# ethz-asl/okvis

Hardware: AMD Instinct MI355X
Metric: Gauss-Newton iterations/sec on 10-KF x 2-cam x 400-landmark windows (batch throughput: window-iterations/s) (higher is better)
Workload: dtype f64

## Files before the change

include/okvis_amd_ba.h:

```cpp
#ifndef OKVIS_AMD_BA_H_
#define OKVIS_AMD_BA_H_

#include <stdint.h>

#ifdef __cplusplus
extern "C" {
#endif

#define OKVIS_BA_ABI_VERSION 7

#define OKVIS_BA_OK 0
#define OKVIS_BA_ERR_ARG (-1)
#define OKVIS_BA_ERR_STATE (-2)
#define OKVIS_BA_ERR_UNSUPPORTED (-3)
#define OKVIS_BA_ERR_NO_DEVICE (-4)
#define OKVIS_BA_ERR_NUMERIC (-5)
#define OKVIS_BA_HIP_ERROR_BASE 1000

#define OKVIS_BA_DIST_NONE 0
#define OKVIS_BA_DIST_RADTAN 1
#define OKVIS_BA_DIST_EQUIDISTANT 2
#define OKVIS_BA_DIST_RADTAN8 3

#define OKVIS_BA_IMU_CACHE_DOUBLES 290
// ... 11 lines not shown
  double a_max;
} okvis_ba_imu_params;

typedef struct okvis_ba_window {
  int32_t n_pose;
  const double* pose;
  const uint8_t* pose_fixed;
  int32_t n_sb;
  const double* sb;
  const uint8_t* sb_fixed;
  int32_t n_lm;
  const double* lm;

  int32_t n_cam;
  const double* cam_intr;
  const int32_t* cam_model;

  int32_t n_obs;
  const int32_t* obs_lm;
  const int32_t* obs_pose;
  const int32_t* obs_ext;
  const int32_t* obs_cam;
  const double* obs_uv;
  const double* obs_sqrtw;
  double cauchy_b;

  int32_t n_imu;
  const int32_t* imu_pose0;
  const int32_t* imu_sb0;
  const int32_t* imu_pose1;
  const int32_t* imu_sb1;
  const int64_t* imu_t0;
  const int64_t* imu_t1;
  const int32_t* imu_s_begin;
  const int32_t* imu_s_count;
  int32_t n_imu_samples;
  const int64_t* imu_s_t;
  const double* imu_s_gyr;
  const double* imu_s_acc;
  okvis_ba_imu_params imu_params;

  int32_t n_pprior;
  const int32_t* pprior_pose;
  const double* pprior_meas;
  const double* pprior_sqrtinfo;

  int32_t n_sbprior;
  const int32_t* sbprior_sb;
  const double* sbprior_meas;
  const double* sbprior_sqrtinfo;

  int32_t n_relpose;
  const int32_t* rel_pose0;
  const int32_t* rel_pose1;
  const double* rel_sqrtinfo;

  int32_t marg_dim;
  int32_t marg_nblocks;
  const int32_t* marg_block_type;
  const int32_t* marg_block_idx;
  const int32_t* marg_block_off;
  const double* marg_J;
  const double* marg_e0;
  const double* marg_lin;

  const double* imu_sb_ref;
  const uint8_t* imu_sb_ref_valid;
  const double* imu_cache;
} okvis_ba_window;

#define OKVIS_BA_STRATEGY_DOGLEG 0
#define OKVIS_BA_STRATEGY_LM 1
#define OKVIS_BA_TUNE_SCHUR_DECIDES 0x1u
#define OKVIS_BA_TUNE_SCHUR_VALU 0x2u
#define OKVIS_BA_TUNE_SCHUR_MFMA_LARGE 0x4u
#define OKVIS_BA_TUNE_NO_LDL_COMP 0x8u
#define OKVIS_BA_TUNE_LDL_COMP_ALL 0x10u
#define OKVIS_BA_TUNE_H0_ON_HOST 0x20u
#define OKVIS_BA_TUNE_NO_EARLY_PREINTEGRATION 0x40u
#define OKVIS_BA_TUNE_NO_MARG_TILES 0x80u
#define OKVIS_BA_TUNE_NO_SMALL_RIDE 0x100u
#define OKVIS_BA_TUNE_SCHUR_SERIAL_BATCHES 0x200u
#define OKVIS_BA_TUNE_LIN_NO_RECORDS 0x400u
#define OKVIS_BA_SOLVE_AUTO 0
#define OKVIS_BA_SOLVE_DENSE 1
#define OKVIS_BA_SOLVE_CHAIN 2
typedef struct okvis_ba_tuning {
  uint32_t flags;
  int32_t fused_max_windows;
  int32_t group_lm;
  int32_t group_work;
  int32_t split_small_min;
  int32_t lin2_occupancy;
  int32_t stagger_us;
  int32_t solve_mode;
} okvis_ba_tuning;
typedef struct okvis_ba_options {
  double initial_radius;
  double max_radius;
  double min_radius;
  double min_lm_diagonal;
  double max_lm_diagonal;
  double min_relative_decrease;
  double function_tolerance;
  double gradient_tolerance;
  double parameter_tolerance;
  int32_t use_graph;
  int32_t schur_lm_per_block;
  int32_t debug_arrays;
  int32_t gauss_newton;
  int32_t n_streams;
  int32_t fp32_linearize;
  int32_t strategy;
  int32_t jacobi_scaling;
  int32_t max_consecutive_invalid_steps;
  int32_t reserved0;
  okvis_ba_tuning tuning;
} okvis_ba_options;

typedef struct okvis_ba_summary {
  double initial_cost;
  double final_cost;
  int32_t iterations;
  int32_t successful_steps;
  int32_t termination;
  int32_t reserved;
  double final_radius;
  double gradient_max_norm;
} okvis_ba_summary;

typedef struct okvis_ba_limits {
  int32_t max_obs_per_lm;
  int32_t max_reduced_dim;
  int32_t max_marg_dim;
  int32_t max_imu_samples_per_factor;
} okvis_ba_limits;

typedef struct okvis_ba_solver okvis_ba_solver;

enum okvis_ba_array {
  OKVIS_BA_ARR_POSE = 0,
  OKVIS_BA_ARR_SB = 1,
  OKVIS_BA_ARR_LM = 2,
  OKVIS_BA_ARR_OBS_RESIDUAL = 3,
  OKVIS_BA_ARR_LM_V = 4,
  OKVIS_BA_ARR_LM_B = 5,
  OKVIS_BA_ARR_LM_HQ = 6,
  OKVIS_BA_ARR_PAIR_W = 7,
  OKVIS_BA_ARR_REDUCED_S = 8,
  OKVIS_BA_ARR_REDUCED_RHS = 9,
  OKVIS_BA_ARR_STEP = 10,
  OKVIS_BA_ARR_LM_QUALITY = 11,
  OKVIS_BA_ARR_GRADIENT = 12,
  OKVIS_BA_ARR_IMU_RESIDUAL = 13,
  OKVIS_BA_ARR_HPP = 14,
  OKVIS_BA_ARR_DAMPING = 15,
  OKVIS_BA_ARR_IMU_SB_REF = 16,
  OKVIS_BA_ARR_IMU_LIN = 17
};
#define OKVIS_BA_IMU_LIN_DOUBLES 511

int okvis_ba_abi_version(void);
void okvis_ba_get_limits(okvis_ba_limits* out);
void okvis_ba_default_options(okvis_ba_options* out);
const char* okvis_ba_error_string(int status);

int okvis_ba_create(okvis_ba_solver** out, int device);
int okvis_ba_destroy(okvis_ba_solver* s);

int okvis_ba_upload(okvis_ba_solver* s, int n_windows, const okvis_ba_window* windows);
int okvis_ba_check_window(const okvis_ba_window* w, const okvis_ba_options* opt, int64_t* stats);
#define OKVIS_BA_LIST_GROUPS 0
#define OKVIS_BA_LIST_LM_OBS_BEGIN 1
#define OKVIS_BA_LIST_LM_PAIR_BEGIN 2
#define OKVIS_BA_LIST_PAIR_LM 3
#define OKVIS_BA_LIST_PAIR_BLOCK 4
#define OKVIS_BA_LIST_PAIR_OFF 5
#define OKVIS_BA_LIST_PAIR_ROLE 6
#define OKVIS_BA_LIST_LM_PIECE_BEGIN 7
#define OKVIS_BA_LIST_PAIR_PIECE 8
#define OKVIS_BA_LIST_PAIR_LIST_BEGIN 9
#define OKVIS_BA_LIST_PAIR_LIST 10
#define OKVIS_BA_LIST_TASKS 11
#define OKVIS_BA_LIST_TASK_LIST 12
#define OKVIS_BA_LIST_CHUNKS 13
#define OKVIS_BA_LIST_CHUNK_DIAG_BEGIN 14
#define OKVIS_BA_LIST_CHUNK_DIAG_OUT 15
#define OKVIS_BA_LIST_CHUNK_DESC 16
#define OKVIS_BA_LIST_PIECE_PATH 17
#define OKVIS_BA_LIST_LDL_COMP 18
#define OKVIS_BA_LIST_CHAIN 19
#define OKVIS_BA_LIST_CHUNK_RECS 20
#define OKVIS_BA_LIST_GROUP_RECS 21
int okvis_ba_check_window_lists(const okvis_ba_window* w, const okvis_ba_options* opt, int32_t n_windows, int32_t which,
                                int32_t* out, int64_t capacity, int64_t* n);
#define OKVIS_BA_PATCH_POSE_PRIORS 1
#define OKVIS_BA_PATCH_SB_PRIORS 2
#define OKVIS_BA_PATCH_RELPOSE 4
#define OKVIS_BA_PATCH_MARG_PRIOR 8
typedef struct okvis_ba_patch {
  int32_t n_remove_obs;  const int32_t* remove_obs;
  int32_t n_remove_lm;   const int32_t* remove_lm;
  int32_t n_remove_pose; const int32_t* remove_pose;
  int32_t n_remove_sb;   const int32_t* remove_sb;
  int32_t n_remove_imu;  const int32_t* remove_imu;
  int32_t n_add_pose; const double* add_pose;  const uint8_t* add_pose_fixed;
  int32_t n_add_sb;   const double* add_sb;    const uint8_t* add_sb_fixed;
  int32_t n_add_lm;   const double* add_lm;
  int32_t n_add_obs;
  const int32_t* add_obs_lm; const int32_t* add_obs_pose; const int32_t* add_obs_ext; const int32_t* add_obs_cam;
  const double* add_obs_uv; const double* add_obs_sqrtw;
  int32_t n_add_imu;
  const int32_t* add_imu_pose0; const int32_t* add_imu_sb0; const int32_t* add_imu_pose1; const int32_t* add_imu_sb1;
  const int64_t* add_imu_t0; const int64_t* add_imu_t1; const int32_t* add_imu_s_begin; const int32_t* add_imu_s_count;
  int32_t n_add_imu_samples;
  const int64_t* add_imu_s_t; const double* add_imu_s_gyr; const double* add_imu_s_acc;
  int32_t replace;
  int32_t n_pprior;  const int32_t* pprior_pose; const double* pprior_meas; const double* pprior_sqrtinfo;
  int32_t n_sbprior; const int32_t* sbprior_sb;  const double* sbprior_meas; const double* sbprior_sqrtinfo;
  int32_t n_relpose; const int32_t* rel_pose0; const int32_t* rel_pose1; const double* rel_sqrtinfo;
  int32_t marg_dim; int32_t marg_nblocks; const int32_t* marg_block_type; const int32_t* marg_block_idx; const int32_t* marg_block_off;
  const double* marg_J; const double* marg_e0; const double* marg_lin;
  int32_t n_set_pose; const int32_t* set_pose_idx; const double* set_pose;
  int32_t n_set_sb;   const int32_t* set_sb_idx;   const double* set_sb;
  int32_t n_set_lm;   const int32_t* set_lm_idx;   const double* set_lm;
  const int32_t* add_lm_before;
} okvis_ba_patch;

typedef struct okvis_ba_window_store okvis_ba_window_store;
int okvis_ba_store_create(const okvis_ba_window* w, okvis_ba_window_store** out);
int okvis_ba_store_patch(okvis_ba_window_store* st, const okvis_ba_patch* p);
int okvis_ba_store_view(const okvis_ba_window_store* st, okvis_ba_window* out);
void okvis_ba_store_destroy(okvis_ba_window_store* st);

int okvis_ba_set_patchable(okvis_ba_solver* s, int on);
int okvis_ba_patch_window(okvis_ba_solver* s, int w, const okvis_ba_patch* p);
int okvis_ba_patched_view(okvis_ba_solver* s, int w, okvis_ba_window* out);
int okvis_ba_set_marg_prior_values(okvis_ba_solver* s, int w, const double* J, const double* e0);

int okvis_ba_set_state(okvis_ba_solver* s, int w, const double* pose, const double* sb, const double* lm);
int okvis_ba_set_options(okvis_ba_solver* s, const okvis_ba_options* opt);

int okvis_ba_optimize(okvis_ba_solver* s, int num_iter, okvis_ba_summary* summaries);

int okvis_ba_optimize_timed(okvis_ba_solver* s, int max_iter, int min_iter, double time_limit_s,
                            okvis_ba_summary* summaries);

int okvis_ba_begin(okvis_ba_solver* s);
int okvis_ba_iterate(okvis_ba_solver* s, int n);
int okvis_ba_finish(okvis_ba_solver* s, okvis_ba_summary* summaries);

int okvis_ba_evaluate_cost(okvis_ba_solver* s, double* costs);

int okvis_ba_get_state(okvis_ba_solver* s, int w, double* pose, double* sb, double* lm);
int okvis_ba_fetch_results(okvis_ba_solver* s, int w, double* pose, double* sb, double* lm, double* lm_quality,
                           double* imu_sb_ref);
int okvis_ba_fetch_imu_caches(okvis_ba_solver* s, int w, double* caches);
int okvis_ba_array_size(okvis_ba_solver* s, int w, int which, int64_t* n_doubles);
int okvis_ba_download(okvis_ba_solver* s, int w, int which, double* out, int64_t n_doubles);
int okvis_ba_reduced_dim(okvis_ba_solver* s, int w, int32_t* dim);
int okvis_ba_pair_count(okvis_ba_solver* s, int w, int32_t* n_pair);
int okvis_ba_pairs(okvis_ba_solver* s, int w, int32_t* pair_lm, int32_t* pair_block);

int okvis_ba_last_iterate_ms(okvis_ba_solver* s, float* total_ms);
int okvis_ba_profile_iterations(okvis_ba_solver* s, int n, float* ms4);
int okvis_ba_profile_launches(okvis_ba_solver* s, int n, float* ms );
int okvis_ba_algorithmic_bytes(okvis_ba_solver* s, int64_t* linearize_bytes, int64_t* schur_bytes,
                               int64_t* solve_bytes, int64_t* small_bytes);
int okvis_ba_synchronize(okvis_ba_solver* s);
int okvis_ba_helper_timeouts(okvis_ba_solver* s, int64_t* count);
#define OKVIS_BA_ROUTE_WINDOWS 0
#define OKVIS_BA_ROUTE_FUSED 1
#define OKVIS_BA_ROUTE_DECISION_FREE_SCHUR 2
#define OKVIS_BA_ROUTE_PIECE_PATH 3
#define OKVIS_BA_ROUTE_SPLIT_SMALL 4
#define OKVIS_BA_ROUTE_SUB_BATCHES 5
#define OKVIS_BA_ROUTE_SUB_BATCH_MAX_WINDOWS 6
#define OKVIS_BA_ROUTE_SCHUR_KERNEL 7
#define OKVIS_BA_ROUTE_SOLVE_DBUF 8
#define OKVIS_BA_ROUTE_SOLVE_TILED 9
#define OKVIS_BA_ROUTE_SOLVE_HELPERS 10
#define OKVIS_BA_ROUTE_GRAPH 11
#define OKVIS_BA_ROUTE_MAX_CHUNKS 12
#define OKVIS_BA_ROUTE_SLOTS 13
#define OKVIS_BA_ROUTE_SOLVE_MODE 14
#define OKVIS_BA_ROUTE_SMALL_RIDES 15
#define OKVIS_BA_ROUTE_LIN_RECORDS 16
#define OKVIS_BA_ROUTE_COUNT 17
int okvis_ba_launch_route(okvis_ba_solver* s, int32_t* route);

#define OKVIS_BA_MARG_MAX_WINDOW_DIM 900
typedef struct okvis_ba_marg_spec {
  const uint8_t* pose_marg;
  const uint8_t* sb_marg;
  int32_t prior_dim, prior_nblocks;
  const int32_t* prior_block_type;
  const int32_t* prior_block_idx;
  const int32_t* prior_block_off;
  const double* prior_H;
  const double* prior_b0;
} okvis_ba_marg_spec;

typedef struct okvis_ba_marg_result {
  int32_t capacity_dim, capacity_blocks;
  int32_t dim, nblocks, rank;
  int32_t* block_type;
  int32_t* block_idx;
  int32_t* block_off;
  double* H;
  double* b0;
  double* J;
  double* e0;
  int32_t sweeps[2];
} okvis_ba_marg_result;

int okvis_ba_marginalize(okvis_ba_solver* s, int w, const okvis_ba_marg_spec* spec, okvis_ba_marg_result* result);
int okvis_ba_marginalize_begin(okvis_ba_solver* s, int w, const okvis_ba_marg_spec* spec, okvis_ba_marg_result* result);
int okvis_ba_marginalize_end(okvis_ba_solver* s, okvis_ba_marg_result* result);
int okvis_ba_marginalize_batch(okvis_ba_solver* s, int w0, int n, const okvis_ba_marg_spec* specs, okvis_ba_marg_result* results);
int okvis_ba_marginalize_batch_begin(okvis_ba_solver* s, int w0, int n, const okvis_ba_marg_spec* specs, okvis_ba_marg_result* results);
int okvis_ba_marginalize_batch_end(okvis_ba_solver* s, okvis_ba_marg_result* results);

#define OKVIS_BA_COV_MAX_WINDOW_DIM 174
#define OKVIS_BA_COV_MAX_DIM 30

typedef struct okvis_ba_cov_spec {
  int32_t n_blocks;
  const int32_t *block_type, *block_idx;
} okvis_ba_cov_spec;

typedef struct okvis_ba_cov_result {
  int32_t capacity;
  int32_t dim, info;
  double min_pivot;
  double* cov;
  double* S0;
} okvis_ba_cov_result;

int okvis_ba_state_covariance(okvis_ba_solver* s, int w0, int n,
                              const okvis_ba_cov_spec* specs, okvis_ba_cov_result* results);
int okvis_ba_last_covariance_ms(okvis_ba_solver* s, float* assembly_ms, float* kernel_ms);

typedef struct okvis_ba_lmcov_spec {
  int32_t n_lm;
  const int32_t* lm_idx;
} okvis_ba_lmcov_spec;

typedef struct okvis_ba_lmcov_result {
  int32_t capacity;
  int32_t n, info;
  double min_pivot;
  double* cov;
  uint8_t* flags;
  double *S0, *Spp, *V, *W;
} okvis_ba_lmcov_result;

int okvis_ba_landmark_covariance(okvis_ba_solver* s, int w0, int n,
                                 const okvis_ba_lmcov_spec* specs, okvis_ba_lmcov_result* results);
int okvis_ba_last_landmark_covariance_ms(okvis_ba_solver* s, float* assembly_ms, float* inverse_ms, float* landmark_ms);

#define OKVIS_BA_PRED_NO_COV 1
#define OKVIS_BA_PRED_NO_PROJECTION 2

typedef struct okvis_ba_pred_spec {
  int32_t n_q;
  const int32_t *q_lm, *q_pose, *q_ext, *q_cam;
} okvis_ba_pred_spec;

typedef struct okvis_ba_pred_result {
  int32_t capacity;
  int32_t n, info;
  double min_pivot;
// ... 35 lines not shown
```

okvis_amd/_lib.py:

```python
from __future__ import annotations

import ctypes as C
import os

from .window import CovResultC, CovSpecC, LimitsC, LmcovResultC, LmcovSpecC, MargResultC, MargSpecC, OptionsC, PatchC, PredResultC, PredSpecC, SummaryC, WindowC

_HERE = os.path.dirname(os.path.abspath(__file__))
LIB_PATH = os.path.join(os.environ.get("OKVIS_AMD_LIB_DIR") or os.path.join(_HERE, "lib"), "libokvis_amd_ba.so")

SYMBOLS = [
    "okvis_ba_abi_version", "okvis_ba_get_limits", "okvis_ba_default_options", "okvis_ba_error_string",
    "okvis_ba_create", "okvis_ba_destroy", "okvis_ba_upload", "okvis_ba_check_window", "okvis_ba_check_window_lists", "okvis_ba_set_state", "okvis_ba_set_options",
    "okvis_ba_optimize", "okvis_ba_optimize_timed", "okvis_ba_begin", "okvis_ba_iterate", "okvis_ba_finish",
    "okvis_ba_evaluate_cost", "okvis_ba_get_state", "okvis_ba_fetch_results", "okvis_ba_fetch_imu_caches", "okvis_ba_array_size", "okvis_ba_download",
    "okvis_ba_reduced_dim", "okvis_ba_pair_count", "okvis_ba_pairs", "okvis_ba_last_iterate_ms",
    "okvis_ba_profile_iterations", "okvis_ba_profile_launches", "okvis_ba_algorithmic_bytes", "okvis_ba_synchronize",
    "okvis_ba_helper_timeouts", "okvis_ba_launch_route", "okvis_ba_marginalize", "okvis_ba_marginalize_begin", "okvis_ba_marginalize_end",
    "okvis_ba_marginalize_batch", "okvis_ba_marginalize_batch_begin", "okvis_ba_marginalize_batch_end",
    "okvis_ba_state_covariance", "okvis_ba_last_covariance_ms",
    "okvis_ba_landmark_covariance", "okvis_ba_last_landmark_covariance_ms",
    "okvis_ba_predicted_measurement", "okvis_ba_last_predicted_measurement_ms",
    "okvis_ba_store_create", "okvis_ba_store_patch", "okvis_ba_store_view", "okvis_ba_store_destroy", "okvis_ba_set_patchable",
    "okvis_ba_patch_window", "okvis_ba_patched_view", "okvis_ba_set_marg_prior_values",
    "okvis_ba_dense_solve", "okvis_ba_reduced_solve", "okvis_ba_shard", "okvis_ba_batch_run", "okvis_ba_gather_records", "okvis_ba_batch_run_gathered",
]

_dp = C.POINTER(C.c_double)
_ip = C.POINTER(C.c_int32)
_lib = None


class BackendError(RuntimeError):
    def __init__(self, status, what=""):
        self.status = status
        msg = lib().okvis_ba_error_string(status).decode() if _lib is not None else str(status)
        super().__init__(f"okvis_ba status {status}: {msg} {what}")


def lib():
    global _lib
    if _lib is not None:
        return _lib
    if not os.path.exists(LIB_PATH):
        raise ImportError(f"{LIB_PATH} is missing: run `python -m okvis_amd.build` (hipcc, gfx950). "
                          "okvis_amd has no CPU fallback.")
    L = C.CDLL(LIB_PATH)
    for s in SYMBOLS:
        getattr(L, s)
    vp = C.c_void_p
    L.okvis_ba_error_string.restype = C.c_char_p
    L.okvis_ba_error_string.argtypes = [C.c_int]
    L.okvis_ba_get_limits.argtypes = [C.POINTER(LimitsC)]
    L.okvis_ba_default_options.argtypes = [C.POINTER(OptionsC)]
    L.okvis_ba_create.argtypes = [C.POINTER(vp), C.c_int]
    L.okvis_ba_destroy.argtypes = [vp]
    L.okvis_ba_upload.argtypes = [vp, C.c_int, C.POINTER(WindowC)]
    L.okvis_ba_set_state.argtypes = [vp, C.c_int, _dp, _dp, _dp]
    L.okvis_ba_store_create.argtypes = [C.POINTER(WindowC), C.POINTER(vp)]
    L.okvis_ba_store_patch.argtypes = [vp, C.POINTER(PatchC)]
    L.okvis_ba_store_view.argtypes = [vp, C.POINTER(WindowC)]
    L.okvis_ba_store_destroy.argtypes = [vp]
    L.okvis_ba_store_destroy.restype = None
    L.okvis_ba_set_patchable.argtypes = [vp, C.c_int]
    L.okvis_ba_patch_window.argtypes = [vp, C.c_int, C.POINTER(PatchC)]
    L.okvis_ba_patched_view.argtypes = [vp, C.c_int, C.POINTER(WindowC)]
    L.okvis_ba_set_marg_prior_values.argtypes = [vp, C.c_int, _dp, _dp]
    L.okvis_ba_check_window.argtypes = [C.POINTER(WindowC), C.POINTER(OptionsC), C.POINTER(C.c_int64)]
    L.okvis_ba_check_window_lists.argtypes = [C.POINTER(WindowC), C.POINTER(OptionsC), C.c_int32, C.c_int32, _ip, C.c_int64,
                                              C.POINTER(C.c_int64)]
    L.okvis_ba_get_state.argtypes = [vp, C.c_int, _dp, _dp, _dp]
    L.okvis_ba_fetch_results.argtypes = [vp, C.c_int, _dp, _dp, _dp, _dp, _dp]
    L.okvis_ba_fetch_imu_caches.argtypes = [vp, C.c_int, _dp]
    L.okvis_ba_set_options.argtypes = [vp, C.POINTER(OptionsC)]
    L.okvis_ba_optimize.argtypes = [vp, C.c_int, C.POINTER(SummaryC)]
    L.okvis_ba_optimize_timed.argtypes = [vp, C.c_int, C.c_int, C.c_double, C.POINTER(SummaryC)]
    L.okvis_ba_begin.argtypes = [vp]
    L.okvis_ba_iterate.argtypes = [vp, C.c_int]
    L.okvis_ba_finish.argtypes = [vp, C.POINTER(SummaryC)]
    L.okvis_ba_dense_solve.argtypes = [C.c_int, C.c_int32, _dp, _dp, _dp, C.POINTER(C.c_int32)]
    L.okvis_ba_reduced_solve.argtypes = [C.c_int, C.c_int32, C.c_int32, C.c_int32, C.c_uint32, _dp, _dp, _dp, C.POINTER(C.c_int64),
                                         C.POINTER(C.c_int32), C.c_int32, _dp, C.c_int64]
    L.okvis_ba_shard.argtypes = [C.c_int32, C.c_int32, C.c_int32, _ip, C.POINTER(C.c_int32)]
    L.okvis_ba_batch_run.argtypes = [C.c_int, C.c_int32, C.c_int32, C.c_int32, C.POINTER(WindowC), C.POINTER(OptionsC), C.c_int,
                                     C.c_void_p, C.POINTER(C.c_int32)]
    L.okvis_ba_marginalize.argtypes = [vp, C.c_int, C.POINTER(MargSpecC), C.POINTER(MargResultC)]
    L.okvis_ba_marginalize_begin.argtypes = [vp, C.c_int, C.POINTER(MargSpecC), C.POINTER(MargResultC)]
    L.okvis_ba_marginalize_end.argtypes = [vp, C.POINTER(MargResultC)]
    L.okvis_ba_marginalize_batch.argtypes = [vp, C.c_int, C.c_int, C.POINTER(MargSpecC), C.POINTER(MargResultC)]
    L.okvis_ba_marginalize_batch_begin.argtypes = [vp, C.c_int, C.c_int, C.POINTER(MargSpecC), C.POINTER(MargResultC)]
    L.okvis_ba_marginalize_batch_end.argtypes = [vp, C.POINTER(MargResultC)]
    L.okvis_ba_state_covariance.argtypes = [vp, C.c_int, C.c_int, C.POINTER(CovSpecC), C.POINTER(CovResultC)]
    L.okvis_ba_last_covariance_ms.argtypes = [vp, C.POINTER(C.c_float), C.POINTER(C.c_float)]
    L.okvis_ba_landmark_covariance.argtypes = [vp, C.c_int, C.c_int, C.POINTER(LmcovSpecC), C.POINTER(LmcovResultC)]
    L.okvis_ba_last_landmark_covariance_ms.argtypes = [vp] + [C.POINTER(C.c_float)] * 3
    L.okvis_ba_predicted_measurement.argtypes = [vp, C.c_int, C.c_int, C.POINTER(PredSpecC), C.POINTER(PredResultC)]
    L.okvis_ba_last_predicted_measurement_ms.argtypes = [vp] + [C.POINTER(C.c_float)] * 3
    L.okvis_ba_evaluate_cost.argtypes = [vp, _dp]
    L.okvis_ba_array_size.argtypes = [vp, C.c_int, C.c_int, C.POINTER(C.c_int64)]
    L.okvis_ba_download.argtypes = [vp, C.c_int, C.c_int, _dp, C.c_int64]
    L.okvis_ba_reduced_dim.argtypes = [vp, C.c_int, _ip]
    L.okvis_ba_pair_count.argtypes = [vp, C.c_int, _ip]
    L.okvis_ba_helper_timeouts.argtypes = [vp, C.POINTER(C.c_int64)]
    L.okvis_ba_launch_route.argtypes = [vp, _ip]
    L.okvis_ba_pairs.argtypes = [vp, C.c_int, _ip, _ip]
    L.okvis_ba_last_iterate_ms.argtypes = [vp, C.POINTER(C.c_float)]
    L.okvis_ba_profile_iterations.argtypes = [vp, C.c_int, C.POINTER(C.c_float)]
    L.okvis_ba_profile_launches.argtypes = [vp, C.c_int, C.POINTER(C.c_float)]
    L.okvis_ba_algorithmic_bytes.argtypes = [vp] + [C.POINTER(C.c_int64)] * 4
    L.okvis_ba_synchronize.argtypes = [vp]
    _lib = L
    return L


def check(status, what=""):
    if status != 0:
        raise BackendError(status, what)
```

okvis_amd/csrc/ba_capi.hip:

```cpp
#include <hip/hip_runtime.h>

#include <algorithm>
#include <array>
#include <chrono>
#include <cstdio>
#include <cstring>
#include <map>
#include <string>
#include <type_traits>
#include <vector>

#include "../../include/okvis_amd_ba.h"
#include "ba_imu.hpp"
#include "ba_chol_tiles.hpp"
#include "ba_cov.hpp"
#include "ba_lmcov.hpp"
#include "ba_predcov.hpp"
#include "ba_linearize.hpp"
#include "ba_linearize2.hpp"
#include "ba_schur2.hpp"
#include "ba_marg.hpp"
#include "ba_marg_tiles.hpp"
#include "ba_schur.hpp"
#include "ba_solve.hpp"
#include "ba_store.hpp"

using namespace ba;

#include "capi_solver.inc"
#include "capi_index_build.inc"
#include "capi_launch.inc"

#define REFUSE_BETWEEN_MARG_HALVES(s) do { if ((s) && (s)->marg_pending.active) return OKVIS_BA_ERR_STATE; } while (0)

extern "C" {

int okvis_ba_abi_version(void) { return OKVIS_BA_ABI_VERSION; }

void okvis_ba_get_limits(okvis_ba_limits* out) {
  if (!out) return;
  out->max_obs_per_lm = GROUP_OBS;
  out->max_reduced_dim = MAX_D;
  out->max_marg_dim = MAX_MARG_DIM;
  out->max_imu_samples_per_factor = MAX_IMU_SAMPLES;
}

void okvis_ba_default_options(okvis_ba_options* o) {
  if (!o) return;
  o->initial_radius = 1e4;
  o->max_radius = 1e16;
  o->min_radius = 1e-32;
  o->min_lm_diagonal = 1e-6;
  o->max_lm_diagonal = 1e32;
  o->min_relative_decrease = 1e-3;
  o->function_tolerance = 1e-6;
  o->gradient_tolerance = 1e-10;
  o->parameter_tolerance = 1e-8;
  o->use_graph = 1;
  o->schur_lm_per_block = 0;
  o->debug_arrays = 0;
  o->gauss_newton = 0;
  o->n_streams = 0;
  o->fp32_linearize = 0;
  o->strategy = OKVIS_BA_STRATEGY_DOGLEG;
  o->jacobi_scaling = 1;
  o->max_consecutive_invalid_steps = 5;
  o->reserved0 = 0;
  std::memset(&o->tuning, 0, sizeof(o->tuning));
}

const char* okvis_ba_error_string(int status) {
  switch (status) {
    case OKVIS_BA_OK: return "ok";
    case OKVIS_BA_ERR_ARG: return "invalid argument (null pointer, index out of range, unsorted/duplicate observations)";
    case OKVIS_BA_ERR_STATE: return "call order violated";
    case OKVIS_BA_ERR_UNSUPPORTED: return "structure exceeds a documented limit (okvis_ba_get_limits)";
    case OKVIS_BA_ERR_NO_DEVICE: return "no HIP device visible: this backend has no CPU path";
    case OKVIS_BA_ERR_NUMERIC: return "numeric failure";
  }
  if (status >= OKVIS_BA_HIP_ERROR_BASE) return hipGetErrorString((hipError_t)(status - OKVIS_BA_HIP_ERROR_BASE));
  return "unknown status";
}

int okvis_ba_create(okvis_ba_solver** out, int device) {
  if (!out) return OKVIS_BA_ERR_ARG;
  *out = nullptr;
  int n = 0;
  if (hipGetDeviceCount(&n) != hipSuccess || n <= 0) return OKVIS_BA_ERR_NO_DEVICE;
  if (device < 0 || device >= n) return OKVIS_BA_ERR_ARG;
  okvis_ba_solver* s = new okvis_ba_solver();
  s->device = device;
  okvis_ba_default_options(&s->opt);
  s->stagger_ticks = 10 * 100;
  hipError_t e = hipSetDevice(device);
  if (e == hipSuccess) e = hipStreamCreateWithFlags(&s->stream, hipStreamNonBlocking);
  if (e == hipSuccess) e = hipEventCreate(&s->ev0);
  if (e == hipSuccess) e = hipEventCreate(&s->ev1);
  if (e == hipSuccess) e = hipEventCreateWithFlags(&s->ev_fork, hipEventDisableTiming);
  if (e == hipSuccess) e = hipMalloc(&s->d_opt, records_bytes(1));
  if (e == hipSuccess) {
    s->d_wins = reinterpret_cast<WinPtrs*>(reinterpret_cast<unsigned char*>(s->d_opt) + OPT_PAD);
    s->d_ctrl = reinterpret_cast<CtrlSlot*>(reinterpret_cast<unsigned char*>(s->d_opt) + ctrl_off(1));
    s->wins_capacity = 1;
  }
  auto lds = [&](auto f, size_t bytes) {
    if (e == hipSuccess) e = hipFuncSetAttribute(reinterpret_cast<const void*>(f), hipFuncAttributeMaxDynamicSharedMemorySize, (int)bytes);
  };
  for (const auto& k : plan_kernels()) lds(k.first, k.second);
  lds(&chol_tiles_window_kernel, CT_SMEM_DOUBLES * 8);
  lds(&marg_dense_kernel<MAX_D_LDS, MARG_SMALL_PRIOR>, MARG_LDS_DOUBLES * 8);
  lds(&marg_dense_kernel<MAX_D, MAX_MARG_DIM>, MARG_LDS_DOUBLES_LARGE * 8);
  lds(&cov_kernel, cov_lds_bytes(MAX_D_LDS));

  if (e != hipSuccess) {
    int code = OKVIS_BA_HIP_ERROR_BASE + (int)e;
    okvis_ba_destroy(s);
    return code;
  }
  *out = s;
  return OKVIS_BA_OK;
}

int okvis_ba_destroy(okvis_ba_solver* s) {
  if (!s) return OKVIS_BA_OK;
  (void)hipSetDevice(s->device);
  destroy_graphs(s);
  if (s->d_arena) (void)hipFree(s->d_arena);
  if (s->d_pre) (void)hipFree(s->d_pre);
  if (s->ev_marg_vals) (void)hipEventDestroy(s->ev_marg_vals);
  if (s->d_opt) (void)hipFree(s->d_opt);
  if (s->h_ctrl_stage) (void)hipHostFree(s->h_ctrl_stage);
  if (s->d_ctrl_stage) (void)hipFree(s->d_ctrl_stage);
  if (s->marg_scratch) (void)hipFree(s->marg_scratch);
  for (auto ev : s->ev_cov)
    if (ev) (void)hipEventDestroy(ev);
  for (auto ev : s->ev_lmcov)
    if (ev) (void)hipEventDestroy(ev);
  for (auto ev : s->ev_pred)
    if (ev) (void)hipEventDestroy(ev);
  if (s->ev0) (void)hipEventDestroy(s->ev0);
  if (s->ev1) (void)hipEventDestroy(s->ev1);
  if (s->ev_fork) (void)hipEventDestroy(s->ev_fork);
  for (auto st : s->sub_streams)
    if (st != s->stream) (void)hipStreamDestroy(st);
  for (auto ev : s->sub_events) (void)hipEventDestroy(ev);
  if (s->stream) (void)hipStreamDestroy(s->stream);
  delete s;
  return OKVIS_BA_OK;
}

int okvis_ba_set_options(okvis_ba_solver* s, const okvis_ba_options* opt) {
  if (!s || !opt) return OKVIS_BA_ERR_ARG;
  if (!(opt->initial_radius > 0) || !(opt->min_lm_diagonal > 0) || !(opt->max_lm_diagonal >= opt->min_lm_diagonal))
    return OKVIS_BA_ERR_ARG;
  if (s->uploaded && (opt->debug_arrays != s->opt.debug_arrays || opt->schur_lm_per_block != s->opt.schur_lm_per_block ||
                      opt->n_streams != s->opt.n_streams))
    return OKVIS_BA_ERR_STATE;
  if (s->uploaded) {
    const uint32_t per_call = OKVIS_BA_TUNE_NO_MARG_TILES | OKVIS_BA_TUNE_NO_EARLY_PREINTEGRATION | OKVIS_BA_TUNE_H0_ON_HOST;
    okvis_ba_tuning a = opt->tuning, b = s->opt.tuning;
    a.flags &= ~per_call; b.flags &= ~per_call;
    a.stagger_us = b.stagger_us = 0;
    if (std::memcmp(&a, &b, sizeof(a)) != 0) return OKVIS_BA_ERR_STATE;
  }
  if (std::memcmp(opt, &s->opt, sizeof(*opt)) == 0) return OKVIS_BA_OK;
  s->opt = *opt;
  if (s->uploaded) {
    s->plan = make_plan(s->layout, s->max, s->opt, (int)s->wins.size());
    keep_graphs(s);
  }
  s->stagger_ticks = (long long)(opt->tuning.stagger_us > 0 ? opt->tuning.stagger_us : opt->tuning.stagger_us < 0 ? 0 : 10) * 100;
  HIP_TRY(hipSetDevice(s->device));
  OptD d = make_optd(s->opt, (int)s->wins.size());
  HIP_TRY(hipMemcpyAsync(s->d_opt, &d, sizeof(d), hipMemcpyHostToDevice, s->stream));
  HIP_TRY(hipStreamSynchronize(s->stream));
  return OKVIS_BA_OK;
}

static int upload_impl(okvis_ba_solver* s, int n_windows, const okvis_ba_window* windows);

int okvis_ba_upload(okvis_ba_solver* s, int n_windows, const okvis_ba_window* windows) {
  if (!s || n_windows <= 0 || !windows) return OKVIS_BA_ERR_ARG;
  const int rc = upload_impl(s, n_windows, windows);
  s->mirror_fresh = false;
  if (rc != OKVIS_BA_OK || !s->patchable) {
    s->mirrors.clear();
    return rc;
  }
  const auto t_c0 = std::chrono::steady_clock::now();
  struct Note {
    std::chrono::steady_clock::time_point t0;
    ~Note() {
      if (g_build_times.on) g_build_times.ms["upload: copy into the container"] += std::chrono::duration<double, std::milli>(std::chrono::steady_clock::now() - t0).count();
    }
  } note{t_c0};
  try {
    s->mirrors.resize((size_t)n_windows);
    for (int i = 0; i < n_windows; ++i)
      if (int rs = s->mirrors[i].assign(windows[i])) {
        s->mirrors.clear();
        return rs;
      }
  } catch (const std::bad_alloc&) {
    s->mirrors.clear();
    return OKVIS_BA_ERR_ARG;
  }
  s->mirror_fresh = true;
  return OKVIS_BA_OK;
}

constexpr int PRE_MAX_TERMS = 8;
static int pre_launch(okvis_ba_solver* s, int n_windows, const okvis_ba_window* windows, const int2** where_dev, const ImuCacheD** src_dev) {
  if (s->opt.tuning.flags & OKVIS_BA_TUNE_NO_EARLY_PREINTEGRATION) return 0;
  struct Item {
    int w, f;
// ... 173 lines not shown
        hipStream_t st;
        hipEvent_t ev;
        if (k == 0) st = s->stream;
        else HIP_TRY(hipStreamCreateWithFlags(&st, hipStreamNonBlocking));
        HIP_TRY(hipEventCreateWithFlags(&ev, hipEventDisableTiming));
        s->sub_streams.push_back(st);
        s->sub_events.push_back(ev);
      }
    }
  }
  keep_graphs(s);
  s->uploaded = true;
  s->evaluated = false;
  s->res_staged = false;
  s->acc_fresh = true;
  if (g_build_times.on) {
    const auto t_u2 = std::chrono::steady_clock::now();
    auto d = [](auto a, auto b) { return std::chrono::duration<double, std::milli>(b - a).count(); };
    g_build_times.ms["upload_impl: wait for the stream"] += d(t_enter, t_synced);
    g_build_times.ms["upload_impl: index build (sum of the sections)"] += d(t_u0, t_u1);
    g_build_times.ms["upload_impl: staging + enqueue"] += d(t_u1, t_u2);
    g_build_times.ms["upload_impl calls"] += 1.0;
  }
  if (dbg_t) {
    const auto t_u2 = std::chrono::steady_clock::now();
    std::fprintf(stderr, "upload: sync %.3f ms, graphs %.3f ms, index build %.3f ms, staging + enqueue %.3f ms, arena %zu bytes data + %zu zero\n",
                 std::chrono::duration<double, std::milli>(t_synced - t_enter).count(),
                 std::chrono::duration<double, std::milli>(t_u0 - t_synced).count(),
                 std::chrono::duration<double, std::milli>(t_u1 - t_u0).count(),
                 std::chrono::duration<double, std::milli>(t_u2 - t_u1).count(), (size_t)A.size, (size_t)A.zsize);
  }
  return OKVIS_BA_OK;
}

int okvis_ba_check_window(const okvis_ba_window* w, const okvis_ba_options* opt, int64_t* stats) {
  if (!w) return OKVIS_BA_ERR_ARG;
  okvis_ba_options o;
  if (opt) o = *opt; else okvis_ba_default_options(&o);
  Arena A;
  HostWin H;
  static thread_local StageVec kept;
  const bool dumping = !debug_word().arena.empty();
  if (!dumping) A.host.swap(kept);
  struct GiveBack {
    StageVec& a;
    StageVec& b;
    bool on;
    ~GiveBack() {
      if (on) a.swap(b);
    }
  } give_back{A.host, kept, !dumping};
  BatchLayout L = batch_layout(o, 1);
  if (int rc = build_batch(w, 1, o, L, A, &H)) return rc;
  if (dumping) {
    if (FILE* f = std::fopen(debug_word().arena.c_str(), "wb")) {
      std::fwrite(A.host.data(), 1, A.size, f);
      std::fwrite(&H.ptrs, 1, sizeof(H.ptrs), f);
      std::fclose(f);
    }
  }
  if (stats) {
    stats[0] = H.D; stats[1] = H.Dp; stats[2] = H.n_pair; stats[3] = H.n_group; stats[4] = H.n_chunk;
    stats[5] = H.ptrs.n_task; stats[6] = H.ptrs.gpart_size; stats[7] = (int64_t)A.total();
  }
  return OKVIS_BA_OK;
}

int okvis_ba_check_window_lists(const okvis_ba_window* w, const okvis_ba_options* opt, int32_t n_windows, int32_t which,
                                int32_t* out, int64_t capacity, int64_t* n) {
  if (!w || !n || n_windows <= 0 || capacity < 0 || (capacity > 0 && !out)) return OKVIS_BA_ERR_ARG;
  okvis_ba_options o;
  if (opt) o = *opt; else okvis_ba_default_options(&o);
  Arena A;
  HostWin H;
  BatchLayout L = batch_layout(o, n_windows);
  if (int rc = build_batch(w, 1, o, L, A, &H)) return rc;
  const WinPtrs& P = H.ptrs;
  const unsigned char* base = A.host.data();
  auto at = [&](const void* field) { return base + reinterpret_cast<size_t>(field); };
  const int nb = P.Dp / 6;
  const void* src = nullptr;
  int64_t count = 0;
  int width = 4;
  switch (which) {
    case OKVIS_BA_LIST_GROUPS: src = at((const void*)P.groups), count = 16 * (int64_t)P.n_group; break;
    case OKVIS_BA_LIST_LM_OBS_BEGIN: src = at((const void*)P.lm_obs_begin), count = P.n_lm + 1; break;
    case OKVIS_BA_LIST_LM_PAIR_BEGIN: src = at((const void*)P.lm_pair_begin), count = P.n_lm + 1; break;
    case OKVIS_BA_LIST_PAIR_LM: src = at((const void*)P.pair_lm), count = P.n_pair; break;
    case OKVIS_BA_LIST_PAIR_BLOCK: src = at((const void*)P.pair_block), count = P.lin2 ? P.n_pair : 0; break;
    case OKVIS_BA_LIST_PAIR_OFF: src = at((const void*)P.pair_off), count = P.n_pair; break;
    case OKVIS_BA_LIST_PAIR_ROLE: src = at((const void*)P.pair_role), count = P.n_pair; break;
    case OKVIS_BA_LIST_LM_PIECE_BEGIN: src = at((const void*)P.lm_piece_begin), count = P.lin2 ? P.n_lm + 1 : 0; break;
    case OKVIS_BA_LIST_PAIR_PIECE: src = at((const void*)P.pair_piece), count = P.lin2 ? P.n_pair : 0; break;
    case OKVIS_BA_LIST_PAIR_LIST_BEGIN: src = at((const void*)P.pair_list_begin), count = P.n_pair + 1; break;
    case OKVIS_BA_LIST_PAIR_LIST:
      src = at((const void*)P.pair_list), width = 2;
      count = reinterpret_cast<const int*>(at((const void*)P.pair_list_begin))[P.n_pair];
      break;
    case OKVIS_BA_LIST_TASKS: src = at((const void*)P.tasks), count = 6 * (int64_t)P.n_task; break;
    case OKVIS_BA_LIST_TASK_LIST: {
      src = at((const void*)P.task_list), width = 2;
      const Group* g = reinterpret_cast<const Group*>(at((const void*)P.groups));
      count = P.n_group ? g[P.n_group - 1].tlist_end : 0;
      break;
    }
    case OKVIS_BA_LIST_CHUNKS: src = at((const void*)P.chunks), count = 2 * (int64_t)P.n_chunk; break;
    case OKVIS_BA_LIST_CHUNK_DIAG_BEGIN: src = at((const void*)P.chunk_diag_begin), count = (int64_t)P.n_chunk * nb + 1; break;
    case OKVIS_BA_LIST_CHUNK_DIAG_OUT:
      src = at((const void*)P.chunk_diag_out);
      count = reinterpret_cast<const int*>(at((const void*)P.chunk_diag_begin))[(size_t)P.n_chunk * nb];
      break;
    case OKVIS_BA_LIST_CHUNK_DESC: src = at((const void*)P.chunk_desc), count = (int64_t)P.n_chunk * SCHUR_DESC_INTS; break;
    case OKVIS_BA_LIST_PIECE_PATH: count = 1; break;
    case OKVIS_BA_LIST_LDL_COMP: count = 1; break;
    case OKVIS_BA_LIST_CHAIN: count = 1; break;
    case OKVIS_BA_LIST_CHUNK_RECS: {
      size_t off = 0;
      const int stride = build_chunk_records(A, &H, 1, &off);
      src = A.host.data() + off, count = (int64_t)stride * SCHUR_REC_INTS;
      break;
    }
    case OKVIS_BA_LIST_GROUP_RECS: {
      size_t off = 0;
      const int stride = build_group_records(A, &H, 1, &off);
      src = A.host.data() + off, count = (int64_t)stride * LIN_REC_INTS;
      break;
    }
    default: return OKVIS_BA_ERR_ARG;
  }
  *n = count;
  if (capacity < count) return OKVIS_BA_ERR_ARG;
  if (which == OKVIS_BA_LIST_PIECE_PATH) {
    out[0] = P.lin2;
  } else if (which == OKVIS_BA_LIST_LDL_COMP) {
    out[0] = (int32_t)P.ldl_comp;
  } else if (which == OKVIS_BA_LIST_CHAIN) {
    out[0] = P.chain;
  } else if (width == 4) {
    if (count) std::memcpy(out, src, 4 * (size_t)count);
  } else {
    const uint16_t* s16 = static_cast<const uint16_t*>(src);
    for (int64_t i = 0; i < count; ++i) out[i] = s16[i];
  }
  return OKVIS_BA_OK;
}

int okvis_ba_set_state(okvis_ba_solver* s, int w, const double* pose, const double* sb, const double* lm) {
  REFUSE_BETWEEN_MARG_HALVES(s);
  if (!s || !s->uploaded || w < 0 || w >= (int)s->wins.size()) return s && !s->uploaded ? OKVIS_BA_ERR_STATE : OKVIS_BA_ERR_ARG;
  HIP_TRY(hipSetDevice(s->device));
  if (int rc = refresh_acc(s, w)) return rc;
  HostWin& H = s->wins[w];
  if (pose) HIP_TRY(hipMemcpyAsync(H.ptrs.pose[H.acc], pose, 56 * (size_t)H.n_pose, hipMemcpyHostToDevice, s->stream));
  if (sb) HIP_TRY(hipMemcpyAsync(H.ptrs.sb[H.acc], sb, 72 * (size_t)H.n_sb, hipMemcpyHostToDevice, s->stream));
  if (lm) HIP_TRY(hipMemcpyAsync(H.ptrs.lm[H.acc], lm, 32 * (size_t)H.n_lm, hipMemcpyHostToDevice, s->stream));
  HIP_TRY(hipStreamSynchronize(s->stream));
  s->begun = false;
  s->res_staged = s->mirror_fresh = false;
  return OKVIS_BA_OK;
}

int okvis_ba_get_state(okvis_ba_solver* s, int w, double* pose, double* sb, double* lm) {
  REFUSE_BETWEEN_MARG_HALVES(s);
  if (!s || !s->uploaded || w < 0 || w >= (int)s->wins.size()) return s && !s->uploaded ? OKVIS_BA_ERR_STATE : OKVIS_BA_ERR_ARG;
  HIP_TRY(hipSetDevice(s->device));
  if (int rc = refresh_acc(s, w)) return rc;
  HostWin& H = s->wins[w];
  if (pose) HIP_TRY(hipMemcpyAsync(pose, H.ptrs.pose[H.acc], 56 * (size_t)H.n_pose, hipMemcpyDeviceToHost, s->stream));
  if (sb) HIP_TRY(hipMemcpyAsync(sb, H.ptrs.sb[H.acc], 72 * (size_t)H.n_sb, hipMemcpyDeviceToHost, s->stream));
  if (lm) HIP_TRY(hipMemcpyAsync(lm, H.ptrs.lm[H.acc], 32 * (size_t)H.n_lm, hipMemcpyDeviceToHost, s->stream));
  HIP_TRY(hipStreamSynchronize(s->stream));
  return OKVIS_BA_OK;
}

static int stage_results(okvis_ba_solver* s, int w, const unsigned char** rec) {
  HostWin& H = s->wins[w];
  *rec = nullptr;
  if (s->marg_pending.active) return OKVIS_BA_ERR_STATE;
  const size_t total = results_bytes(H.n_pose, H.n_sb, H.n_lm, H.n_imu);
  if (total == 0) return OKVIS_BA_OK;
  if (s->res_staged && w == 0 && s->wins.size() == 1) {
    *rec = s->stage_res.data();
    return OKVIS_BA_OK;
  }
  if (int rc = refresh_acc(s, w)) return rc;
  s->stage_dl.resize(total);
  HIP_TRY(launch_imu_take_back(s, w, 1));
  hipLaunchKernelGGL(pack_results_kernel, dim3(8), dim3(256), 0, s->stream, s->d_wins + w, H.acc);
  HIP_TRY(hipGetLastError());
  HIP_TRY(hipMemcpyAsync(s->stage_dl.data(), H.ptrs.results, total, hipMemcpyDeviceToHost, s->stream));
  HIP_TRY(hipStreamSynchronize(s->stream));
  *rec = s->stage_dl.data();
  return OKVIS_BA_OK;
}

int okvis_ba_set_patchable(okvis_ba_solver* s, int on) {
  if (!s) return OKVIS_BA_ERR_ARG;
  s->patchable = on != 0;
  if (!s->patchable) s->mirrors.clear();
  return OKVIS_BA_OK;
}

static int refresh_mirrors(okvis_ba_solver* s) {
  if (s->mirror_fresh) return OKVIS_BA_OK;
  for (size_t i = 0; i < s->wins.size(); ++i) {
    const unsigned char* rec = nullptr;
    if (int rc = stage_results(s, (int)i, &rec)) return rc;
    if (rec) s->mirrors[i].take_results(rec, s->evaluated);
  }
  s->mirror_fresh = true;
// ... 87 lines not shown
    HIP_TRY(hipGetLastError());
  } else {
    HIP_TRY(hipMemcpyAsync(dJ, h, span, hipMemcpyHostToDevice, s->stream));
  }
  HIP_TRY(hipEventRecord(s->ev_marg_vals, s->stream));
  if (s->patchable && (size_t)w < s->mirrors.size()) {
    try {
      s->mirrors[w].marg_J.assign(J, J + (size_t)Dm * Dm);
      s->mirrors[w].marg_e0.assign(e0, e0 + Dm);
    } catch (const std::bad_alloc&) {
      s->mirrors.clear();
      s->mirror_fresh = false;
    }
  }
  s->begun = false;
  s->evaluated = false;
  s->res_staged = false;
  return OKVIS_BA_OK;
}

int okvis_ba_patched_view(okvis_ba_solver* s, int w, okvis_ba_window* out) {
  if (!s || !out) return OKVIS_BA_ERR_ARG;
  if (!s->patchable || s->mirrors.size() != s->wins.size() || s->mirrors.empty()) return OKVIS_BA_ERR_STATE;
  if (w < 0 || w >= (int)s->mirrors.size()) return OKVIS_BA_ERR_ARG;
  if (s->uploaded) {
    HIP_TRY(hipSetDevice(s->device));
    if (int rc = refresh_mirrors(s)) return rc;
  }
  s->mirrors[w].view(out);
  return OKVIS_BA_OK;
}

int okvis_ba_fetch_results(okvis_ba_solver* s, int w, double* pose, double* sb, double* lm, double* lm_quality,
                           double* imu_sb_ref) {
  REFUSE_BETWEEN_MARG_HALVES(s);
  if (!s || !s->uploaded || w < 0 || w >= (int)s->wins.size()) return s && !s->uploaded ? OKVIS_BA_ERR_STATE : OKVIS_BA_ERR_ARG;
  HIP_TRY(hipSetDevice(s->device));
  HostWin& H = s->wins[w];
  const size_t b_pose = 56 * (size_t)H.n_pose, b_sb = 72 * (size_t)H.n_sb, b_lm = 32 * (size_t)H.n_lm;
  const size_t b_q = 8 * (size_t)H.n_lm, b_ref = 72 * (size_t)H.n_imu;
  const size_t o_sb = b_pose, o_lm = o_sb + b_sb, o_q = o_lm + b_lm, o_ref = o_q + b_q, total = o_ref + b_ref;
  if (total == 0) return OKVIS_BA_OK;
  const unsigned char* st = nullptr;
  if (int rc = stage_results(s, w, &st)) return rc;
  if (pose && b_pose) std::memcpy(pose, st, b_pose);
  if (sb && b_sb) std::memcpy(sb, st + o_sb, b_sb);
  if (lm && b_lm) std::memcpy(lm, st + o_lm, b_lm);
  if (lm_quality && b_q) std::memcpy(lm_quality, st + o_q, b_q);
  if (imu_sb_ref && b_ref) std::memcpy(imu_sb_ref, st + o_ref, b_ref);
  return OKVIS_BA_OK;
}

int okvis_ba_fetch_imu_caches(okvis_ba_solver* s, int w, double* caches) {
  REFUSE_BETWEEN_MARG_HALVES(s);
  if (!s || !s->uploaded || w < 0 || w >= (int)s->wins.size()) return s && !s->uploaded ? OKVIS_BA_ERR_STATE : OKVIS_BA_ERR_ARG;
  if (!caches) return OKVIS_BA_ERR_ARG;
  HIP_TRY(hipSetDevice(s->device));
  HostWin& H = s->wins[w];
  if (H.n_imu == 0) return OKVIS_BA_OK;
  const unsigned char* st = nullptr;
  if (int rc = stage_results(s, w, &st)) return rc;
  std::memcpy(caches, st + results_bytes(H.n_pose, H.n_sb, H.n_lm, 0) + 72 * (size_t)H.n_imu, sizeof(ImuCacheD) * (size_t)H.n_imu);
  return OKVIS_BA_OK;
}

int okvis_ba_begin(okvis_ba_solver* s) {
  REFUSE_BETWEEN_MARG_HALVES(s);
  if (s) s->acc_fresh = s->res_staged = s->mirror_fresh = false;
  if (!s) return OKVIS_BA_ERR_ARG;
  if (!s->uploaded) return OKVIS_BA_ERR_STATE;
  HIP_TRY(hipSetDevice(s->device));
  s->slots = 0;
  {
    const size_t n = s->wins.size();
    HIP_TRY(reserve_ctrl_stage(s, n));
    int* accs = reinterpret_cast<int*>(s->h_ctrl_stage);
    for (size_t i = 0; i < n; ++i) accs[i] = s->wins[i].acc;
    HIP_TRY(hipMemcpyAsync(s->d_ctrl_stage, accs, sizeof(int) * n, hipMemcpyHostToDevice, s->stream));
    hipLaunchKernelGGL(begin_kernel, dim3((unsigned)n), dim3(256), 0, s->stream, s->d_wins, reinterpret_cast<const int*>(s->d_ctrl_stage),
                       s->opt.initial_radius);
    HIP_TRY(hipGetLastError());
  }
  HIP_TRY(launch_lin(s, whole(s), 1));
  s->begun = true;
  s->evaluated = true;
  return OKVIS_BA_OK;
}

int okvis_ba_iterate(okvis_ba_solver* s, int n) {
  REFUSE_BETWEEN_MARG_HALVES(s);
  if (s) s->acc_fresh = false;
  if (!s || n < 0) return OKVIS_BA_ERR_ARG;
  if (!s->begun) return OKVIS_BA_ERR_STATE;
  if (n == 0) return OKVIS_BA_OK;
  HIP_TRY(hipSetDevice(s->device));
  s->slots += n;
  HIP_TRY(hipEventRecord(s->ev0, s->stream));
  const int nsub = (int)s->sub_streams.size();
  if (s->plan.graph && nsub > 1) {
    HIP_TRY(hipEventRecord(s->ev_fork, s->stream));
    for (int k = 0; k < nsub; ++k) {
      hipGraphExec_t exec = nullptr;
      auto it = s->sub_graphs.find({n, k});
      if (it == s->sub_graphs.end()) {
        hipGraph_t graph = nullptr;
        const Sub b = sub(s->sub_streams[k], s->plan.subs[k]);
        HIP_TRY(hipStreamBeginCapture(b.st, hipStreamCaptureModeRelaxed));
        hipError_t e = launch_chain(s, b, n, n);
        hipError_t e2 = hipStreamEndCapture(b.st, &graph);
        if (e != hipSuccess) HIP_TRY(e);
        HIP_TRY(e2);
        HIP_TRY(hipGraphInstantiate(&exec, graph, nullptr, nullptr, 0));
        HIP_TRY(hipGraphDestroy(graph));
        s->sub_graphs[{n, k}] = exec;
      } else {
        exec = it->second;
      }
      HIP_TRY(hipStreamWaitEvent(s->sub_streams[k], s->ev_fork, 0));
      if (k > 0 && s->stagger_ticks > 0) {
        hipLaunchKernelGGL(delay_kernel, dim3(1), dim3(64), 0, s->sub_streams[k], (long long)k * s->stagger_ticks);
        HIP_TRY(hipGetLastError());
      }
      HIP_TRY(hipGraphLaunch(exec, s->sub_streams[k]));
      HIP_TRY(hipEventRecord(s->sub_events[k], s->sub_streams[k]));
      HIP_TRY(hipStreamWaitEvent(s->stream, s->sub_events[k], 0));
    }
  } else if (s->plan.graph) {
    hipGraphExec_t exec = nullptr;
    auto it = s->graphs.find(n);
    if (it == s->graphs.end()) {
      hipGraph_t graph = nullptr;
      HIP_TRY(hipStreamBeginCapture(s->stream, hipStreamCaptureModeRelaxed));
      hipError_t e = launch_iterations_forked(s, n);
      hipError_t e2 = hipStreamEndCapture(s->stream, &graph);
      if (e != hipSuccess) HIP_TRY(e);
      HIP_TRY(e2);
      HIP_TRY(hipGraphInstantiate(&exec, graph, nullptr, nullptr, 0));
      HIP_TRY(hipGraphDestroy(graph));
      s->graphs[n] = exec;
      HIP_TRY(hipEventRecord(s->ev0, s->stream));
    } else {
      exec = it->second;
    }
    HIP_TRY(hipGraphLaunch(exec, s->stream));
  } else {
    HIP_TRY(launch_iterations_forked(s, n));
  }
  HIP_TRY(hipEventRecord(s->ev1, s->stream));
  return OKVIS_BA_OK;
}

int okvis_ba_last_iterate_ms(okvis_ba_solver* s, float* total_ms) {
  if (!s || !total_ms) return OKVIS_BA_ERR_ARG;
  HIP_TRY(hipSetDevice(s->device));
  HIP_TRY(hipEventSynchronize(s->ev1));
  HIP_TRY(hipEventElapsedTime(total_ms, s->ev0, s->ev1));
  return OKVIS_BA_OK;
}

int okvis_ba_finish(okvis_ba_solver* s, okvis_ba_summary* summaries) {
  REFUSE_BETWEEN_MARG_HALVES(s);
  if (!s) return OKVIS_BA_ERR_ARG;
  if (!s->begun) return OKVIS_BA_ERR_STATE;
  HIP_TRY(hipSetDevice(s->device));
  HIP_TRY(launch_schur(s, whole(s), 1));
  HIP_TRY(launch_solve(s, whole(s), 1));
  std::vector<Ctrl> cs;
  size_t res_bytes = 0;
  auto finalize = [&]() -> int {
    HIP_TRY(launch_imu_take_back(s, 0, (int)s->wins.size()));
    if (s->max.lm > 0) {
      hipLaunchKernelGGL(quality_kernel, dim3((s->max.lm + 255) / 256, (unsigned)s->wins.size()), dim3(256), 0, s->stream, s->d_wins);
      HIP_TRY(hipGetLastError());
    }
    if (s->wins.size() == 1) {
      const HostWin& H0 = s->wins[0];
      res_bytes = results_bytes(H0.n_pose, H0.n_sb, H0.n_lm, H0.n_imu);
      if (res_bytes) {
        s->stage_res.resize(res_bytes);
        hipLaunchKernelGGL(pack_results_kernel, dim3(8), dim3(256), 0, s->stream, s->d_wins, -1);
        HIP_TRY(hipGetLastError());
        HIP_TRY(hipMemcpyAsync(s->stage_res.data(), H0.ptrs.results, res_bytes, hipMemcpyDeviceToHost, s->stream));
      }
    }
    return fetch_ctrl(s, cs);
  };
  int rc = finalize();
  if (rc != OKVIS_BA_OK) return rc;
  if (s->opt.strategy == OKVIS_BA_STRATEGY_DOGLEG && !s->opt.gauss_newton) {
    for (int round = 0; round < 64 && !s->skip_topup; ++round) {
      int need = 0;
      for (const Ctrl& c : cs) {
        if (c.done) continue;
        int k = c.max_iter - c.iter;
        if (c.explicit_next == 2) k += 1;
        need = std::max(need, k);
      }
      if (need <= 0) break;
      s->slots += need;
      HIP_TRY(launch_iterations_forked(s, need, 0));
      HIP_TRY(launch_schur(s, whole(s), 1));
      HIP_TRY(launch_solve(s, whole(s), 1));
      rc = finalize();
      if (rc != OKVIS_BA_OK) return rc;
    }
  }
  s->res_staged = res_bytes > 0;
  for (size_t i = 0; i < s->wins.size(); ++i) {
    s->wins[i].acc = cs[i].acc;
    if (summaries) {
      okvis_ba_summary& o = summaries[i];
      o.initial_cost = cs[i].initial_cost;
      o.final_cost = cs[i].cost;
      o.iterations = cs[i].iter;
      o.successful_steps = cs[i].successful;
      o.termination = cs[i].done ? (cs[i].done - 1 == 6 ? 0 : cs[i].done - 1) : 0;
      o.reserved = cs[i].chol_fail;
      o.final_radius = cs[i].radius;
      o.gradient_max_norm = cs[i].grad_max;
    }
  }
  s->begun = false;
  s->acc_fresh = true;
  return OKVIS_BA_OK;
}

int okvis_ba_optimize(okvis_ba_solver* s, int num_iter, okvis_ba_summary* summaries) {
  int rc = okvis_ba_begin(s);
  if (rc != OKVIS_BA_OK) return rc;
  rc = okvis_ba_iterate(s, num_iter);
  if (rc != OKVIS_BA_OK) return rc;
  return okvis_ba_finish(s, summaries);
}

int okvis_ba_optimize_timed(okvis_ba_solver* s, int max_iter, int min_iter, double time_limit_s,
                            okvis_ba_summary* summaries) {
  if (!s || max_iter < 0 || min_iter < 0) return OKVIS_BA_ERR_ARG;
  const auto t0 = std::chrono::steady_clock::now();
  int rc = okvis_ba_begin(s);
  if (rc != OKVIS_BA_OK) return rc;
  int done = 0;
  if (time_limit_s < 0) {
    rc = okvis_ba_iterate(s, max_iter);
    if (rc != OKVIS_BA_OK) return rc;
  } else {
    const int first = std::min(min_iter, max_iter);
    rc = okvis_ba_iterate(s, first);
    if (rc != OKVIS_BA_OK) return rc;
    done = first;
    while (done < max_iter) {
      HIP_TRY(hipStreamSynchronize(s->stream));
      const double el = std::chrono::duration<double>(std::chrono::steady_clock::now() - t0).count();
      if (done >= min_iter && el > time_limit_s) {
        s->skip_topup = true;
        break;
      }
      rc = okvis_ba_iterate(s, 1);
      if (rc != OKVIS_BA_OK) return rc;
      ++done;
    }
  }
  rc = okvis_ba_finish(s, summaries);
  s->skip_topup = false;
  return rc;
}

int okvis_ba_evaluate_cost(okvis_ba_solver* s, double* costs) {
  if (s) s->acc_fresh = false;
  if (!s || !costs) return OKVIS_BA_ERR_ARG;
  int rc = okvis_ba_begin(s);
  if (rc != OKVIS_BA_OK) return rc;
  std::vector<okvis_ba_summary> sum(s->wins.size());
  rc = okvis_ba_finish(s, sum.data());
  if (rc != OKVIS_BA_OK) return rc;
  for (size_t i = 0; i < sum.size(); ++i) costs[i] = sum[i].final_cost;
  return OKVIS_BA_OK;
}

int okvis_ba_reduced_dim(okvis_ba_solver* s, int w, int32_t* dim) {
  if (!s || !dim || w < 0 || w >= (int)s->wins.size()) return OKVIS_BA_ERR_ARG;
  *dim = s->wins[w].D;
  return OKVIS_BA_OK;
}
int okvis_ba_helper_timeouts(okvis_ba_solver* s, int64_t* count) {
  if (!s || !count) return OKVIS_BA_ERR_ARG;
  if (!s->uploaded) return OKVIS_BA_ERR_STATE;
  HIP_TRY(hipSetDevice(s->device));
  HIP_TRY(hipStreamSynchronize(s->stream));
  *count = 0;
  for (const HostWin& H : s->wins) {
    int n = 0;
    HIP_TRY(hipMemcpy(&n, H.ptrs.sum_sync + 2, sizeof(int), hipMemcpyDeviceToHost));
    *count += n;
  }
  return OKVIS_BA_OK;
}
int okvis_ba_launch_route(okvis_ba_solver* s, int32_t* route) {
  if (!s || !route) return OKVIS_BA_ERR_ARG;
  if (!s->uploaded) return OKVIS_BA_ERR_STATE;
  const LaunchPlan& p = s->plan;
  const Extent& big = *std::max_element(p.subs.begin(), p.subs.end(), [](const Extent& a, const Extent& b) { return a.nw < b.nw; });
  route[OKVIS_BA_ROUTE_WINDOWS] = p.whole.nw;
  route[OKVIS_BA_ROUTE_FUSED] = p.fused;
  route[OKVIS_BA_ROUTE_DECISION_FREE_SCHUR] = p.nodec;
  route[OKVIS_BA_ROUTE_PIECE_PATH] = p.lin2;
  route[OKVIS_BA_ROUTE_SPLIT_SMALL] = p.split_small;
  route[OKVIS_BA_ROUTE_SUB_BATCHES] = (int)p.subs.size();
  route[OKVIS_BA_ROUTE_SUB_BATCH_MAX_WINDOWS] = big.nw;
  route[OKVIS_BA_ROUTE_SCHUR_KERNEL] = p.schur.k == SCHUR_RIDE3 ? SCHUR_MFMA3 : p.schur.k >= SCHUR_MFMA3_SERIAL ? 4 : p.schur.k;
  route[OKVIS_BA_ROUTE_SOLVE_DBUF] = p.solve.k == SOLVE_DENSE_DBUF || p.solve.k == SOLVE_CHAIN_DBUF;
  route[OKVIS_BA_ROUTE_SOLVE_TILED] = p.tiled.k != SOLVE_NONE;
  route[OKVIS_BA_ROUTE_SOLVE_HELPERS] = big.helpers;
  route[OKVIS_BA_ROUTE_GRAPH] = p.graph;
  route[OKVIS_BA_ROUTE_MAX_CHUNKS] = s->max.chunks;
  route[OKVIS_BA_ROUTE_SLOTS] = (int32_t)std::min<long long>(s->slots, 0x7fffffff);
  route[OKVIS_BA_ROUTE_SMALL_RIDES] = p.rides;
  route[OKVIS_BA_ROUTE_LIN_RECORDS] = p.grec_stride > 0;
  route[OKVIS_BA_ROUTE_SOLVE_MODE] = p.solve.k == SOLVE_NONE ? 0 : p.solve.k >= SOLVE_CHAIN ? OKVIS_BA_SOLVE_CHAIN : OKVIS_BA_SOLVE_DENSE;
  return OKVIS_BA_OK;
}
int okvis_ba_pair_count(okvis_ba_solver* s, int w, int32_t* n_pair) {
  if (!s || !n_pair || w < 0 || w >= (int)s->wins.size()) return OKVIS_BA_ERR_ARG;
  *n_pair = s->wins[w].n_pair;
  return OKVIS_BA_OK;
}
int okvis_ba_pairs(okvis_ba_solver* s, int w, int32_t* pair_lm, int32_t* pair_block) {
  if (!s || !pair_lm || !pair_block || w < 0 || w >= (int)s->wins.size()) return OKVIS_BA_ERR_ARG;
  const HostWin& H = s->wins[w];
  for (int i = 0; i < H.n_pair; ++i) {
    pair_lm[i] = H.pair_lm[i];
    pair_block[i] = H.pair_block[i];
  }
  return OKVIS_BA_OK;
}

static int locate(okvis_ba_solver* s, int w, int which, const double** ptr, int64_t* n) {
  const HostWin& H = s->wins[w];
  const WinPtrs& P = H.ptrs;
  const int a = H.acc;
  switch (which) {
    case OKVIS_BA_ARR_POSE: *ptr = P.pose[a]; *n = 7 * (int64_t)H.n_pose; return 0;
    case OKVIS_BA_ARR_SB: *ptr = P.sb[a]; *n = 9 * (int64_t)H.n_sb; return 0;
    case OKVIS_BA_ARR_LM: *ptr = P.lm[a]; *n = 4 * (int64_t)H.n_lm; return 0;
    case OKVIS_BA_ARR_OBS_RESIDUAL: *ptr = P.obs_r[a]; *n = 2 * (int64_t)H.n_obs; return P.obs_r[a] ? 0 : OKVIS_BA_ERR_STATE;
    case OKVIS_BA_ARR_LM_V: *ptr = P.V[a]; *n = 6 * (int64_t)H.n_lm; return 0;
    case OKVIS_BA_ARR_LM_B: *ptr = P.bl[a]; *n = 3 * (int64_t)H.n_lm; return 0;
    case OKVIS_BA_ARR_LM_HQ: *ptr = P.Hq[a]; *n = 6 * (int64_t)H.n_lm; return 0;
    case OKVIS_BA_ARR_PAIR_W: *ptr = P.W[a]; *n = 18 * (int64_t)H.n_pair; return 0;
    case OKVIS_BA_ARR_REDUCED_S: *ptr = P.S; *n = (int64_t)H.D * H.D; return P.S ? 0 : OKVIS_BA_ERR_STATE;
    case OKVIS_BA_ARR_REDUCED_RHS: *ptr = P.rhs; *n = H.D; return P.rhs ? 0 : OKVIS_BA_ERR_STATE;
    case OKVIS_BA_ARR_STEP: *ptr = P.step; *n = H.D; return 0;
    case OKVIS_BA_ARR_LM_QUALITY: *ptr = P.quality; *n = H.n_lm; return 0;
    case OKVIS_BA_ARR_GRADIENT: *ptr = P.grad; *n = H.D; return 0;
    case OKVIS_BA_ARR_DAMPING: *ptr = P.Dp2; *n = H.D; return P.Dp2 ? 0 : OKVIS_BA_ERR_STATE;
    case 99: *ptr = P.prof; *n = 64 + 4 * 160; return P.prof ? 0 : OKVIS_BA_ERR_STATE;
    case 98: *ptr = nullptr; *n = H.n_imu; return 0;
    case 97: *ptr = nullptr; *n = 24; return 0;
    case 96: *ptr = nullptr; *n = 1; return 0;
    case 95: *ptr = nullptr; *n = 1 + (int64_t)s->max.grec_stride * LIN_REC_INTS; return 0;
    case OKVIS_BA_ARR_IMU_SB_REF: *ptr = nullptr; *n = 9 * (int64_t)H.n_imu; return 0;
    case OKVIS_BA_ARR_IMU_RESIDUAL: *ptr = nullptr; *n = 15 * (int64_t)H.n_imu; return 0;
    case OKVIS_BA_ARR_IMU_LIN: *ptr = nullptr; *n = OKVIS_BA_IMU_LIN_DOUBLES * (int64_t)H.n_imu; return 0;
  }
  return OKVIS_BA_ERR_ARG;
}

int okvis_ba_array_size(okvis_ba_solver* s, int w, int which, int64_t* n_doubles) {
  if (!s || !n_doubles || !s->uploaded || w < 0 || w >= (int)s->wins.size()) return OKVIS_BA_ERR_ARG;
  const double* p;
  return locate(s, w, which, &p, n_doubles);
}

int okvis_ba_download(okvis_ba_solver* s, int w, int which, double* out, int64_t n_doubles) {
  REFUSE_BETWEEN_MARG_HALVES(s);
  if (!s || !out || !s->uploaded || w < 0 || w >= (int)s->wins.size()) return OKVIS_BA_ERR_ARG;
  HIP_TRY(hipSetDevice(s->device));
  const double* p = nullptr;
  int64_t n = 0;
  if (int rc0 = refresh_acc(s, w)) return rc0;
  int rc = locate(s, w, which, &p, &n);
  if (rc != 0) return rc;
  if (n != n_doubles) return OKVIS_BA_ERR_ARG;
  if (which == OKVIS_BA_ARR_IMU_SB_REF) {
    const HostWin& H = s->wins[w];
    HIP_TRY(launch_imu_take_back(s, w, 1));
    HIP_TRY(hipStreamSynchronize(s->stream));
    if (H.n_imu > 0)
      HIP_TRY(hipMemcpy2D(out, 9 * sizeof(double), reinterpret_cast<const unsigned char*>(H.ptrs.imu_cache) + offsetof(ImuCacheD, sb_ref),
                          sizeof(ImuCacheD), 9 * sizeof(double), (size_t)H.n_imu, hipMemcpyDeviceToHost));
    return OKVIS_BA_OK;
  }
  if (which == 96) {
    out[0] = (double)s->slots;
    return OKVIS_BA_OK;
  }
  if (which == 95) {
    const int stride = s->max.grec_stride;
    std::vector<int> r((size_t)stride * LIN_REC_INTS);
    HIP_TRY(hipStreamSynchronize(s->stream));
    if (stride) HIP_TRY(hipMemcpy(r.data(), s->d_grecs + (size_t)w * stride * LIN_REC_INTS, r.size() * sizeof(int), hipMemcpyDeviceToHost));
    out[0] = stride;
// ... 129 lines not shown
```

okvis_amd/csrc/ba_solve.hpp:

```cpp
#pragma once
#include <climits>
#include "ba_chol_tiles.hpp"
#include "ba_device.hpp"
#include "ba_ldl16.hpp"
#include "ba_chain.hpp"

namespace ba {

constexpr int SBS = 38;
struct SLayout {
  int nbk;
  __device__ __forceinline__ int blk(int bi, int bj) const {
    return (bj * nbk - (bj * (bj - 1)) / 2 + (bi - bj)) * SBS;
  }
  __device__ __forceinline__ int at(int i, int j) const {
    const int bi = i / 6, bj = j / 6;
    return blk(bi, bj) + (i - 6 * bi) * 6 + (j - 6 * bj);
  }
};

template <bool LARGE> struct SolveLayout { typedef SLayout type; };
template <> struct SolveLayout<false> { typedef L16 type; };
__device__ __forceinline__ int imu_dst_off(const SLayout&, const int4& d) { return d.x & 0xFFFFF; }
__device__ __forceinline__ int imu_dst_off(const L16& LY, const int4& d) { return LY.at(d.z >> 16, d.z & 0xFFFF); }
__device__ __forceinline__ int imu_dst_off(const LChain& LY, const int4& d) { return LY.at(d.z >> 16, d.z & 0xFFFF); }

template <class LYT>
__device__ __forceinline__ void add_small_factor(double* S, const LYT LY, double* g, double* d2, const double* J,
                                                 const double* r, int nres, int ncol, const int* col_off, int tid,
                                                 int nthreads) {
  for (int wi = tid; wi < ncol * ncol; wi += nthreads) {
    const int a = wi / ncol, b = wi - a * ncol;
    const int ra = col_off[a], rb = col_off[b];
    if (ra < 0 || rb < 0 || ra < rb) continue;
    double s = 0;
    for (int k = 0; k < nres; ++k) s += J[k * ncol + a] * J[k * ncol + b];
    S[LY.at(ra, rb)] += s;
    if (a == b) d2[ra] += s;
  }
  for (int a = tid; a < ncol; a += nthreads) {
    const int ra = col_off[a];
    if (ra < 0) continue;
    double s = 0;
    for (int k = 0; k < nres; ++k) s += J[k * ncol + a] * r[k];
    g[ra] += s;
  }
}

__device__ __forceinline__ bool chol6(double (&L)[6][6], double (&inv)[6]) {
  bool ok = true;
#pragma unroll
  for (int k = 0; k < 6; ++k) {
    const double d = L[k][k];
    ok = ok && (d > 0.0);
    const double dd = d > 0.0 ? d : 1.0;
    inv[k] = rsqrt_nr(dd);
    L[k][k] = dd * inv[k];
#pragma unroll
    for (int i = k + 1; i < 6; ++i) L[i][k] *= inv[k];
#pragma unroll
    for (int i = k + 1; i < 6; ++i)
#pragma unroll
      for (int j = k + 1; j <= i; ++j) L[i][j] -= L[i][k] * L[j][k];
  }
  return ok;
}


__device__ __forceinline__ void trinv6(const double (&L)[6][6], const double (&inv)[6], double (&X)[6][6]) {
#pragma unroll
  for (int j = 0; j < 6; ++j) {
    X[j][j] = inv[j];
#pragma unroll
    for (int i = j + 1; i < 6; ++i) {
      double a = 0;
#pragma unroll
      for (int m = j; m < i; ++m) a += L[i][m] * X[m][j];
      X[i][j] = -a * inv[i];
    }
  }
}

__device__ __forceinline__ bool factor_diag(const double* dblk, double* Xout) {
  double L[6][6], X[6][6], inv[6];
#pragma unroll
  for (int i = 0; i < 6; ++i)
#pragma unroll
    for (int j = 0; j <= i; ++j) L[i][j] = dblk[6 * i + j];
  const bool ok = chol6(L, inv);
  trinv6(L, inv, X);
#pragma unroll
  for (int i = 0; i < 6; ++i)
#pragma unroll
    for (int j = 0; j <= i; ++j) Xout[6 * i + j] = X[i][j];
  return ok;
}

constexpr int SOLVE_LDS_LIMIT_CHAIN = 144 * 1024;
constexpr int SOLVE_LDS_LIMIT = 148 * 1024;
constexpr int PRI_STAGE = 2;
constexpr int SOLVE_HELPERS = 4;
constexpr int SOLVE_HELPED_MAX_WINDOWS = 8;
constexpr int MARG_BLOCKS_MAX = MAX_MARG_DIM / 6;
constexpr int PRE_BLOCKS = 32;

template <class LYT>
__device__ void assemble_base(const WinPtrs& W, int acc, const LYT LY, double* S, double* g, double* d2,
                              int* coloff, int tid, int nthreads, bool skip_imu,
                              const double* pri = nullptr, const int* pricol = nullptr, int n_pri = 0,
                              bool imu_matrix_elsewhere = false, bool skip_priors = false) {
  static_assert(IMU_LIN_STRIDE == 512, "imu_asm and the factor records share the index");
  {
    const int items = skip_imu ? 0 : W.n_imu * 512;
    constexpr int NE = 6;
    const double* src = W.imu_lin[acc];
    for (int col = 0; col < (skip_imu ? 0 : W.n_imu_color); ++col) {
      if (imu_matrix_elsewhere) {
        for (int it = tid; it < W.n_imu * 60; it += nthreads) {
          const int f = it / 60, k = it - 60 * f;
          const int e = k < 30 ? k * (k + 3) / 2 : 465 + (k - 30);
          const int4 d = W.imu_asm[512 * f + e];
          if (d.x < 0 || (d.x >> 24) != col) continue;
          const double v = src[512 * f + e];
          if (d.x & (1 << 20)) g[d.x & 0xFFFFF] += v;
          else if (d.y >= 0) d2[d.y] += v;
        }
        __syncthreads();
        continue;
      }
      for (int base = tid; base < items; base += NE * nthreads) {
        double v[NE], old[NE];
        int dst[NE], d2i[NE], soff[NE];
#pragma unroll
        for (int u = 0; u < NE; ++u) {
          const int idx = base + u * nthreads;
          dst[u] = -1;
          d2i[u] = -1;
          soff[u] = 0;
          v[u] = 0;
          if (idx < items) {
            const int4 d = W.imu_asm[idx];
            if (d.x >= 0 && (d.x >> 24) == col) {
              dst[u] = d.x;
              d2i[u] = d.y;
              soff[u] = (d.x & (1 << 20)) ? (d.x & 0xFFFFF) : imu_dst_off(LY, d);
            }
            v[u] = (idx & 511) < 495 ? src[idx] : 0.0;
          }
        }
#pragma unroll
        for (int u = 0; u < NE; ++u) old[u] = (dst[u] >= 0 && !(dst[u] & (1 << 20))) ? S[soff[u]] : 0.0;
#pragma unroll
        for (int u = 0; u < NE; ++u) {
          const int d = dst[u];
          if (d < 0) continue;
          const int off = soff[u];
          if (d & (1 << 20)) {
            g[off] += v[u];
          } else {
            S[off] = old[u] + v[u];
            if (d2i[u] >= 0) d2[d2i[u]] += v[u];
          }
        }
      }
      __syncthreads();
    }
  }
  for (int f = 0; f < (skip_priors ? 0 : W.n_pprior); ++f) {
    if (f < n_pri) {
      const double* L = pri + 42 * f;
      add_small_factor(S, LY, g, d2, L, L + 36, 6, 6, pricol + 6 * f, tid, nthreads);
      __syncthreads();
      continue;
    }
    if (tid < 6) {
      const int off = W.pose_off[W.pprior_pose[f]];
      coloff[tid] = off < 0 ? -1 : off + tid;
    }
    __syncthreads();
    const double* L = W.pp_lin[acc] + (size_t)f * 42;
    add_small_factor(S, LY, g, d2, L, L + 36, 6, 6, coloff, tid, nthreads);
    __syncthreads();
  }
  for (int f = 0; f < (skip_priors ? 0 : W.n_sbprior); ++f) {
    const bool st = f < n_pri;
    if (!st) {
      if (tid < 9) {
// ... 158 lines not shown
  }
  *s2 += a2;
  *x2 += b2;
}

__device__ __forceinline__ void dl_landmark_sums(const WinPtrs& W, int acc, const double* xvp, double mu, const OptD& opt,
                                                 int tid, double* Al_out, double* Bl_out) {
  double Al = 0, Bl = 0;
  const double* s_x = xvp;
  for (int l = tid; l < W.n_lm; l += SOLVE_THREADS) {
        const double* Vl = W.V[acc] + 6 * (size_t)l;
        const double* bl = W.bl[acc] + 3 * (size_t)l;
        const double* sl = W.lm_scale + 3 * (size_t)l;
        double v[6] = {Vl[0], Vl[1], Vl[2], Vl[3], Vl[4], Vl[5]};
        const double dt[3] = {damp_diag(v[0], sl[0], opt), damp_diag(v[3], sl[1], opt), damp_diag(v[5], sl[2], opt)};
        const double xl[3] = {bl[0] / dt[0], bl[1] / dt[1], bl[2] / dt[2]};
        double t[3] = {0, 0, 0};
        for (int pr = W.lm_pair_begin[l]; pr < W.lm_pair_begin[l + 1]; ++pr) {
          const double* Wp = W.W[acc] + 18 * (size_t)pr;
          const double* xp = s_x + W.pair_off[pr];
          for (int i = 0; i < 6; ++i) {
            t[0] += Wp[3 * i] * xp[i];
            t[1] += Wp[3 * i + 1] * xp[i];
            t[2] += Wp[3 * i + 2] * xp[i];
          }
        }
        const double quad3 = xl[0] * (v[0] * xl[0] + v[1] * xl[1] + v[2] * xl[2]) +
                             xl[1] * (v[1] * xl[0] + v[3] * xl[1] + v[4] * xl[2]) +
                             xl[2] * (v[2] * xl[0] + v[4] * xl[1] + v[5] * xl[2]);
        v[0] += mu * dt[0];
        v[3] += mu * dt[1];
        v[5] += mu * dt[2];
        double vi[6];
        inv3sym(v, vi);
        const double quad1 = t[0] * (vi[0] * t[0] + vi[1] * t[1] + vi[2] * t[2]) +
                             t[1] * (vi[1] * t[0] + vi[3] * t[1] + vi[4] * t[2]) +
                             t[2] * (vi[2] * t[0] + vi[4] * t[1] + vi[5] * t[2]);
        Al += bl[0] * xl[0] + bl[1] * xl[1] + bl[2] * xl[2];
        Bl += quad1 + 2.0 * (t[0] * xl[0] + t[1] * xl[1] + t[2] * xl[2]) + quad3;
      }
  *Al_out += Al;
  *Bl_out += Bl;
}

__device__ __noinline__ void dogleg_coefficients(double A, double B, double C, double E, double mu, double radius, double* cA,
                                                 double* beta, double* dln, double* model) {
#pragma clang fp contract(off)
  const double alpha = A / B;
  const double gradient_norm = sqrt(A), gn_norm = sqrt(E);
  double a, b, n;
  if (gn_norm <= radius) {
    a = 0.0, b = 1.0, n = gn_norm;
  } else if (gradient_norm * alpha >= radius) {
    a = radius / gradient_norm, b = 0.0, n = radius;
  } else {
    const double b_dot_a = -alpha * C;
    const double a2 = (alpha * gradient_norm) * (alpha * gradient_norm);
    const double bma2 = a2 - 2.0 * b_dot_a + gn_norm * gn_norm;
    const double cc = b_dot_a - a2;
    const double dsc = sqrt(cc * cc + bma2 * (radius * radius - a2));
    b = (cc <= 0.0) ? (dsc - cc) / bma2 : (radius * radius - a2) / (dsc + cc);
    a = alpha * (1.0 - b);
    n = sqrt(a * a * A - 2.0 * a * b * C + b * b * E);
  }
  *cA = a;
  *beta = b;
  *dln = n;
  *model = a * A - b * C - 0.5 * (a * a * B + 2.0 * a * b * (A + mu * C) + b * b * (-C - mu * E));
}

__device__ __forceinline__ void solve_failed_dl(Ctrl* c, const OptD& opt) {
  c->explicit_next = 0;
  c->have_tot = 0;
  c->mu *= DL_MU_INCREASE;
  if (c->mu >= DL_MAX_MU) {
    c->iter++;
    c->invalid_steps++;
    if (c->invalid_steps >= opt.max_invalid) c->done = 5 + 1;
  }
}

template <bool LARGE, bool DBUF, bool CHAIN = false>
__global__ __launch_bounds__(SOLVE_THREADS) void solve_kernel(const WinPtrs* __restrict__ wins,
                                                              const OptD* __restrict__ optp, int final_only, CtrlSlot* ctrls) {
  static_assert(!(LARGE && DBUF), "windows solved in HBM are never fused");
  static_assert(!(LARGE && CHAIN), "the chain solver is an LDS solver");
  extern __shared__ __attribute__((aligned(16))) double smem[];
  const long long t_start = clock64();
  const WinPtrs& W = wins[blockIdx.x];
  Ctrl* gctrl = &ctrls[blockIdx.x].c;
  typedef int ctrl_v4 __attribute__((ext_vector_type(4)));
  const ctrl_v4 chead = *as_global(reinterpret_cast<const ctrl_v4*>(gctrl));
  int warm = 0;
  {
    constexpr int lines = (int)((sizeof(WinPtrs) + 63) / 64);
    static_assert(sizeof(WinPtrs) % 4 == 0 && (lines - 1) * 64 < (int)sizeof(WinPtrs), "lines touched below");
    const int* wi = reinterpret_cast<const int*>(&W);
#pragma unroll
    for (int k = 0; k < lines; ++k) warm |= wi[16 * k];
  }
  const int spec0 = __builtin_amdgcn_readfirstlane(chead.y ? 1 - chead.x : chead.x);
  if (final_only == 0x7ffffff1 && warm == 0x5a5a5a5a) return;
  if (LARGE != (W.Sg != nullptr)) return;
  if (!LARGE && CHAIN != (W.chain != 0)) return;
  const int tid = threadIdx.x;
  if (W.prof && tid == 0 && blockIdx.x == 0 && blockIdx.y + 1 == gridDim.y) {
    W.prof[43] = (double)t_start;
    W.prof[40] = (double)clock64();
  }
  if constexpr (!LARGE) {
    if (blockIdx.y + 1 < gridDim.y) {
      const int nh = (int)gridDim.y - 1;
      const int ntot = W.spart_stride, per = (ntot + nh - 1) / nh;
      if (W.n_chunk > 0) {
        const size_t stride = (size_t)__builtin_amdgcn_readfirstlane(W.spart_stride);
        const int nch = __builtin_amdgcn_readfirstlane(W.n_chunk);
        auto sp0 = W.spart + (DBUF ? (size_t)spec0 * W.spart_buf_stride : (size_t)0);
        for (int k = tid; k < per; k += SOLVE_THREADS) {
          const int i = blockIdx.y * per + k;
          if (i >= ntot) break;
          auto sp = sp0 + i;
          double a = 0;
          constexpr int HB = 36;
          for (int ch = 0; ch < nch; ch += HB) {
            double v[HB];
#pragma unroll
            for (int u = 0; u < HB; ++u) v[u] = (ch + u < nch) ? sp[(size_t)(ch + u) * stride] : 0.0;
#pragma unroll
            for (int u = 0; u < HB; ++u) a += v[u];
          }
          __hip_atomic_store(&W.spart_sum[i], a, __ATOMIC_RELAXED, __HIP_MEMORY_SCOPE_AGENT);
        }
      }
      asm volatile("s_waitcnt vmcnt(0)" ::: "memory");
      __syncthreads();
      if (tid == 0) __hip_atomic_fetch_add(W.sum_sync, 1, __ATOMIC_RELAXED, __HIP_MEMORY_SCOPE_AGENT);
      return;
    }
  }
  const bool helped = !LARGE && gridDim.y > 1;
  __shared__ int s_sum_ready;
  const int t64 = tid - 64;
  const int tl = t64 < 0 ? 0 : t64;
  const int sum_launches = LARGE ? 0 : as_global(W.sum_sync)[1];
  __shared__ double s_Wd[(sizeof(WinPtrs) + 7) / 8];
  static_assert(sizeof(WinPtrs) % 8 == 0, "copied as doubles");
  constexpr int WD_N = (int)(sizeof(WinPtrs) / 8);
  const double wd_v = LARGE ? 0.0 : reinterpret_cast<const double*>(&W)[tl < WD_N ? tl : 0];
  if (LARGE && tid == 0) W.ct_flag[W.ct_nT * (W.ct_nT + 1) / 2 + 1] = 0;
  if (chead.w) {
    if (helped && tid == 64) as_global(W.sum_sync)[1] = sum_launches + ((int)gridDim.y - 1);
    return;
  }
  const OptD& opt = *optp;
  const int D = W.D, Dp = W.Dp;
  const int Dpad = ((D + 5) / 6) * 6, nbk = Dpad / 6;
  typedef typename std::conditional<CHAIN, LChain, typename SolveLayout<LARGE>::type>::type LYT;
  const LYT LY = [&]() {
    if constexpr (CHAIN) return LChain::make(D, Dp);
    else if constexpr (LARGE) return LYT{nbk};
    else return LYT{ldl16_nb(D), D - Dp, D};
  }();
  const int nS = [&]() {
    if constexpr (CHAIN) return LY.total;
    else return LARGE ? nbk * (nbk + 1) / 2 * SBS : ldl16_area_doubles(D);
  }();

  double* S = LARGE ? W.Sg : smem;
  double* s_rhs = LARGE ? smem : smem + nS;
  double* s_g = s_rhs + Dpad;
  double* s_d2 = s_g + Dpad;
  double* s_x = s_d2 + Dpad;
  __shared__ Ctrl c;
  __shared__ int s_accepted, s_was_first, s_fail, s_was_pending;
  __shared__ double s_cost_change, s_old_cost, s_lm_gmax;
  __shared__ int s_coloff[64];
  __shared__ double s_red[SOLVE_THREADS / 64];

#define STAMP(k) do { if (W.prof && tid == 0 && blockIdx.x == 0) W.prof[k] = (double)clock64(); } while (0)
  STAMP(0);
  const double dec_pref = LARGE ? 0.0 : W.dec[tid < DEC_COUNT ? tid : 0];
  const double scale_pref = opt.dogleg ? W.scale_p[tid < D ? tid : 0] : 1.0;
  __shared__ double s_pri[PRI_STAGE * (42 + 9 + 81)];
  __shared__ int s_pricol[PRI_STAGE * (6 + 9)];
  const int n_pri = (!LARGE && W.n_pprior <= PRI_STAGE && W.n_sbprior <= PRI_STAGE) ? PRI_STAGE : 0;
  double pri_a0 = 0, pri_a1 = 0, pri_b = 0, pri_c0 = 0, pri_c1 = 0, pri_c2 = 0;
  int pri_col = -1;
  if (n_pri) {
    const int npp = W.n_pprior, nsp = W.n_sbprior;
    const int l = tid & 63;
    auto pa = W.pp_lin[spec0];
    auto pc = W.sbprior_sqrtinfo;
    pri_a0 = pa[l < npp * 42 ? l : 0];
    pri_a1 = pa[l + 64 < npp * 42 ? l + 64 : 0];
    pri_b = W.sbp_lin[spec0][l < nsp * 9 ? l : 0];
    pri_c0 = pc[l < nsp * 81 ? l : 0];
    pri_c1 = pc[l + 64 < nsp * 81 ? l + 64 : 0];
    pri_c2 = pc[l + 128 < nsp * 81 ? l + 128 : 0];
    pri_col = W.prior_col[l < npp * 6 + nsp * 9 ? l : 0];
  }
  __shared__ double s_pre[PRE_BLOCKS * 16];
  __shared__ int s_preoff[2 * PRE_BLOCKS];
  constexpr bool pre_on = !LARGE;
  double pre_a0 = 0, pre_b0 = 0, pre_a1 = 0, pre_b1 = 0;
  int pre_po = -1, pre_so = -1;
  if constexpr (pre_on) {
    const int np7 = 7 * W.n_pose, ns9 = 9 * W.n_sb;
    const int i0 = 2 * tl, i1 = 2 * tl + 1;
    const int kp0 = i0 < np7 ? i0 : 0, kp1 = i1 < np7 ? i1 : 0;
    const int ks0 = (i0 >= PRE_BLOCKS * 7 && i0 - PRE_BLOCKS * 7 < ns9) ? i0 - PRE_BLOCKS * 7 : 0;
    const int ks1 = (i1 >= PRE_BLOCKS * 7 && i1 - PRE_BLOCKS * 7 < ns9) ? i1 - PRE_BLOCKS * 7 : 0;
    auto pp = W.pose[spec0];
    auto sp = W.sb[spec0];
    pre_a0 = pp[kp0], pre_b0 = sp[ks0], pre_a1 = pp[kp1], pre_b1 = sp[ks1];
    const int to = tl - PRE_BLOCKS * 8;
    pre_po = W.pose_off[(to >= 0 && to < PRE_BLOCKS && to < W.n_pose) ? to : 0];
    pre_so = W.sb_off[(to >= PRE_BLOCKS && to < 2 * PRE_BLOCKS && to - PRE_BLOCKS < W.n_sb) ? to - PRE_BLOCKS : 0];
  }
  constexpr int IMU_NPF = 6, IMU_NL = SOLVE_THREADS - 64;
  const int imu_items = W.n_imu * 512;
  const bool imu_fast = !LARGE && imu_items <= IMU_NPF * IMU_NL && W.n_imu_color < 16;
  const int imu_spec = spec0;
  double imu_v0 = 0, imu_v1 = 0, imu_v2 = 0, imu_v3 = 0, imu_v4 = 0, imu_v5 = 0;
  int imu_w0 = -1, imu_w1 = -1, imu_w2 = -1, imu_w3 = -1, imu_w4 = -1, imu_w5 = -1;
  if (imu_fast && imu_items > 0) {
    auto src = W.imu_lin[imu_spec];
    auto dst = W.imu_fastw;
#define BA_IMU_REQ(j) { const int idx = tl + (j) * IMU_NL; const bool on = t64 >= 0 && idx < imu_items; imu_w##j = dst[on ? idx : 0]; \
                        imu_v##j = src[on ? idx : 0]; }
    BA_IMU_REQ(0) BA_IMU_REQ(1) BA_IMU_REQ(2) BA_IMU_REQ(3) BA_IMU_REQ(4) BA_IMU_REQ(5)
#undef BA_IMU_REQ
  }
  const int goff = (int)(s_g - smem);
  const bool w0pri = !LARGE && n_pri > 0 && (W.n_pprior > 0 || W.n_sbprior > 0);
  static_assert(PRI_STAGE == 2, "the four tasks below");
  double pr_v00 = 0, pr_v01 = 0, pr_v10 = 0, pr_v11 = 0;
  int pr_o00 = -1, pr_o01 = -1, pr_o10 = -1, pr_o11 = -1, pr_d00 = -1, pr_d01 = -1, pr_d10 = -1, pr_d11 = -1;
  auto prior_task = [&](int p, int t, double& val, int& off, int& d2i) {
    if (t < 27) {
      if (p < W.n_pprior) {
        const double* L = s_pri + 42 * p;
        const int* co = s_pricol + 6 * p;
        if (t < 21) {
          int a = 0;
          while ((a + 1) * (a + 2) / 2 <= t) ++a;
          const int b = t - a * (a + 1) / 2;
          const int ra = co[a], rb = co[b];
          if (ra >= 0 && rb >= 0) {
            double sacc = 0;
            for (int k = 0; k < 6; ++k) sacc += L[k * 6 + a] * L[k * 6 + b];
            val = sacc;
            off = LY.at(ra, rb);
            d2i = a == b ? ra : -1;
          }
        } else {
          const int a = t - 21, ra = co[a];
          if (ra >= 0) {
            double sacc = 0;
            for (int k = 0; k < 6; ++k) sacc += L[k * 6 + a] * L[36 + k];
            val = sacc;
            off = goff + ra;
          }
        }
      }
    } else if (t < 81) {
      if (p < W.n_sbprior) {
        const double* Jc = s_pri + PRI_STAGE * 51 + 81 * p;
        const double* r = s_pri + PRI_STAGE * 42 + 9 * p;
        const int* co = s_pricol + PRI_STAGE * 6 + 9 * p;
        if (t < 72) {
          const int e = t - 27;
          int a = 0;
          while ((a + 1) * (a + 2) / 2 <= e) ++a;
          const int b = e - a * (a + 1) / 2;
          const int ra = co[a], rb = co[b];
          if (ra >= 0 && rb >= 0) {
            double sacc = 0;
            for (int k = 0; k < 9; ++k) sacc += Jc[k * 9 + a] * Jc[k * 9 + b];
            val = sacc;
            off = LY.at(ra, rb);
            d2i = a == b ? ra : -1;
          }
        } else {
          const int a = t - 72, ra = co[a];
          if (ra >= 0) {
            double sacc = 0;
            for (int k = 0; k < 9; ++k) sacc -= Jc[k * 9 + a] * r[k];
            val = sacc;
            off = goff + ra;
          }
        }
      }
    }
  };
  auto prior_tasks = [&]() {
    prior_task(0, tid, pr_v00, pr_o00, pr_d00);
    prior_task(0, tid + 64, pr_v01, pr_o01, pr_d01);
    prior_task(1, tid, pr_v10, pr_o10, pr_d10);
    prior_task(1, tid + 64, pr_v11, pr_o11, pr_d11);
  };
  auto prior_apply = [&](double va, int oa, int da, double vb, int ob, int db) {
    const double a0 = oa >= 0 ? smem[oa] : 0.0, a1 = da >= 0 ? s_d2[da] : 0.0;
    const double b0 = ob >= 0 ? smem[ob] : 0.0, b1 = db >= 0 ? s_d2[db] : 0.0;
    if (oa >= 0) smem[oa] = a0 + va;
    if (da >= 0) s_d2[da] = a1 + va;
    if (ob >= 0) smem[ob] = b0 + vb;
    if (db >= 0) s_d2[db] = b1 + vb;
  };
  const int sum_spec = DBUF ? spec0 : 0;
  STAMP(41);
  auto sum_partials = [&](int buf, bool use_sums, const double* pre = nullptr) {
    if constexpr (!LARGE) {
      const int npose_blk = Dp / 6;
      const int nP = npose_blk * (npose_blk + 1) / 2 * 36, ntot = nP + 3 * Dp;
// ... 14 lines not shown
#pragma unroll
            for (int t = 0; t < 3; ++t)
#pragma unroll
              for (int u = 0; u < CB; ++u) v[t][u] = (ch + u < nch && base + t * NL < ntot) ? sp[(size_t)(ch + u) * stride + base + t * NL] : 0.0;
#pragma unroll
            for (int t = 0; t < 3; ++t)
#pragma unroll
              for (int u = 0; u < CB; ++u) a[t] += v[t][u];
          }
        }
#pragma unroll
        for (int t = 0; t < 3; ++t) {
          const int i = base + t * NL;
          if (use_sums) a[t] = i < ntot ? __hip_atomic_load(&ssum[i], __ATOMIC_RELAXED, __HIP_MEMORY_SCOPE_AGENT) : 0.0;
          dst[t] = -1;
          if (i < nP) {
            const int q = i / 36, e = i - 36 * q, ii = e / 6, jj = e - 6 * ii;
            int bi = (int)((sqrtf(8.0f * q + 1.0f) - 1.0f) * 0.5f);
            while ((bi + 1) * (bi + 2) / 2 <= q) ++bi;
            while (bi * (bi + 1) / 2 > q) --bi;
            const int bj = q - bi * (bi + 1) / 2;
            if (bi > bj || ii >= jj) dst[t] = LY.at(6 * bi + ii, 6 * bj + jj);
          }
        }
#pragma unroll
        for (int t = 0; t < 3; ++t) {
          const int i = base + t * NL;
          if (dst[t] >= 0) {
            S[dst[t]] = a[t];
          } else if (i >= nP && i < ntot) {
            const int which = (i - nP) / Dp, j = (i - nP) - which * Dp;
            (which == 0 ? s_rhs : (which == 1 ? s_g : s_d2))[j] = a[t];
          }
        }
      }
    }
  };
  if (tid < 64) {
    double sums[6] = {0, 0, 0, 0, 0, 0};
    Decision d;
    d.accept = 0; d.term = 0;
    double cword = 0;
    if (tid < (int)(sizeof(Ctrl) / 8)) cword = as_global(reinterpret_cast<const double*>(gctrl))[tid];
    double tpart[6] = {0, 0, 0, 0, 0, 0};
    if (chead.y) wave_trial_partials(W, 1 - chead.x, tid, tpart);
    if (tid < (int)(sizeof(Ctrl) / 8)) reinterpret_cast<double*>(&c)[tid] = cword;
    STAMP(42);
    __builtin_amdgcn_fence(__ATOMIC_ACQ_REL, "wavefront");
    asm volatile("" ::: "memory");
    const int pending = c.pending;
    DecisionDL dl;
    dl.accept = 0; dl.term = 0; dl.explicit_next = 0; dl.judged = 0;
    if (pending) {
      __shared__ double s_dec[DEC_COUNT];
      if (tid < DEC_COUNT) s_dec[tid] = dec_pref;
      __builtin_amdgcn_fence(__ATOMIC_ACQ_REL, "wavefront");
      asm volatile("" ::: "memory");
      if (s_dec[DEC_VALID] != 0.0) {
        for (int k = 0; k < 6; ++k) sums[k] = s_dec[DEC_SUMS + k];
        if (opt.dogleg) {
          dl.accept = (int)s_dec[DEC_DL + 0]; dl.term = (int)s_dec[DEC_DL + 1]; dl.explicit_next = (int)s_dec[DEC_DL + 2];
          dl.judged = (int)s_dec[DEC_DL + 3]; dl.invalid_steps = (int)s_dec[DEC_DL + 4]; dl.have_tot = (int)s_dec[DEC_DL + 5];
          dl.radius = s_dec[DEC_DL + 6]; dl.mu = s_dec[DEC_DL + 7]; dl.rho = s_dec[DEC_DL + 8]; dl.model_change = s_dec[DEC_DL + 9];
          dl.tot_C = s_dec[DEC_DL + 10]; dl.tot_E = s_dec[DEC_DL + 11];
        } else {
          d.accept = (int)s_dec[DEC_LM + 0]; d.term = (int)s_dec[DEC_LM + 1]; d.radius = s_dec[DEC_LM + 2];
          d.decrease_factor = s_dec[DEC_LM + 3]; d.rho = s_dec[DEC_LM + 4]; d.model_change = s_dec[DEC_LM + 5];
        }
        if (tid == 0) W.dec[DEC_VALID] = 0.0;
      } else {
        wave_trial_reduce(tpart, sums);
        if (opt.dogleg) decide_dl_inl(&c, &opt, sums, final_only != 0, &dl);
        else decide_inl(&c, &opt, sums, &d);
      }
    }
    if (tid == 0) {
      s_accepted = 0;
      s_was_pending = pending;
      s_was_first = c.first;
      s_cost_change = 0;
      s_old_cost = c.cost;
      s_lm_gmax = 0;
      s_fail = 0;
      if (opt.dogleg) {
        if (pending) {
          c.last_rho = dl.rho;
          c.last_model_change = dl.model_change;
          c.have_tot = dl.have_tot;
          c.tot_C = dl.tot_C;
          c.tot_E = dl.tot_E;
          c.invalid_steps = dl.invalid_steps;
          c.mu = dl.mu;
          c.radius = dl.radius;
          if (dl.accept) {
            s_accepted = 1;
            s_cost_change = c.cost - sums[0];
            c.acc = 1 - c.acc;
            c.cost = sums[0];
            if (!c.first) c.successful++;
            s_lm_gmax = sums[5];
          }
          c.explicit_next = dl.explicit_next ? (dl.judged ? 1 : 2) : 0;
          if (dl.term) c.done = dl.term + 1;
          c.pending = 0;
        } else if (!final_only && c.explicit_next != 2 && c.iter >= c.max_iter) {
          c.done = 6 + 1;
        }
      } else if (pending) {
        c.last_rho = d.rho;
        c.last_model_change = d.model_change;
        if (d.term) {
          c.done = d.term + 1;
          c.radius = d.radius;
          c.decrease_factor = d.decrease_factor;
        } else if (d.accept) {
          s_accepted = 1;
          s_cost_change = c.cost - sums[0];
          c.acc = 1 - c.acc;
          c.cost = sums[0];
          if (!c.first) c.successful++;
          c.radius = d.radius;
          c.decrease_factor = d.decrease_factor;
          s_lm_gmax = sums[5];
        } else {
          c.radius = d.radius;
          c.decrease_factor = d.decrease_factor;
        }
        c.pending = 0;
      }
      if (W.prof && blockIdx.x == 0) W.prof[3] = (double)clock64();
    }
    if (w0pri) {
      __builtin_amdgcn_fence(__ATOMIC_ACQ_REL, "wavefront");
      asm volatile("" ::: "memory");
      const int accn = __builtin_amdgcn_readfirstlane(c.acc);
      const int npp = W.n_pprior, nsp = W.n_sbprior;
      if (accn != spec0) {
        auto pa = W.pp_lin[accn];
        pri_a0 = pa[tid < npp * 42 ? tid : 0];
        pri_a1 = pa[tid + 64 < npp * 42 ? tid + 64 : 0];
        pri_b = W.sbp_lin[accn][tid < nsp * 9 ? tid : 0];
      }
      if (tid < npp * 42) s_pri[tid] = pri_a0;
      if (tid + 64 < npp * 42) s_pri[tid + 64] = pri_a1;
      if (tid < nsp * 9) s_pri[PRI_STAGE * 42 + tid] = pri_b;
      if (tid < nsp * 81) s_pri[PRI_STAGE * 51 + tid] = pri_c0;
      if (tid + 64 < nsp * 81) s_pri[PRI_STAGE * 51 + tid + 64] = pri_c1;
      if (tid + 128 < nsp * 81) s_pri[PRI_STAGE * 51 + tid + 128] = pri_c2;
      if (tid < npp * 6) s_pricol[tid] = pri_col;
      else if (tid < npp * 6 + nsp * 9) s_pricol[PRI_STAGE * 6 + tid - npp * 6] = pri_col;
      __builtin_amdgcn_fence(__ATOMIC_ACQ_REL, "wavefront");
      asm volatile("" ::: "memory");
      prior_tasks();
      if (W.prof && tid == 0 && blockIdx.x == 0) W.prof[44] = (double)clock64();
    }
  } else {
    if constexpr (LARGE) {
      if (W.ct_flag[W.ct_nT * (W.ct_nT + 1) / 2 + 2] == 0)
        for (int i = tid - 64; i < nS; i += SOLVE_THREADS - 64) S[i] = 0.0;
    } else {
      const int npose_blk = Dp / 6;
      const int nP = npose_blk * (npose_blk + 1) / 2 * 36, ntot = nP + 3 * Dp;
      constexpr int NL = SOLVE_THREADS - 64;
      constexpr int PCB = 9;
      const bool early = !helped && W.n_chunk <= PCB && ntot <= 3 * NL;
      double pv0[PCB], pv1[PCB], pv2[PCB];
      if (early) {
        const size_t stride = W.spart_stride;
        const int nch = W.n_chunk;
        auto sp = W.spart + (DBUF ? (size_t)sum_spec * W.spart_buf_stride : (size_t)0);
        const int i0 = tid - 64;
#pragma unroll
        for (int u = 0; u < PCB; ++u) {
          pv0[u] = (u < nch && i0 < ntot) ? sp[(size_t)u * stride + i0] : 0.0;
          pv1[u] = (u < nch && i0 + NL < ntot) ? sp[(size_t)u * stride + i0 + NL] : 0.0;
          pv2[u] = (u < nch && i0 + 2 * NL < ntot) ? sp[(size_t)u * stride + i0 + 2 * NL] : 0.0;
        }
      }
      {
        const L16& PL = [&]() -> const L16& {
          if constexpr (CHAIN) return LY.P;
          else return LY;
        }();
        const int nb16 = PL.nb, nblk16 = L16::blocks(nb16);
        const int Ds = CHAIN ? 0 : D - Dp;
        const int Dz = CHAIN ? Dp : D;
        if constexpr (CHAIN)
          for (int i = LY.oA + tid - 64; i < LY.total; i += NL) S[i] = 0.0;
        const int wv = __builtin_amdgcn_readfirstlane(tid >> 6) - 1, l = tid & 63;
        int I = 0, rem = wv;
        for (int b = wv; b < nblk16; b += SOLVE_THREADS / 64 - 1) {
          while (rem >= nb16 - I) {
            rem -= nb16 - I;
            ++I;
          }
          const int J = I + rem;
          const int cc = 16 * J + (l & 15);
#pragma unroll
          for (int r = 0; r < 4; ++r) {
            const int rr = 16 * I + 4 * r + (l >> 4);
            if (!(rr >= Ds && cc >= rr && cc < Dz)) S[b * 256 + 64 * r + l] = 0.0;
          }
          rem += SOLVE_THREADS / 64 - 1;
        }
      }
      auto stage_stores = [&]() {
        if (t64 < WD_N) s_Wd[t64] = wd_v;
        if (pre_on && t64 < PRE_BLOCKS * 8) {
          const int np7 = 7 * W.n_pose, ns9 = 9 * W.n_sb;
          const int i0 = 2 * t64, i1 = 2 * t64 + 1;
          s_pre[i0] = i0 < PRE_BLOCKS * 7 ? (i0 < np7 ? pre_a0 : 0.0) : (i0 - PRE_BLOCKS * 7 < ns9 ? pre_b0 : 0.0);
          s_pre[i1] = i1 < PRE_BLOCKS * 7 ? (i1 < np7 ? pre_a1 : 0.0) : (i1 - PRE_BLOCKS * 7 < ns9 ? pre_b1 : 0.0);
        } else if (pre_on && t64 < PRE_BLOCKS * 10) {
          const int to = t64 - PRE_BLOCKS * 8;
          s_preoff[to] = to < PRE_BLOCKS ? (to < W.n_pose ? pre_po : -1) : (to - PRE_BLOCKS < W.n_sb ? pre_so : -1);
        }
      };
      const int sum_expected = sum_launches + ((int)gridDim.y - 1);
      if (helped) stage_stores();
      if (helped && tid == 64) {
        as_global(W.sum_sync)[1] = sum_expected;
        int polls = 0;
        while (__hip_atomic_load(W.sum_sync, __ATOMIC_RELAXED, __HIP_MEMORY_SCOPE_AGENT) < sum_expected && polls < opt.helper_polls) {
          __builtin_amdgcn_s_sleep(2);
          ++polls;
        }
        if (polls >= opt.helper_polls) W.sum_sync[2] += 1;
        __hip_atomic_store(&s_sum_ready, (sum_expected << 2) | (polls >= opt.helper_polls ? 2 : 1), __ATOMIC_RELEASE, __HIP_MEMORY_SCOPE_WORKGROUP);
      }
      bool use_sums = false;
      if (helped) {
        int v;
        while (((v = __hip_atomic_load(&s_sum_ready, __ATOMIC_ACQUIRE, __HIP_MEMORY_SCOPE_WORKGROUP)) >> 2) != sum_expected || (v & 3) == 0)
          __builtin_amdgcn_s_sleep(1);
        use_sums = (v & 3) == 1;
      }
      if (early) {
        double pre[3] = {0, 0, 0};
#pragma unroll
        for (int u = 0; u < PCB; ++u) pre[0] += pv0[u];
#pragma unroll
        for (int u = 0; u < PCB; ++u) pre[1] += pv1[u];
#pragma unroll
        for (int u = 0; u < PCB; ++u) pre[2] += pv2[u];
        sum_partials(sum_spec, false, pre);
      } else {
        sum_partials(sum_spec, use_sums);
      }
      if (!helped) stage_stores();
      for (int i = tid - 64; i < 3 * (Dpad - Dp); i += NL) {
        const int which = i / (Dpad - Dp), j = Dp + i - which * (Dpad - Dp);
        (which == 0 ? s_rhs : (which == 1 ? s_g : s_d2))[j] = 0.0;
      }
      for (int i = tid - 64; i < Dpad; i += SOLVE_THREADS - 64) s_x[i] = 0.0;
    }
    if (W.prof && tid == 64 && blockIdx.x == 0) W.prof[4] = (double)clock64();
  }
  if (W.prof && (tid & 63) == 0 && blockIdx.x == 0) W.prof[170 + (tid >> 6)] = (double)clock64();
  __syncthreads();
  if (c.done) {
    if (tid == 0) *gctrl = c;
    return;
  }
  const int acc = __builtin_amdgcn_readfirstlane(c.acc);
  const WinPtrs& Wl = *[&]() -> const WinPtrs* {
    if constexpr (LARGE) return &W;
    else return reinterpret_cast<const WinPtrs*>(s_Wd);
  }();
  if (LARGE && tid == 0) Wl.ct_flag[Wl.ct_nT * (Wl.ct_nT + 1) / 2 + 2] = 0;

  STAMP(1);
  if constexpr (LARGE) {
    const int npose_blk = Dp / 6;
    const int nP = npose_blk * (npose_blk + 1) / 2 * 36;
    const size_t stride = Wl.spart_stride;
    const int nch = Wl.n_chunk;
    const double* sp = Wl.spart;
    for (int i = tid; i < 3 * Dpad; i += SOLVE_THREADS) {
      const int which = i / Dpad, j = i - which * Dpad;
      double a = 0;
      if (j < Dp) {
        for (int ch = 0; ch < nch; ch += 8) {
          double v[8];
#pragma unroll
          for (int u = 0; u < 8; ++u) v[u] = (ch + u < nch) ? sp[(size_t)(ch + u) * stride + nP + which * Dp + j] : 0.0;
#pragma unroll
          for (int u = 0; u < 8; ++u) a += v[u];
        }
      }
      (which == 0 ? s_rhs : (which == 1 ? s_g : s_d2))[j] = a;
    }
    for (int i = tid; i < Dpad; i += SOLVE_THREADS) s_x[i] = 0.0;
    __syncthreads();
  }
  STAMP(2);
  const bool rejected = s_was_pending && !s_accepted;
  if (imu_fast) {
    if (imu_items > 0) {
// ... 126 lines not shown
        if constexpr (!LARGE) S[LY.at(D, i)] = rh;
      } else {
        if constexpr (LARGE) S[LY.at(i, i)] = 1.0;
        s_rhs[i] = 0.0;
      }
    }
  };
  if (final_only) {
    conv_partial();
    __syncthreads();
    if (tid == 0) {
      double gm = s_lm_gmax;
      for (int i = 0; i < SOLVE_THREADS / 64; ++i) gm = fmax(gm, s_red[i]);
      if (s_accepted) {
        c.grad_max = gm;
        if (s_was_first) {
          c.initial_cost = c.cost;
          c.abs_grad_tol = opt.dogleg ? opt.gradient_tolerance : opt.gradient_tolerance * fmax(gm, 2.220446049250313e-16);
        }
        if (opt.gradient_tolerance > 0 && gm <= c.abs_grad_tol) {
          c.done = 2 + 1;
        } else if (!opt.dogleg && !s_was_first && opt.function_tolerance > 0 &&
                   fabs(s_cost_change) < opt.function_tolerance * s_old_cost) {
          c.done = 1 + 1;
        }
        c.first = 0;
      }
    }
    __syncthreads();
    if (Wl.grad)
      for (int i = tid; i < D; i += SOLVE_THREADS) Wl.grad[i] = s_g[i];
    if (final_only == 2) {
      for (int i = tid; i < D; i += SOLVE_THREADS) Wl.rhs[i] = s_rhs[i] - s_g[i];
      if constexpr (LARGE) {
        if (tid == 0) {
          *gctrl = c;
          Wl.ct_flag[Wl.ct_nT * (Wl.ct_nT + 1) / 2 + 1] = 1;
        }
        return;
      }
      for (int k = tid; k < D * D; k += SOLVE_THREADS) {
        const int i = k / D, j = k - i * D;
        Wl.S[k] = (i >= j) ? S[LY.at(i, j)] : S[LY.at(j, i)];
      }
    }
    if (tid == 0) *gctrl = c;
    return;
  }
  conv_partial();
  damping();
  if (Wl.grad)
    for (int i = tid; i < D; i += SOLVE_THREADS) Wl.grad[i] = s_g[i];
  if (tid == 0 && opt.dogleg && c.mu >= DL_MAX_MU) s_fail = 1;
  __syncthreads();
  {
    const int verdict = conv_decide();
    if (tid == 0 && s_accepted) {
      double gm = s_lm_gmax;
      for (int i = 0; i < SOLVE_THREADS / 64; ++i) gm = fmax(gm, s_red[i]);
      c.grad_max = gm;
      if (s_was_first) {
        c.initial_cost = c.cost;
        c.abs_grad_tol = opt.dogleg ? opt.gradient_tolerance : opt.gradient_tolerance * fmax(gm, 2.220446049250313e-16);
      }
      if (verdict & 3) c.done = verdict & 3;
      c.first = 0;
    }
    if (verdict & 3) {
      if (tid == 0) *gctrl = c;
      return;
    }
  }
  if (Wl.S) {
    for (int k = tid; k < D * D; k += SOLVE_THREADS) {
      const int i = k / D, j = k - i * D;
      Wl.S[k] = (i >= j) ? S[LY.at(i, j)] : S[LY.at(j, i)];
    }
    for (int i = tid; i < D; i += SOLVE_THREADS) {
      Wl.rhs[i] = s_rhs[i];
      Wl.Dp2[i] = s_d2[i];
    }
  }
  STAMP(6);
  if constexpr (!LARGE) {
    if (opt.dogleg && c.explicit_next) {
      __shared__ double s_dl[2];
      __shared__ double s_sc5[5][SOLVE_THREADS / 64];
      const double mu = c.mu;
      for (int i = tid; i < Dpad; i += SOLVE_THREADS) {
        s_x[i] = i < D ? s_g[i] / s_d2[i] : 0.0;
        s_rhs[i] = i < D ? Wl.step[i] : 0.0;
      }
      __syncthreads();
      double q1 = 0, q2 = 0, Ap = 0, Al = 0, Bl = 0;
      for (int k = tid; k < D * D; k += SOLVE_THREADS) {
        const int i = k / D, j = k - i * D;
        const double v = (i >= j) ? S[LY.at(i, j)] : S[LY.at(j, i)];
        q1 += v * s_x[i] * s_x[j];
      }
      for (int i = tid; i < D; i += SOLVE_THREADS) {
        q2 += s_d2[i] * s_x[i] * s_x[i];
        Ap += s_g[i] * s_x[i];
      }
      dl_landmark_sums(Wl, acc, s_x, mu, opt, tid, &Al, &Bl);
      q1 = wave_sum_full(q1);
      q2 = wave_sum_full(q2);
      Ap = wave_sum_full(Ap);
      Al = wave_sum_full(Al);
      Bl = wave_sum_full(Bl);
      if ((tid & 63) == 0) {
        s_sc5[0][tid >> 6] = q1;
        s_sc5[1][tid >> 6] = q2;
        s_sc5[2][tid >> 6] = Ap;
        s_sc5[3][tid >> 6] = Al;
        s_sc5[4][tid >> 6] = Bl;
      }
      __syncthreads();
      if (tid == 0) {
        double a[5] = {0, 0, 0, 0, 0};
        for (int k = 0; k < 5; ++k)
          for (int i = 0; i < SOLVE_THREADS / 64; ++i) a[k] += s_sc5[k][i];
        double cA, beta, dln, model;
        dogleg_coefficients(a[2] + a[3], (a[0] - mu * a[1]) + a[4], c.tot_C, c.tot_E, mu, c.radius, &cA, &beta, &dln, &model);
        s_dl[0] = cA;
        s_dl[1] = beta;
        c.cA = cA;
        c.beta = beta;
        c.dl_norm = dln;
        c.pend_model = model;
        c.tot_A = a[2] + a[3];
      }
      __syncthreads();
      {
        const double cA = s_dl[0], beta = s_dl[1];
        for (int i = tid; i < Dpad; i += SOLVE_THREADS) s_x[i] = -cA * s_x[i] + beta * s_rhs[i];
      }
      __syncthreads();
      double s2 = 0, x2 = 0;
      trial_states(Wl, acc, s_x, tid, true, &s2, &x2, pre_on ? s_pre : nullptr, pre_on ? s_preoff : nullptr);
      s2 = wave_sum_full(s2);
      x2 = wave_sum_full(x2);
      if ((tid & 63) == 0) {
        s_sc5[0][tid >> 6] = s2;
        s_sc5[1][tid >> 6] = x2;
      }
      __syncthreads();
      if (tid == 0) {
        double a0 = 0, a1 = 0;
        for (int i = 0; i < SOLVE_THREADS / 64; ++i) {
          a0 += s_sc5[0][i];
          a1 += s_sc5[1][i];
        }
        c.step2_p = a0;
        c.x2_p = a1;
        c.tr_kind = 1;
        c.spec_discard = c.explicit_next == 2;
        if (c.explicit_next == 1) c.iter++;
        c.explicit_next = 0;
        c.lambda = mu;
        c.pending = 1;
        *gctrl = c;
      }
      return;
    }
  }
  if constexpr (LARGE) {
    const int nT = Wl.ct_nT, ntile = nT * (nT + 1) / 2;
    for (int i = tid; i < nT * CT_TB; i += SOLVE_THREADS) {
      Wl.ct_rhs[i] = i < Dpad ? s_rhs[i] : 0.0;
      Wl.ct_g[i] = i < D ? s_g[i] : 0.0;
      Wl.ct_d2[i] = i < D ? s_d2[i] : 0.0;
    }
    for (int i = tid; i < ntile + 1; i += SOLVE_THREADS) Wl.ct_flag[i] = 0;
    if (tid == 0) Wl.ct_flag[ntile + 3] = 0;
    for (int i = tid; i < 2 * nT; i += SOLVE_THREADS) Wl.ct_flag[ntile + 4 + i] = 0;
    for (int i = tid; i < nT * CT_TB; i += SOLVE_THREADS)
      reinterpret_cast<unsigned long long*>(Wl.ct_x)[i] = CT_X_SENTINEL;
    __syncthreads();
    if (tid == 0) {
      *gctrl = c;
      Wl.ct_flag[ntile + 1] = (opt.dogleg && c.explicit_next) ? 2 : 1;
    }
    return;
  }
  if constexpr (!LARGE) {
    STAMP(10);
    long long* const stamps = (W.prof && blockIdx.x == 0) ? reinterpret_cast<long long*>(W.prof + 64) : nullptr;
    if constexpr (CHAIN) chain_solve<SOLVE_THREADS / 64>(S, LY, tid, s_x, &s_fail, stamps, W.ldl_comp);
    else ldl16_solve<SOLVE_THREADS / 64>(S, D, tid, s_x, &s_fail, stamps, D - Dp, W.ldl_comp);
  }
  STAMP(7);
  if (s_fail) {
    if (tid == 0) {
      c.chol_fail++;
      c.pending = 0;
      if (opt.dogleg) {
        solve_failed_dl(&c, opt);
      } else {
        c.iter++;
        c.radius = c.radius / c.decrease_factor;
        c.decrease_factor *= 2.0;
        if (c.radius < opt.min_radius) c.done = 5 + 1;
      }
      *gctrl = c;
    }
    return;
  }
  STAMP(8);

  {
    double gd = 0, ddd = 0, s2 = 0;
    for (int i = tid; i < D; i += SOLVE_THREADS) {
      const double x = s_x[i];
      Wl.step[i] = x;
      gd += s_g[i] * x;
      ddd += s_d2[i] * x * x;
      s2 += x * x;
    }
    STAMP(31);
    double x2 = 0, s2a = 0;
    trial_states(Wl, acc, s_x, tid, opt.dogleg != 0, &s2a, &x2, pre_on ? s_pre : nullptr, pre_on ? s_preoff : nullptr);
    STAMP(32);
    if (opt.dogleg) s2 = s2a;
    __shared__ double s_sc[4][SOLVE_THREADS / 64];
    gd = wave_sum_full(gd);
    ddd = wave_sum_full(ddd);
    s2 = wave_sum_full(s2);
    x2 = wave_sum_full(x2);
    if ((tid & 63) == 0) {
      s_sc[0][tid >> 6] = gd;
      s_sc[1][tid >> 6] = ddd;
      s_sc[2][tid >> 6] = s2;
      s_sc[3][tid >> 6] = x2;
    }
    __syncthreads();
    STAMP(33);
    if (tid == 0) {
      double a0 = 0, a1 = 0, a2 = 0, a3 = 0;
      for (int i = 0; i < SOLVE_THREADS / 64; ++i) {
        a0 += s_sc[0][i];
        a1 += s_sc[1][i];
        a2 += s_sc[2][i];
        a3 += s_sc[3][i];
      }
      c.gd_p = a0;
      c.ddd_p = a1;
      c.step2_p = a2;
      c.x2_p = a3;
      c.lambda = lambda;
      c.tr_kind = 0;
      c.spec_discard = 0;
      c.explicit_next = 0;
      c.have_tot = 0;
      c.iter++;
      c.pending = 1;
      *gctrl = c;
    }
  }
  STAMP(9);
#undef STAMP
}

template <bool CHAIN>
__global__ __launch_bounds__(SOLVE_THREADS) void reduced_solve_kernel(const double* __restrict__ Sd, const double* __restrict__ rhs, int D, int Dp,
                                                                      unsigned comp_mask, double* __restrict__ x, long long* __restrict__ ticks,
                                                                      int* __restrict__ info, int repeats, double* __restrict__ dump) {
  extern __shared__ __attribute__((aligned(16))) double smem[];
  const int tid = threadIdx.x;
  typedef typename std::conditional<CHAIN, LChain, L16>::type LYT;
  const LYT LY = [&]() {
    if constexpr (CHAIN) return LChain::make(D, Dp);
    else return L16{ldl16_nb(D), D - Dp, D};
  }();
  const int nS = CHAIN ? LChain::make(D, Dp).total : ldl16_area_doubles(D);
  double* s_x = smem + nS;
  __shared__ int s_fail;
  long long total = 0;
  for (int rep = 0; rep < repeats; ++rep) {
    for (int i = tid; i < nS; i += SOLVE_THREADS) smem[i] = 0.0;
    if (tid == 0) s_fail = 0;
    __syncthreads();
    for (int k = tid; k < D * D; k += SOLVE_THREADS) {
      const int i = k / D, j = k - i * D;
      if (i >= j) {
        const double v = Sd[k];
        if (v != 0.0 || i == j) smem[LY.at(i, j)] = v;
      }
    }
    for (int i = tid; i < D; i += SOLVE_THREADS) smem[LY.at(D, i)] = rhs[i];
    __syncthreads();
    const long long t0 = clock64();
    if constexpr (CHAIN) chain_solve<SOLVE_THREADS / 64>(smem, LY, tid, s_x, &s_fail, nullptr, comp_mask);
    else ldl16_solve<SOLVE_THREADS / 64>(smem, D, tid, s_x, &s_fail, nullptr, D - Dp, comp_mask);
    total += clock64() - t0;
    __syncthreads();
  }
  for (int i = tid; i < D; i += SOLVE_THREADS) x[i] = s_x[i];
  if (dump)
    for (int i = tid; i < nS; i += SOLVE_THREADS) dump[i] = smem[i];
  if (tid == 0) {
    ticks[0] = total / repeats;
    info[0] = s_fail;
  }
}

__global__ __launch_bounds__(CT_THREADS) void large_export_kernel(const WinPtrs* __restrict__ wins) {
  const WinPtrs& W = wins[blockIdx.y];
  const int nT = W.ct_nT, ntile = nT * (nT + 1) / 2;
  if (nT == 0 || (int)blockIdx.x >= ntile) return;
  if (W.ct_flag[ntile + 1] == 0) return;
  const int t = blockIdx.x;
  int ti = 0;
  while ((ti + 1) * (ti + 2) / 2 <= t) ++ti;
  const int tj = t - ti * (ti + 1) / 2;
  const int D = W.D, Dp = W.Dp, Dpad = ((D + 5) / 6) * 6;
  const SLayout LY{Dpad / 6};
  const int nch = W.n_chunk;
  const size_t stride = W.spart_stride;
  for (int r = blockIdx.z * CT_THREADS + threadIdx.x; r < CT_TILE; r += gridDim.z * CT_THREADS) {
    int gi = CT_TB * ti + r / CT_TB, gj = CT_TB * tj + r % CT_TB;
    const int oi = gi, oj = gj;
    double v;
    if (ti == tj && oi < oj && !W.S) {
      v = 0.0;
    } else if (gi < Dpad && gj < Dpad) {
      const bool owner = gi >= gj;
      if (!owner) {
        const int tmp = gi;
        gi = gj;
        gj = tmp;
      }
      const int at = LY.at(gi, gj);
      v = W.Sg[at];
      {
        const int2 sr = W.imu_rev[at];
        const double* lin = W.imu_lin[W.ctrl->acc];
        if (sr.x >= 0) v += lin[sr.x];
        if (sr.y >= 0) v += lin[sr.y];
      }
// ... 261 lines not shown
```

okvis_amd/csrc/capi_launch.inc:

```
namespace {

size_t lin_smem(bool ext, bool f32 = false) {
  const int d = f32 ? (ext ? LinCfg<true, float>::SMEM_DOUBLES : LinCfg<false, float>::SMEM_DOUBLES)
                    : (ext ? LinCfg<true, double>::SMEM_DOUBLES : LinCfg<false, double>::SMEM_DOUBLES);
  return (size_t)d * sizeof(double);
}
size_t solve_smem(int Dpad, bool large) {
  return ((large ? 0 : (size_t)ldl16_area_doubles(Dpad)) + 4 * (size_t)Dpad) * sizeof(double) + 16;
}
size_t solve_smem_chain(int chain_doubles, int Dpad) { return ((size_t)chain_doubles + 4 * (size_t)Dpad) * sizeof(double) + 16; }
int lin2_step_doubles(int max_Dp, bool fuse, bool f32) {
  const int aux = fuse ? (f32 ? Lin2Cfg<float, true>::MIN_STEP_DOUBLES : Lin2Cfg<double, true>::MIN_STEP_DOUBLES) : Lin2Cfg<double, false>::MIN_STEP_DOUBLES;
  return ((max_Dp + 1) / 2) * 2 + 8 + aux;
}
size_t lin2_smem(int max_Dp, bool fuse, bool f32, bool two_rounds = false) {
  const int fixed = two_rounds ? (f32 ? Lin2Cfg<float, false, 14>::FIXED_DOUBLES : Lin2Cfg<double, false, 14>::FIXED_DOUBLES)
                    : f32 ? (fuse ? Lin2Cfg<float, true>::FIXED_DOUBLES : Lin2Cfg<float, false>::FIXED_DOUBLES)
                          : (fuse ? Lin2Cfg<double, true>::FIXED_DOUBLES : Lin2Cfg<double, false>::FIXED_DOUBLES);
  return (size_t)(fixed + lin2_step_doubles(max_Dp, fuse, f32)) * sizeof(double);
}
size_t small_smem() { return (size_t)std::max<int>(std::max<int>(ImuLds::TOTAL, EvalLds::TOTAL), 2 * MAX_MARG_DIM) * sizeof(double); }

size_t small_eval_smem() { return (size_t)std::max<int>(EvalLds::TOTAL, 2 * MAX_MARG_DIM) * sizeof(double); }

int sch2_serial_nlb(int trows) {
  const int nlb = sch2_nlb(trows, 5120);
  return nlb < 12 ? sch2_nlb(trows, 9216) : nlb;
}

std::vector<std::pair<const void*, size_t>> plan_kernels() {
  auto f = [](auto k) { return reinterpret_cast<const void*>(k); };
  const size_t dense = std::max(solve_smem(((MAX_D_LDS + 5) / 6) * 6, false), (size_t)SOLVE_LDS_LIMIT), chain = SOLVE_LDS_LIMIT_CHAIN;
  size_t wide = 0;
  for (int t = 1; t <= TILE_DIM; ++t) wide = std::max(wide, (size_t)sch2_tile_doubles(t, sch2_serial_nlb(t)) * sizeof(double));
  const size_t d = std::max(lin2_smem(MAX_D, true, false), small_smem()), s = std::max(lin2_smem(MAX_D, true, true), small_smem());
  const size_t ef = std::max(lin_smem(true, true), small_smem()), ed = std::max(lin_smem(true), small_smem());
  const size_t pf = std::max(lin_smem(false, true), small_smem()), pd = std::max(lin_smem(false), small_smem());
  return {{f(&solve_kernel<false, true, true>), chain}, {f(&solve_kernel<false, false, true>), chain},
          {f(&solve_kernel<false, true>), dense}, {f(&solve_kernel<false, false>), dense},
          {f(&schur_ride_kernel<3>), std::max(wide, small_eval_smem())}, {f(&schur_mfma_kernel<3>), wide}, {f(&schur_mfma_kernel<9>), wide},
          {f(&schur_kernel), 2 * SCHUR_LM_BATCH * TILE_DIM * 3 * sizeof(double)},
          {f(&solve_kernel<true, false>), solve_smem(((MAX_D + 5) / 6) * 6, true)},
          {f(&small_kernel), small_smem()}, {f(&small_prepare_kernel), small_smem()},
          {f(&linearize2_kernel<float, true, false>), s}, {f(&linearize2_kernel<float, false, false, 4, 14>), s},
          {f(&linearize2_kernel<float, false, false, 3>), s}, {f(&linearize2_kernel<double, true, false>), d},
          {f(&linearize2_kernel<double, false, false, 4, 14>), d}, {f(&linearize2_kernel<double, false, false, 3>), d},
          {f(&linearize2_kernel<float, true, true>), s}, {f(&linearize2_kernel<float, false, true>), s},
          {f(&linearize2_kernel<double, true, true>), d}, {f(&linearize2_kernel<double, false, true>), d},
          {f(&linearize_kernel<true, float, true>), ef}, {f(&linearize_kernel<true, float, false>), ef},
          {f(&linearize_kernel<true, double, true>), ed}, {f(&linearize_kernel<true, double, false>), ed},
          {f(&linearize_kernel<false, float, true>), pf}, {f(&linearize_kernel<false, float, false>), pf},
          {f(&linearize_kernel<false, double, true>), pd}, {f(&linearize_kernel<false, double, false>), pd},
          {f(&schur_ride_kernel<3, true>), std::max(wide, small_eval_smem())}, {f(&schur_mfma_kernel<3, true>), wide},
          {f(&linearize2_rec_kernel<double, 3>), d}, {f(&linearize2_rec_kernel<double, 4, 14>), d},
          {f(&linearize2_rec_kernel<float, 3>), s}, {f(&linearize2_rec_kernel<float, 4, 14>), s}};
}

using LinFn = decltype(&linearize_kernel<false, double, false>);
using Lin2Fn = decltype(&linearize2_kernel<double, false, true>);
using SolveFn = decltype(&solve_kernel<false, false>);
const LinFn LIN[8] = {&linearize_kernel<false, double, false>, &linearize_kernel<false, double, true>, &linearize_kernel<false, float, false>,
                      &linearize_kernel<false, float, true>,   &linearize_kernel<true, double, false>,  &linearize_kernel<true, double, true>,
                      &linearize_kernel<true, float, false>,   &linearize_kernel<true, float, true>};
enum { LIN2_FUSED, LIN2_FUSED_SMALL, LIN2_SMALL, LIN2_OCC3, LIN2_OCC4 };
const Lin2Fn LIN2[10] = {&linearize2_kernel<double, true, false>, &linearize2_kernel<double, true, true>, &linearize2_kernel<double, false, true>,
                         &linearize2_kernel<double, false, false, 3>, &linearize2_kernel<double, false, false, 4, 14>,
                         &linearize2_kernel<float, true, false>, &linearize2_kernel<float, true, true>, &linearize2_kernel<float, false, true>,
                         &linearize2_kernel<float, false, false, 3>, &linearize2_kernel<float, false, false, 4, 14>};
using Lin2RecFn = decltype(&linearize2_rec_kernel<double, 3>);
const Lin2RecFn LIN2R[4] = {&linearize2_rec_kernel<double, 3>, &linearize2_rec_kernel<double, 4, 14>, &linearize2_rec_kernel<float, 3>,
                            &linearize2_rec_kernel<float, 4, 14>};
enum { SOLVE_NONE, SOLVE_DENSE, SOLVE_DENSE_DBUF, SOLVE_CHAIN, SOLVE_CHAIN_DBUF, SOLVE_TILED };
const SolveFn SOLVE[6] = {nullptr, &solve_kernel<false, false>, &solve_kernel<false, true>, &solve_kernel<false, false, true>,
                          &solve_kernel<false, true, true>, &solve_kernel<true, false>};
enum { SCHUR_NONE, SCHUR_VALU, SCHUR_MFMA3, SCHUR_MFMA9, SCHUR_RIDE3, SCHUR_MFMA3_SERIAL, SCHUR_RIDE3_SERIAL };
enum { SMALL_NONE, SMALL_ALL, SMALL_PREPARE };
LaunchPlan make_plan(const BatchLayout& L, const BatchMax& M, const okvis_ba_options& o, int n_windows) {
  LaunchPlan p;
  const bool f32 = o.fp32_linearize != 0;
  p.fused = M.group_chunks && f32 == L.fp32 && decision_free(o);
  p.nodec = M.spec_schur && !p.fused && decision_free(o);
  p.lin2 = L.lin2, p.split_small = L.split_small, p.graph = o.use_graph != 0;
  p.n_small = M.imu + 1;
  p.trows = std::min(TILE_DIM, M.Dp);
  if (M.schur_blocks > 0 && !p.fused) {
    const bool small_tiles = schur_small_tiles(M.Dp);
    if (!M.any_ext && schur_mfma_allowed(o) && (small_tiles || (o.tuning.flags & OKVIS_BA_TUNE_SCHUR_MFMA_LARGE))) {
      p.nlb = sch2_serial_nlb(p.trows);
      const bool serial = !small_tiles || M.rec_stride == 0 || (o.tuning.flags & OKVIS_BA_TUNE_SCHUR_SERIAL_BATCHES);
      p.rec_stride = serial ? 0 : M.rec_stride;
      if (!serial) p.nlb = SCH2_STAGE_LM;
      const int sm = (serial ? sch2_tile_doubles(p.trows, p.nlb) : sch2_ring_doubles(p.trows)) * (int)sizeof(double);
      p.rides = small_tiles && p.nodec && L.split_small && !(o.tuning.flags & OKVIS_BA_TUNE_NO_SMALL_RIDE);
      if (p.rides) p.schur = Launch{serial ? SCHUR_RIDE3_SERIAL : SCHUR_RIDE3, p.n_small + M.schur_blocks, std::max(sm, (int)small_eval_smem())};
      else p.schur = Launch{!small_tiles ? SCHUR_MFMA9 : serial ? SCHUR_MFMA3_SERIAL : SCHUR_MFMA3, M.schur_blocks, sm};
    } else {
      p.schur = Launch{SCHUR_VALU, M.schur_blocks, (int)(2 * SCHUR_LM_BATCH * p.trows * 3 * sizeof(double))};
    }
  }
  if (M.Dpad_small > 0)
    p.solve = Launch{(M.chain ? SOLVE_CHAIN : SOLVE_DENSE) + (M.group_chunks || M.spec_schur), 0,
                     (int)(M.chain ? solve_smem_chain(M.chain_doubles, M.Dpad_small) : solve_smem(M.Dpad_small, false))};
  if (M.Dpad_large > 0) {
    p.tiled = Launch{SOLVE_TILED, 0, (int)solve_smem(M.Dpad_large, true)};
    p.nT = (M.Dpad_large + CT_TB - 1) / CT_TB;
  }
  const Launch small{SMALL_ALL, p.n_small, (int)small_smem()};
  if (L.lin2) {
    const int t = f32 ? 5 : 0, smem2 = (int)lin2_smem(M.Dp, p.fused, f32);
    p.sd = lin2_step_doubles(M.Dp, p.fused, f32);
    if (L.split_small) {
      p.small_init = small;
      p.small_iter = !p.rides ? small : M.imu > 0 ? Launch{SMALL_PREPARE, M.imu, (int)small_smem()} : Launch{};
      const int occ = o.tuning.lin2_occupancy > 0 ? o.tuning.lin2_occupancy : 4;
      const bool two_rounds = !p.fused && occ >= 4;
      p.lin = Launch{t + (p.fused ? LIN2_FUSED : occ >= 4 ? LIN2_OCC4 : LIN2_OCC3), M.group,
                     two_rounds ? (int)lin2_smem(M.Dp, false, f32, true) : smem2};
      if (!p.fused && M.grec_stride > 0 && !(o.tuning.flags & OKVIS_BA_TUNE_LIN_NO_RECORDS)) p.grec_stride = M.grec_stride;
    } else {
      p.lin = Launch{t + (p.fused ? LIN2_FUSED_SMALL : LIN2_SMALL), p.n_small + M.group, std::max(smem2, (int)small_smem())};
      p.lin_n_small = p.n_small;
    }
  } else {
    p.lin = Launch{4 * M.any_ext + 2 * f32 + p.fused, p.n_small + M.group, (int)std::max(lin_smem(M.any_ext, f32), small_smem())};
    p.lin_n_small = p.n_small;
  }
  if (M.imu > 0 && o.strategy == OKVIS_BA_STRATEGY_DOGLEG && !o.gauss_newton) p.take_back = Launch{1, M.imu, 0};
  p.budget = o.strategy == OKVIS_BA_STRATEGY_DOGLEG;
  int nsub = o.n_streams > 0 ? o.n_streams : (n_windows >= 128 ? 2 : (n_windows >= 56 ? 3 : (n_windows >= 8 ? 2 : 1)));
  nsub = std::max(1, std::min(nsub, n_windows));
  auto extent = [](int w0, int nw) { return Extent{w0, nw, nw <= SOLVE_HELPED_MAX_WINDOWS ? SOLVE_HELPERS : 0}; };
  for (int k = 0; k < nsub; ++k) {
    const int w0 = (int)((int64_t)n_windows * k / nsub), w1 = (int)((int64_t)n_windows * (k + 1) / nsub);
    p.subs.push_back(extent(w0, w1 - w0));
  }
  p.whole = extent(0, n_windows);
  p.one_helpers = extent(0, 1).helpers;
  return p;
}

__global__ void begin_kernel(const WinPtrs* wins, const int* accs, double initial_radius) {
  const WinPtrs& W = wins[blockIdx.x];
  const int acc = accs[blockIdx.x], tr = 1 - acc, tid = threadIdx.x;
  for (int i = tid; i < 7 * W.n_pose; i += blockDim.x) W.pose[tr][i] = W.pose[acc][i];
  for (int i = tid; i < 9 * W.n_sb; i += blockDim.x) W.sb[tr][i] = W.sb[acc][i];
  for (int i = tid; i < 4 * W.n_lm; i += blockDim.x) W.lm[tr][i] = W.lm[acc][i];
  if (tid == 0) {
    Ctrl c;
    for (size_t k = 0; k < sizeof(Ctrl) / 8; ++k) reinterpret_cast<double*>(&c)[k] = 0.0;
    c.acc = acc;
    c.pending = 1;
    c.first = 1;
    c.radius = initial_radius;
    c.decrease_factor = 2.0;
    c.lambda = 1.0 / initial_radius;
    c.mu = DL_MIN_MU;
    *W.ctrl = c;
  }
}
__global__ void gather_ctrl_kernel(const WinPtrs* wins, Ctrl* out, int n) {
  const int w = blockIdx.x * (blockDim.x / 64) + threadIdx.x / 64, lane = threadIdx.x & 63;
  if (w < n && lane < (int)(sizeof(Ctrl) / 8))
    reinterpret_cast<double*>(out + w)[lane] = reinterpret_cast<const double*>(wins[w].ctrl)[lane];
}

__global__ void delay_kernel(long long ticks) {
  const long long t0 = wall_clock64();
  while (wall_clock64() - t0 < ticks) __builtin_amdgcn_s_sleep(32);
}

struct Sub { hipStream_t st; int w0, nw, helpers; };
Sub sub(hipStream_t st, const Extent& e) { return Sub{st, e.w0, e.nw, e.helpers}; }
Sub whole(okvis_ba_solver* s) { return sub(s->stream, s->plan.whole); }

hipError_t launch_schur(okvis_ba_solver* s, Sub b, int final_call = 0) {
  const LaunchPlan& p = s->plan;
  const dim3 grid((unsigned)p.schur.gx, (unsigned)b.nw), blk(SCHUR_THREADS);
  const WinPtrs* wins = s->d_wins + b.w0;
  const CtrlSlot* ctrls = s->d_ctrl + b.w0;
  const int* recs = p.rec_stride ? s->d_recs + (size_t)b.w0 * p.rec_stride * SCHUR_REC_INTS : nullptr;
  switch (p.schur.k) {
    case SCHUR_NONE: return hipSuccess;
    case SCHUR_VALU: hipLaunchKernelGGL(schur_kernel, grid, blk, p.schur.lds, b.st, wins, s->d_opt, p.trows, final_call); break;
    case SCHUR_MFMA3: hipLaunchKernelGGL(schur_mfma_kernel<3>, grid, blk, p.schur.lds, b.st, wins, s->d_opt, p.trows, final_call, p.nlb, ctrls, p.nodec, recs, p.rec_stride); break;
    case SCHUR_MFMA9: hipLaunchKernelGGL(schur_mfma_kernel<9>, grid, blk, p.schur.lds, b.st, wins, s->d_opt, p.trows, final_call, p.nlb, ctrls, p.nodec, recs, p.rec_stride); break;
    case SCHUR_RIDE3: hipLaunchKernelGGL(schur_ride_kernel<3>, grid, blk, p.schur.lds, b.st, wins, s->d_opt, p.trows, final_call, p.nlb, ctrls, p.nodec, p.n_small, recs, p.rec_stride); break;
    case SCHUR_MFMA3_SERIAL: hipLaunchKernelGGL((schur_mfma_kernel<3, true>), grid, blk, p.schur.lds, b.st, wins, s->d_opt, p.trows, final_call, p.nlb, ctrls, p.nodec, recs, p.rec_stride); break;
    case SCHUR_RIDE3_SERIAL: hipLaunchKernelGGL((schur_ride_kernel<3, true>), grid, blk, p.schur.lds, b.st, wins, s->d_opt, p.trows, final_call, p.nlb, ctrls, p.nodec, p.n_small, recs, p.rec_stride); break;
  }
  return hipGetLastError();
}
void launch_solve_kernel(okvis_ba_solver* s, const Launch& l, dim3 grid, hipStream_t st, const WinPtrs* wins, int final_only, CtrlSlot* ctrls) {
  const SolveFn fn = SOLVE[l.k];
  hipLaunchKernelGGL(fn, grid, dim3(SOLVE_THREADS), l.lds, st, wins, s->d_opt, final_only, ctrls);
}
hipError_t launch_solve(okvis_ba_solver* s, Sub b, int final_only) {
  const LaunchPlan& p = s->plan;
  if (p.solve.k) launch_solve_kernel(s, p.solve, dim3((unsigned)b.nw, 1 + b.helpers), b.st, s->d_wins + b.w0, final_only, s->d_ctrl + b.w0);
  if (p.tiled.k) {
    launch_solve_kernel(s, p.tiled, dim3((unsigned)b.nw), b.st, s->d_wins + b.w0, final_only, s->d_ctrl + b.w0);
    if (!final_only) {
      const int nT = p.nT;
      hipLaunchKernelGGL(large_export_kernel, dim3(nT * (nT + 1) / 2, (unsigned)b.nw, CT_TILE / CT_THREADS), dim3(CT_THREADS), 0, b.st,
                         s->d_wins + b.w0);
      hipLaunchKernelGGL(chol_tiles_window_kernel, dim3(nT * (nT + 1) / 2 + nT, (unsigned)b.nw), dim3(CT_THREADS), CT_SMEM_DOUBLES * 8,
                         b.st, s->d_wins + b.w0);
      hipLaunchKernelGGL(solve_large_tail_kernel, dim3((unsigned)b.nw), dim3(SOLVE_THREADS), 0, b.st, s->d_wins + b.w0, s->d_opt);
    }
  }
  return hipGetLastError();
}
hipError_t launch_lin(okvis_ba_solver* s, Sub b, int init) {
  const LaunchPlan& p = s->plan;
  const WinPtrs* wins = s->d_wins + b.w0;
  const Launch& f = init ? p.small_init : p.small_iter;
  if (f.k == SMALL_ALL) hipLaunchKernelGGL(small_kernel, dim3((unsigned)f.gx, (unsigned)b.nw), dim3(LIN_THREADS), f.lds, b.st, wins, init);
  if (f.k == SMALL_PREPARE) hipLaunchKernelGGL(small_prepare_kernel, dim3((unsigned)f.gx, (unsigned)b.nw), dim3(LIN_THREADS), f.lds, b.st, wins);
  const dim3 grid((unsigned)p.lin.gx, (unsigned)b.nw);
  if (p.lin2 && p.grec_stride) {
    const Lin2RecFn fn = LIN2R[2 * (p.lin.k >= 5) + (p.lin.k % 5 - LIN2_OCC3)];
    hipLaunchKernelGGL(fn, grid, dim3(LIN_THREADS), p.lin.lds, b.st, wins, s->d_opt, init, p.sd, s->d_ctrl + b.w0,
                       s->d_grecs + (size_t)b.w0 * p.grec_stride * LIN_REC_INTS, p.grec_stride);
  } else if (p.lin2) {
    const Lin2Fn fn = LIN2[p.lin.k];
    hipLaunchKernelGGL(fn, grid, dim3(LIN_THREADS), p.lin.lds, b.st, wins, s->d_opt, init, p.lin_n_small, p.sd);
  } else {
    const LinFn fn = LIN[p.lin.k];
    hipLaunchKernelGGL(fn, grid, dim3(LIN_THREADS), p.lin.lds, b.st, wins, s->d_opt, init, p.lin_n_small);
  }
  return hipGetLastError();
}
hipError_t launch_imu_take_back(okvis_ba_solver* s, int w0, int nw) {
  if (!s->plan.take_back.k) return hipSuccess;
  hipLaunchKernelGGL(imu_take_back_kernel, dim3((unsigned)s->plan.take_back.gx, (unsigned)nw), dim3(64), 0, s->stream, s->d_wins + w0);
  return hipGetLastError();
}
hipError_t launch_iteration(okvis_ba_solver* s, Sub b) {
  hipError_t e;
  if ((e = launch_schur(s, b)) != hipSuccess) return e;
  if ((e = launch_solve(s, b, 0)) != hipSuccess) return e;
  return launch_lin(s, b, 0);
}
hipError_t launch_budget(okvis_ba_solver* s, Sub b, int n) {
  if (!s->plan.budget || n <= 0) return hipSuccess;
  hipLaunchKernelGGL(add_budget_kernel, dim3((unsigned)b.nw), dim3(64), 0, b.st, s->d_wins + b.w0, n);
  return hipGetLastError();
}
hipError_t launch_chain(okvis_ba_solver* s, Sub b, int n, int budget) {
  hipError_t e = launch_budget(s, b, budget);
  for (int i = 0; i < n && e == hipSuccess; ++i) e = launch_iteration(s, b);
  return e;
}
hipError_t launch_iterations_forked(okvis_ba_solver* s, int n, int budget = -1) {
  const int nsub = (int)s->sub_streams.size();
  if (budget < 0) budget = n;
  if (nsub <= 1) return launch_chain(s, whole(s), n, budget);
  hipError_t e = hipEventRecord(s->ev_fork, s->stream);
  for (int k = 0; k < nsub && e == hipSuccess; ++k) {
    e = hipStreamWaitEvent(s->sub_streams[k], s->ev_fork, 0);
    if (e == hipSuccess) e = launch_chain(s, sub(s->sub_streams[k], s->plan.subs[k]), n, budget);
    if (e == hipSuccess) e = hipEventRecord(s->sub_events[k], s->sub_streams[k]);
    if (e == hipSuccess) e = hipStreamWaitEvent(s->stream, s->sub_events[k], 0);
  }
  return e;
}

int refresh_acc(okvis_ba_solver* s, int w) {
  if (s->acc_fresh) return OKVIS_BA_OK;
  int acc = 0;
  HIP_TRY(hipMemcpyAsync(&acc, &s->wins[w].ptrs.ctrl->acc, sizeof(int), hipMemcpyDeviceToHost, s->stream));
  HIP_TRY(hipStreamSynchronize(s->stream));
  s->wins[w].acc = acc & 1;
  return OKVIS_BA_OK;
}

hipError_t reserve_ctrl_stage(okvis_ba_solver* s, size_t n_windows) {
  const size_t bytes = std::max(sizeof(Ctrl), sizeof(int)) * n_windows;
  if (bytes <= s->ctrl_stage_bytes) return hipSuccess;
  if (s->h_ctrl_stage) (void)hipHostFree(s->h_ctrl_stage);
  if (s->d_ctrl_stage) (void)hipFree(s->d_ctrl_stage);
  s->h_ctrl_stage = s->d_ctrl_stage = nullptr;
  s->ctrl_stage_bytes = 0;
  hipError_t e = hipHostMalloc((void**)&s->h_ctrl_stage, bytes, hipHostMallocDefault);
  if (e == hipSuccess) e = hipMalloc((void**)&s->d_ctrl_stage, bytes);
  if (e == hipSuccess) s->ctrl_stage_bytes = bytes;
  return e;
}

int fetch_ctrl(okvis_ba_solver* s, std::vector<Ctrl>& out) {
  const size_t n = s->wins.size();
  out.resize(n);
  HIP_TRY(reserve_ctrl_stage(s, n));
  hipLaunchKernelGGL(gather_ctrl_kernel, dim3((unsigned)((n + 3) / 4)), dim3(256), 0, s->stream, s->d_wins, reinterpret_cast<Ctrl*>(s->d_ctrl_stage), (int)n);
  HIP_TRY(hipGetLastError());
  HIP_TRY(hipMemcpyAsync(s->h_ctrl_stage, s->d_ctrl_stage, sizeof(Ctrl) * n, hipMemcpyDeviceToHost, s->stream));
  HIP_TRY(hipStreamSynchronize(s->stream));
  std::memcpy(out.data(), s->h_ctrl_stage, sizeof(Ctrl) * n);
  return OKVIS_BA_OK;
}

}
```

okvis_amd/csrc/capi_solver.inc:

```
namespace {

#define HIP_TRY(expr)                                              \
  do {                                                             \
    hipError_t _e = (expr);                                        \
    if (_e != hipSuccess) {                                        \
      s->last_hip_error = (int)_e;                                 \
      return OKVIS_BA_HIP_ERROR_BASE + (int)_e;                    \
    }                                                              \
  } while (0)

struct HostWin {
  int n_pose = 0, n_sb = 0, n_lm = 0, n_obs = 0, n_imu = 0, D = 0, Dp = 0, n_pair = 0, n_group = 0, n_chunk = 0;
  std::vector<int> pair_lm, pair_block;
  std::vector<int> pose_off, sb_off;
  int marg_dim = 0;
  bool h0_on_device = false;
  bool group_chunks = false;
  bool spec_ok = false;
  bool chain = false;
  WinPtrs ptrs;
  int acc = 0;
  int64_t bytes_lin = 0, bytes_schur = 0, bytes_solve = 0, bytes_small = 0;
};

constexpr size_t ARENA_ZFLAG = size_t(1) << 62;
template <class T>
struct StageAlloc {
  typedef T value_type;
  StageAlloc() = default;
  template <class U>
  StageAlloc(const StageAlloc<U>&) {}
  T* allocate(size_t n) {
    const size_t bytes = n * sizeof(T) + 16;
    void* p = nullptr;
    unsigned char tag = 1;
    if (hipHostMalloc(&p, bytes, hipHostMallocDefault) != hipSuccess || !p) {
      (void)hipGetLastError();
      p = std::malloc(bytes);
      tag = 0;
      if (!p) throw std::bad_alloc();
    }
    static_cast<unsigned char*>(p)[0] = tag;
    return reinterpret_cast<T*>(static_cast<unsigned char*>(p) + 16);
  }
  void deallocate(T* q, size_t) {
    unsigned char* p = reinterpret_cast<unsigned char*>(q) - 16;
    if (p[0]) (void)hipHostFree(p); else std::free(p);
  }
  template <class U>
  bool operator==(const StageAlloc<U>&) const { return true; }
  template <class U>
  bool operator!=(const StageAlloc<U>&) const { return false; }
};
typedef std::vector<unsigned char, StageAlloc<unsigned char>> StageVec;
inline bool stage_is_pinned(const StageVec& v) { return !v.empty() && (v.data() - 16)[0] == 1; }
struct Arena {
  StageVec host;
  size_t size = 0;
  size_t zsize = 0;
  size_t alloc(size_t bytes) {
    size_t off = (size + 255) & ~size_t(255);
    size = off + bytes;
    return off;
  }
  size_t zalloc(size_t bytes) {
    size_t off = (zsize + 255) & ~size_t(255);
    zsize = off + bytes;
    return off | ARENA_ZFLAG;
  }
  size_t data_bytes() const { return (size + 255) & ~size_t(255); }
  size_t total() const { return data_bytes() + zsize; }
};

struct BatchLayout {
  bool lin2 = false, chain = false;
  int chain_min = 1;
  bool fuse = false, spec = false;
  int schur_lm = 0, group_lm = 0;
  bool split_small = false;
  bool fp32 = false;
};
struct BatchMax {
  int group = 0, imu = 0, schur_blocks = 0, lm = 0, Dp = 0, chunks = 0;
  int Dpad_small = 0, Dpad_large = 0, chain_doubles = 0;
  bool any_ext = false, chain = false;
  bool group_chunks = false;
  bool spec_schur = false;
  int rec_stride = 0;
  int grec_stride = 0;
};
struct Launch {
  int k = 0, gx = 0, lds = 0;
};
struct Extent {
  int w0 = 0, nw = 0, helpers = 0;
  bool operator==(const Extent& o) const { return w0 == o.w0 && nw == o.nw && helpers == o.helpers; }
};
struct PlanFixed {
  int lin2 = 0, split_small = 0, fused = 0, nodec = 0, rides = 0, graph = 0;
  Launch schur; int trows = 0, nlb = 0, n_small = 0, rec_stride = 0;
  Launch solve, tiled; int nT = 0;
  Launch small_init, small_iter, lin; int lin_n_small = 0, sd = 0;
  int grec_stride = 0;
  Launch take_back; int budget = 0;
  Extent whole; int one_helpers = 0;
};
struct LaunchPlan : PlanFixed {
  std::vector<Extent> subs;
  bool operator==(const LaunchPlan& o) const {
    return std::memcmp(static_cast<const PlanFixed*>(this), static_cast<const PlanFixed*>(&o), sizeof(PlanFixed)) == 0 && subs == o.subs;
  }
};

}

struct okvis_ba_solver {
  int device = 0;
  hipStream_t stream = nullptr;
  std::vector<hipStream_t> sub_streams;
  std::vector<hipEvent_t> sub_events;
  hipEvent_t ev0 = nullptr, ev1 = nullptr, ev_fork = nullptr;
  okvis_ba_options opt;
  OptD* d_opt = nullptr;
  unsigned char* d_arena = nullptr;
  size_t arena_bytes = 0, arena_capacity = 0, wins_capacity = 0;
  WinPtrs* d_wins = nullptr;
  CtrlSlot* d_ctrl = nullptr;
  const int* d_recs = nullptr;
  const int* d_grecs = nullptr;
  StageVec stage_dl;
  StageVec stage, stage_small;
  std::vector<HostWin> wins;
  bool uploaded = false, begun = false;
  BatchLayout layout;
  BatchMax max;
  LaunchPlan plan;
  LaunchPlan graph_plan;
  std::vector<const void*> graph_addr;
  unsigned char* h_ctrl_stage = nullptr;
  unsigned char* d_ctrl_stage = nullptr;
  size_t ctrl_stage_bytes = 0;
  bool patchable = false;
  std::vector<WindowStore> mirrors;
  WindowStore mirror_edit;
  long marg_tiles_fallbacks = 0;
  bool evaluated = false;
  bool mirror_fresh = false;
  bool res_staged = false;
  StageVec stage_res;
  StageVec stage_marg;
  StageVec stage_marg_vals;
  hipEvent_t ev_marg_vals = nullptr;
  struct MargPending {
    bool active = false;
    bool batch = false;
    struct Item {
      int w = 0, na = 0;
      size_t nn = 0, n1 = 0, out_bytes = 0;
      size_t at = 0;
      std::vector<int> bt, bi, bo;
    };
    std::vector<Item> items;
  } marg_pending;
  StageVec stage_pre;
  unsigned char* d_pre = nullptr;
  bool acc_fresh = false;
  long long stagger_ticks = 0;
  bool skip_topup = false;
  long long slots = 0;
  std::map<int, hipGraphExec_t> graphs;
  std::map<std::pair<int, int>, hipGraphExec_t> sub_graphs;
  float last_iterate_ms = 0.f;
  int last_hip_error = 0;
  unsigned char* marg_scratch = nullptr;
  hipEvent_t ev_cov[3] = {nullptr, nullptr, nullptr};
  hipEvent_t ev_lmcov[4] = {nullptr, nullptr, nullptr, nullptr};
  hipEvent_t ev_pred[4] = {nullptr, nullptr, nullptr, nullptr};
  size_t marg_scratch_bytes = 0;
};

namespace {

size_t solve_smem_chain(int chain_doubles, int Dpad);

constexpr int FUSED_MAX_WINDOWS = 48;
int fused_max_windows(const okvis_ba_options& o) {
  return o.tuning.fused_max_windows > 0 ? o.tuning.fused_max_windows : o.tuning.fused_max_windows < 0 ? 0 : FUSED_MAX_WINDOWS;
}
inline bool decision_free(const okvis_ba_options& o) { return o.strategy == OKVIS_BA_STRATEGY_DOGLEG || o.gauss_newton; }
inline bool schur_mfma_allowed(const okvis_ba_options& o) { return !(o.tuning.flags & OKVIS_BA_TUNE_SCHUR_VALU); }
inline bool schur_small_tiles(int Dp) { return std::min(TILE_DIM, Dp) + 1 <= SCH2_MAXT_SMALL_ROWS; }
struct DebugWord {
  bool build = false, upload = false, marg = false;
  std::string arena;
  DebugWord() {
    const char* e = std::getenv("OKVIS_BA_DEBUG");
    if (!e) return;
    std::string w(e);
    size_t at = 0;
    while (at <= w.size()) {
      size_t c = w.find(',', at);
      if (c == std::string::npos) c = w.size();
      const std::string tok = w.substr(at, c - at);
      if (tok == "build") build = true;
      else if (tok == "upload") upload = true;
      else if (tok == "marg") marg = true;
      else if (tok.rfind("arena=", 0) == 0) arena = tok.substr(6);
      at = c + 1;
    }
  }
};
const DebugWord& debug_word() {
  static const DebugWord w;
  return w;
}
constexpr size_t OPT_PAD = (sizeof(OptD) + 255) & ~size_t(255);
constexpr size_t ctrl_off(size_t n) { return (OPT_PAD + sizeof(WinPtrs) * n + 255) & ~size_t(255); }
constexpr size_t records_bytes(size_t n) { return ctrl_off(n) + sizeof(CtrlSlot) * n; }
constexpr int SMALL_BATCH_WINDOWS = 40;

OptD make_optd(const okvis_ba_options& o, int n_windows) {
  OptD d;
  d.initial_radius = o.initial_radius;
  d.max_radius = o.max_radius;
  d.min_radius = o.min_radius;
  d.min_lm_diag2 = o.min_lm_diagonal;
  d.max_lm_diag2 = o.max_lm_diagonal;
  d.min_relative_decrease = o.min_relative_decrease;
  d.function_tolerance = o.function_tolerance;
  d.gradient_tolerance = o.gradient_tolerance;
  d.parameter_tolerance = o.parameter_tolerance;
  d.gauss_newton = o.gauss_newton;
  d.marg_mode = 0;
  d.dogleg = o.strategy == OKVIS_BA_STRATEGY_DOGLEG;
  d.jacobi_scaling = o.jacobi_scaling != 0;
  d.max_invalid = o.max_consecutive_invalid_steps > 0 ? o.max_consecutive_invalid_steps : 5;
  d.helper_polls = (o.reserved0 & 16) ? 0 : 1 << 22;
  return d;
}

void destroy_graphs(okvis_ba_solver* s) {
  for (auto& kv : s->graphs) (void)hipGraphExecDestroy(kv.second);
  s->graphs.clear();
  for (auto& kv : s->sub_graphs) (void)hipGraphExecDestroy(kv.second);
  s->sub_graphs.clear();
}
void keep_graphs(okvis_ba_solver* s) {
  std::vector<const void*> addr = {s->d_wins, s->d_opt, s->d_ctrl, s->d_recs, s->d_grecs};
  for (auto st : s->sub_streams) addr.push_back(st);
  if (s->plan == s->graph_plan && addr == s->graph_addr) return;
  destroy_graphs(s);
  s->graph_plan = s->plan;
  s->graph_addr.swap(addr);
}
// ... 3 lines not shown
```

okvis_amd/solver.py:

```python
from __future__ import annotations

import ctypes as C
from typing import Sequence

import numpy as np

from . import _lib
from .window import LimitsC, OptionsC, SummaryC, Window, WindowC, default_options

ARR = dict(POSE=0, SB=1, LM=2, OBS_RESIDUAL=3, LM_V=4, LM_B=5, LM_HQ=6, PAIR_W=7, REDUCED_S=8,
           REDUCED_RHS=9, STEP=10, LM_QUALITY=11, GRADIENT=12, IMU_RESIDUAL=13, HPP=14, DAMPING=15, IMU_SB_REF=16, IMU_LIN=17, PROF=99, IMU_REDO_COUNT=98, CTRL=97, SLOTS=96, GROUP_RECS=95)
_dp = C.POINTER(C.c_double)


def limits() -> dict:
    lim = LimitsC()
    _lib.lib().okvis_ba_get_limits(C.byref(lim))
    return {n: getattr(lim, n) for n, _ in lim._fields_}


def check_window(window: Window, options: OptionsC | None = None) -> dict:
    window.validate()
    wc, keep = window.as_c()
    st = (C.c_int64 * 8)()
    _lib.check(_lib.lib().okvis_ba_check_window(C.byref(wc), C.byref(options) if options is not None else None, st),
               "check_window")
    del keep
    return dict(D=st[0], Dp=st[1], n_pair=st[2], n_group=st[3], n_chunk=st[4], n_task=st[5], gpart=st[6],
                arena_bytes=st[7])


INDEX_LISTS = ("groups", "lm_obs_begin", "lm_pair_begin", "pair_lm", "pair_block", "pair_off", "pair_role", "lm_piece_begin",
               "pair_piece", "pair_list_begin", "pair_list", "tasks", "task_list", "chunks", "chunk_diag_begin", "chunk_diag_out",
               "chunk_desc", "piece_path", "ldl_comp", "chain", "chunk_recs", "group_recs")


def index_lists(window: Window, options: OptionsC | None = None, n_windows: int = 1) -> dict:
    wc, keep = window.as_c()
    L = _lib.lib()
    po = C.byref(options) if options is not None else None
    out = {}
    for which, name in enumerate(INDEX_LISTS):
        n = C.c_int64()
        rc = L.okvis_ba_check_window_lists(C.byref(wc), po, n_windows, which, None, 0, C.byref(n))
        if rc != 0 and not (rc == -1 and n.value > 0):
            _lib.check(rc, "check_window_lists")
        a = np.zeros(max(n.value, 1), np.int32)
        if n.value:
            _lib.check(L.okvis_ba_check_window_lists(C.byref(wc), po, n_windows, which, a.ctypes.data_as(C.POINTER(C.c_int32)), n.value,
                                                     C.byref(n)), "check_window_lists")
        out[name] = a[:n.value]
    del keep
    out["groups"] = out["groups"].reshape(-1, 16)
    out["tasks"] = out["tasks"].reshape(-1, 6)
    out["chunks"] = out["chunks"].reshape(-1, 2)
    out["chunk_recs"] = out["chunk_recs"].reshape(-1, 128)
    out["group_recs"] = out["group_recs"].reshape(-1, 32)
    out["piece_path"] = int(out["piece_path"][0])
    out["ldl_comp"] = int(out["ldl_comp"][0]) & 0xFFFFFFFF
    out["chain"] = int(out["chain"][0])
    return out


class WindowStore:

    def __init__(self, window: Window):
        self._L = _lib.lib()
        self._h = C.c_void_p()
        wc, keep = window.as_c()
        _lib.check(self._L.okvis_ba_store_create(C.byref(wc), C.byref(self._h)), "store_create")
        del keep

    def patch(self, patch) -> int:
        pc, keep = patch.as_c()
        rc = self._L.okvis_ba_store_patch(self._h, C.byref(pc))
        del keep
        return rc

    def view(self) -> Window:
        from .window import window_from_c
        wc = WindowC()
        _lib.check(self._L.okvis_ba_store_view(self._h, C.byref(wc)), "store_view")
        return window_from_c(wc)

    def close(self):
        if getattr(self, "_h", None) is not None and self._h:
            self._L.okvis_ba_store_destroy(self._h)
            self._h = None

    def __del__(self):
        try:
            self.close()
        except Exception:
            pass


class WindowBatch:

    def __init__(self, windows: Sequence[Window], device: int = 0, options: OptionsC | None = None, patchable: bool = False):
        self._L = _lib.lib()
        self._h = C.c_void_p()
        _lib.check(self._L.okvis_ba_create(C.byref(self._h), int(device)), "create")
        self.options = options or default_options()
        _lib.check(self._L.okvis_ba_set_options(self._h, C.byref(self.options)), "set_options")
        if patchable:
            _lib.check(self._L.okvis_ba_set_patchable(self._h, 1), "set_patchable")
        self.upload(windows)

    def patch(self, w: int, patch):
        pc, keep = patch.as_c()
        _lib.check(self._L.okvis_ba_patch_window(self._h, int(w), C.byref(pc)), "patch_window")
        del keep
        self.windows[w] = self.patched_view(w)

    def patched_view(self, w: int) -> Window:
        from .window import window_from_c
        wc = WindowC()
# ... 234 lines not shown
            err = _lib.BackendError(st, "predicted_measurement")
            err.results = res
            raise err
        return res

    def last_predicted_measurement_ms(self) -> dict:
        a, k, q = C.c_float(), C.c_float(), C.c_float()
        _lib.check(self._L.okvis_ba_last_predicted_measurement_ms(self._h, C.byref(a), C.byref(k), C.byref(q)), "last_predicted_measurement_ms")
        return dict(assembly=a.value, inverse=k.value, query=q.value)

    def synchronize(self):
        _lib.check(self._L.okvis_ba_synchronize(self._h), "synchronize")

    def get_state(self, w: int = 0):
        W = self.windows[w]
        pose, sb, lm = np.zeros((W.n_pose, 7)), np.zeros((W.n_sb, 9)), np.zeros((W.n_lm, 4))
        _lib.check(self._L.okvis_ba_get_state(self._h, w, pose.ctypes.data_as(_dp), sb.ctypes.data_as(_dp),
                                              lm.ctypes.data_as(_dp)), "get_state")
        return pose, sb, lm

    def fetch_results(self, w: int = 0):
        W = self.windows[w]
        pose, sb, lm = np.zeros((W.n_pose, 7)), np.zeros((W.n_sb, 9)), np.zeros((W.n_lm, 4))
        q, ref = np.zeros(W.n_lm), np.zeros((W.n_imu, 9))
        _lib.check(self._L.okvis_ba_fetch_results(self._h, w, pose.ctypes.data_as(_dp), sb.ctypes.data_as(_dp), lm.ctypes.data_as(_dp),
                                                  q.ctypes.data_as(_dp), ref.ctypes.data_as(_dp)), "fetch_results")
        return dict(pose=pose, sb=sb, lm=lm, quality=q, imu_sb_ref=ref)

    def fetch_imu_caches(self, w: int = 0):
        from .window import IMU_CACHE_DOUBLES
        out = np.zeros((self.windows[w].n_imu, IMU_CACHE_DOUBLES))
        _lib.check(self._L.okvis_ba_fetch_imu_caches(self._h, w, out.ctypes.data_as(_dp)), "fetch_imu_caches")
        return out

    def set_state(self, w: int, pose=None, sb=None, lm=None):
        def p(a):
            return None if a is None else np.ascontiguousarray(a, np.float64)
        pose, sb, lm = p(pose), p(sb), p(lm)
        _lib.check(self._L.okvis_ba_set_state(
            self._h, w, None if pose is None else pose.ctypes.data_as(_dp),
            None if sb is None else sb.ctypes.data_as(_dp), None if lm is None else lm.ctypes.data_as(_dp)), "set_state")

    def array(self, name: str, w: int = 0) -> np.ndarray:
        n = C.c_int64()
        _lib.check(self._L.okvis_ba_array_size(self._h, w, ARR[name], C.byref(n)), f"array_size {name}")
        out = np.zeros(max(n.value, 0))
        _lib.check(self._L.okvis_ba_download(self._h, w, ARR[name], out.ctypes.data_as(_dp), n.value), f"download {name}")
        return out

    def reduced_dim(self, w: int = 0) -> int:
        d = C.c_int32()
        _lib.check(self._L.okvis_ba_reduced_dim(self._h, w, C.byref(d)))
        return d.value

    def pairs(self, w: int = 0):
        n = C.c_int32()
        _lib.check(self._L.okvis_ba_pair_count(self._h, w, C.byref(n)))
        a, b = np.zeros(n.value, np.int32), np.zeros(n.value, np.int32)
        ip = C.POINTER(C.c_int32)
        _lib.check(self._L.okvis_ba_pairs(self._h, w, a.ctypes.data_as(ip), b.ctypes.data_as(ip)))
        return a, b

    def last_iterate_ms(self) -> float:
        t = C.c_float()
        _lib.check(self._L.okvis_ba_last_iterate_ms(self._h, C.byref(t)))
        return t.value

    def profile_iterations(self, n: int):
        ms = (C.c_float * 4)()
        _lib.check(self._L.okvis_ba_profile_iterations(self._h, int(n), ms))
        return dict(schur=ms[0], solve=ms[1], small=ms[2], linearize=ms[3])

    def profile_launches(self, n: int):
        ms = (C.c_float * (4 * int(n)))()
        _lib.check(self._L.okvis_ba_profile_launches(self._h, int(n), ms))
        a = np.array(ms[:], dtype=np.float64).reshape(int(n), 4)
        return dict(schur=a[:, 0], solve=a[:, 1], linearize=a[:, 2] + a[:, 3])

    def helper_timeouts(self) -> int:
        n = C.c_int64()
        _lib.check(self._L.okvis_ba_helper_timeouts(self._h, C.byref(n)))
        return n.value

    ROUTE = ("windows", "fused", "decision_free_schur", "piece_path", "split_small", "sub_batches", "sub_batch_max_windows",
             "schur_kernel", "solve_dbuf", "solve_tiled", "solve_helpers", "graph", "max_chunks", "slots", "solve_mode", "small_rides",
             "lin_records")

    def launch_route(self) -> dict:
        r = (C.c_int32 * len(self.ROUTE))()
        _lib.check(self._L.okvis_ba_launch_route(self._h, r), "launch_route")
        return {n: int(r[i]) for i, n in enumerate(self.ROUTE)}

    def algorithmic_bytes(self):
        v = [C.c_int64() for _ in range(4)]
        _lib.check(self._L.okvis_ba_algorithmic_bytes(self._h, *[C.byref(x) for x in v]))
        return dict(linearize=v[0].value, schur=v[1].value, solve=v[2].value, small=v[3].value)
```

okvis_amd/window.py:

```python
from __future__ import annotations

import ctypes as C
from dataclasses import dataclass, field

import numpy as np

DIST_NONE, DIST_RADTAN, DIST_EQUIDISTANT, DIST_RADTAN8 = 0, 1, 2, 3
BLOCK_POSE, BLOCK_SPEEDBIAS = 0, 1

IMU_CACHE_DOUBLES = 290
_dp = C.POINTER(C.c_double)
_ip = C.POINTER(C.c_int32)
_lp = C.POINTER(C.c_int64)
_bp = C.POINTER(C.c_uint8)


class ImuParamsC(C.Structure):
    _fields_ = [(n, C.c_double) for n in
                ("sigma_g_c", "sigma_a_c", "sigma_gw_c", "sigma_aw_c", "g", "g_max", "a_max")]


class WindowC(C.Structure):
    _fields_ = [
        ("n_pose", C.c_int32), ("pose", _dp), ("pose_fixed", _bp),
        ("n_sb", C.c_int32), ("sb", _dp), ("sb_fixed", _bp),
        ("n_lm", C.c_int32), ("lm", _dp),
        ("n_cam", C.c_int32), ("cam_intr", _dp), ("cam_model", _ip),
        ("n_obs", C.c_int32), ("obs_lm", _ip), ("obs_pose", _ip), ("obs_ext", _ip), ("obs_cam", _ip),
        ("obs_uv", _dp), ("obs_sqrtw", _dp), ("cauchy_b", C.c_double),
        ("n_imu", C.c_int32), ("imu_pose0", _ip), ("imu_sb0", _ip), ("imu_pose1", _ip), ("imu_sb1", _ip),
        ("imu_t0", _lp), ("imu_t1", _lp), ("imu_s_begin", _ip), ("imu_s_count", _ip),
        ("n_imu_samples", C.c_int32), ("imu_s_t", _lp), ("imu_s_gyr", _dp), ("imu_s_acc", _dp),
        ("imu_params", ImuParamsC),
        ("n_pprior", C.c_int32), ("pprior_pose", _ip), ("pprior_meas", _dp), ("pprior_sqrtinfo", _dp),
        ("n_sbprior", C.c_int32), ("sbprior_sb", _ip), ("sbprior_meas", _dp), ("sbprior_sqrtinfo", _dp),
        ("n_relpose", C.c_int32), ("rel_pose0", _ip), ("rel_pose1", _ip), ("rel_sqrtinfo", _dp),
        ("marg_dim", C.c_int32), ("marg_nblocks", C.c_int32), ("marg_block_type", _ip),
        ("marg_block_idx", _ip), ("marg_block_off", _ip), ("marg_J", _dp), ("marg_e0", _dp),
        ("marg_lin", _dp),
        ("imu_sb_ref", _dp), ("imu_sb_ref_valid", _bp), ("imu_cache", _dp),
    ]


TUNE_SCHUR_DECIDES, TUNE_SCHUR_VALU, TUNE_SCHUR_MFMA_LARGE, TUNE_NO_LDL_COMP, TUNE_LDL_COMP_ALL = 0x1, 0x2, 0x4, 0x8, 0x10
TUNE_H0_ON_HOST, TUNE_NO_EARLY_PREINTEGRATION, TUNE_NO_MARG_TILES, TUNE_NO_SMALL_RIDE = 0x20, 0x40, 0x80, 0x100
TUNE_SCHUR_SERIAL_BATCHES, TUNE_LIN_NO_RECORDS = 0x200, 0x400
SOLVE_AUTO, SOLVE_DENSE, SOLVE_CHAIN = 0, 1, 2


class TuningC(C.Structure):
    _fields_ = [
        ("flags", C.c_uint32), ("fused_max_windows", C.c_int32), ("group_lm", C.c_int32), ("group_work", C.c_int32),
        ("split_small_min", C.c_int32), ("lin2_occupancy", C.c_int32), ("stagger_us", C.c_int32), ("solve_mode", C.c_int32),
    ]


class OptionsC(C.Structure):
    _fields_ = [
        ("initial_radius", C.c_double), ("max_radius", C.c_double), ("min_radius", C.c_double),
        ("min_lm_diagonal", C.c_double), ("max_lm_diagonal", C.c_double),
        ("min_relative_decrease", C.c_double), ("function_tolerance", C.c_double),
        ("gradient_tolerance", C.c_double), ("parameter_tolerance", C.c_double),
        ("use_graph", C.c_int32), ("schur_lm_per_block", C.c_int32),
        ("debug_arrays", C.c_int32), ("gauss_newton", C.c_int32),
        ("n_streams", C.c_int32), ("fp32_linearize", C.c_int32),
        ("strategy", C.c_int32), ("jacobi_scaling", C.c_int32), ("max_consecutive_invalid_steps", C.c_int32),
        ("reserved0", C.c_int32), ("tuning", TuningC),
    ]


class SummaryC(C.Structure):
    _fields_ = [
        ("initial_cost", C.c_double), ("final_cost", C.c_double), ("iterations", C.c_int32),
        ("successful_steps", C.c_int32), ("termination", C.c_int32), ("reserved", C.c_int32),
        ("final_radius", C.c_double), ("gradient_max_norm", C.c_double),
    ]

    def as_dict(self):
        return {n: getattr(self, n) for n, _ in self._fields_ if n != "reserved"}


class LimitsC(C.Structure):
    _fields_ = [("max_obs_per_lm", C.c_int32), ("max_reduced_dim", C.c_int32),
                ("max_marg_dim", C.c_int32), ("max_imu_samples_per_factor", C.c_int32)]


class MargSpecC(C.Structure):
    _fields_ = [("pose_marg", _bp), ("sb_marg", _bp), ("prior_dim", C.c_int32), ("prior_nblocks", C.c_int32),
                ("prior_block_type", _ip), ("prior_block_idx", _ip), ("prior_block_off", _ip),
                ("prior_H", _dp), ("prior_b0", _dp)]


class MargResultC(C.Structure):
    _fields_ = [("capacity_dim", C.c_int32), ("capacity_blocks", C.c_int32), ("dim", C.c_int32),
                ("nblocks", C.c_int32), ("rank", C.c_int32), ("block_type", _ip), ("block_idx", _ip),
                ("block_off", _ip), ("H", _dp), ("b0", _dp), ("J", _dp), ("e0", _dp), ("sweeps", C.c_int32 * 2)]


class CovSpecC(C.Structure):
    _fields_ = [("n_blocks", C.c_int32), ("block_type", _ip), ("block_idx", _ip)]


class CovResultC(C.Structure):
    _fields_ = [("capacity", C.c_int32), ("dim", C.c_int32), ("info", C.c_int32), ("min_pivot", C.c_double),
                ("cov", _dp), ("S0", _dp)]


class LmcovSpecC(C.Structure):
    _fields_ = [("n_lm", C.c_int32), ("lm_idx", _ip)]


class LmcovResultC(C.Structure):
    _fields_ = [("capacity", C.c_int32), ("n", C.c_int32), ("info", C.c_int32), ("min_pivot", C.c_double),
                ("cov", _dp), ("flags", _bp), ("S0", _dp), ("Spp", _dp), ("V", _dp), ("W", _dp)]


class PredSpecC(C.Structure):
    _fields_ = [("n_q", C.c_int32), ("q_lm", _ip), ("q_pose", _ip), ("q_ext", _ip), ("q_cam", _ip)]


class PredResultC(C.Structure):
    _fields_ = [("capacity", C.c_int32), ("n", C.c_int32), ("info", C.c_int32), ("min_pivot", C.c_double),
                ("uv", _dp), ("cov", _dp), ("flags", _bp), ("S0", _dp), ("Spp", _dp), ("V", _dp), ("W", _dp), ("jac", _dp)]


PRED_NO_COV, PRED_NO_PROJECTION = 1, 2
BLOCK_POSE, BLOCK_SPEEDBIAS = 0, 1
COV_MAX_WINDOW_DIM, COV_MAX_DIM = 174, 30

# ... 494 lines not shown
```

Measured before the change: 565,400.

## Drop per-iteration small-factor launch via in-solve IMU repropagation pause check

Adds a three-launch iteration path in which the small-factor (IMU preintegration) kernel is skipped each iteration. Instead, the solve kernel checks whether the speed/bias change since the cached linearization point exceeds a threshold. If it does, the window pauses, a host-visible pause word is bumped, and the host later resumes paused windows with a full four-launch chain. This removes one kernel launch per Gauss-Newton iteration. In exchange it adds per-iteration checks inside the solve kernel, dual graph variants, extra host synchronization when pauses occur, and a redo/resume protocol that must keep the numerics identical.

```diff
diff --git a/include/okvis_amd_ba.h b/include/okvis_amd_ba.h
--- a/include/okvis_amd_ba.h
+++ b/include/okvis_amd_ba.h
@@ -117,6 +117,7 @@
 #define OKVIS_BA_TUNE_NO_SMALL_RIDE 0x100u
 #define OKVIS_BA_TUNE_SCHUR_SERIAL_BATCHES 0x200u
 #define OKVIS_BA_TUNE_LIN_NO_RECORDS 0x400u
+#define OKVIS_BA_TUNE_FOUR_LAUNCH 0x800u
 #define OKVIS_BA_SOLVE_AUTO 0
 #define OKVIS_BA_SOLVE_DENSE 1
 #define OKVIS_BA_SOLVE_CHAIN 2
@@ -227,6 +228,7 @@
 #define OKVIS_BA_LIST_CHAIN 19
 #define OKVIS_BA_LIST_CHUNK_RECS 20
 #define OKVIS_BA_LIST_GROUP_RECS 21
+#define OKVIS_BA_LIST_PLAN 22
 int okvis_ba_check_window_lists(const okvis_ba_window* w, const okvis_ba_options* opt, int32_t n_windows, int32_t which,
                                 int32_t* out, int64_t capacity, int64_t* n);
 #define OKVIS_BA_PATCH_POSE_PRIORS 1
@@ -321,8 +323,10 @@
 #define OKVIS_BA_ROUTE_SOLVE_MODE 14
 #define OKVIS_BA_ROUTE_SMALL_RIDES 15
 #define OKVIS_BA_ROUTE_LIN_RECORDS 16
-#define OKVIS_BA_ROUTE_COUNT 17
+#define OKVIS_BA_ROUTE_THREE_LAUNCH 17
+#define OKVIS_BA_ROUTE_COUNT 18
 int okvis_ba_launch_route(okvis_ba_solver* s, int32_t* route);
+int okvis_ba_pause_count(okvis_ba_solver* s, int64_t* count);
 
 #define OKVIS_BA_MARG_MAX_WINDOW_DIM 900
 typedef struct okvis_ba_marg_spec {
diff --git a/okvis_amd/_lib.py b/okvis_amd/_lib.py
--- a/okvis_amd/_lib.py
+++ b/okvis_amd/_lib.py
@@ -15,7 +15,7 @@
     "okvis_ba_evaluate_cost", "okvis_ba_get_state", "okvis_ba_fetch_results", "okvis_ba_fetch_imu_caches", "okvis_ba_array_size", "okvis_ba_download",
     "okvis_ba_reduced_dim", "okvis_ba_pair_count", "okvis_ba_pairs", "okvis_ba_last_iterate_ms",
     "okvis_ba_profile_iterations", "okvis_ba_profile_launches", "okvis_ba_algorithmic_bytes", "okvis_ba_synchronize",
-    "okvis_ba_helper_timeouts", "okvis_ba_launch_route", "okvis_ba_marginalize", "okvis_ba_marginalize_begin", "okvis_ba_marginalize_end",
+    "okvis_ba_helper_timeouts", "okvis_ba_launch_route", "okvis_ba_pause_count", "okvis_ba_marginalize", "okvis_ba_marginalize_begin", "okvis_ba_marginalize_end",
     "okvis_ba_marginalize_batch", "okvis_ba_marginalize_batch_begin", "okvis_ba_marginalize_batch_end",
     "okvis_ba_state_covariance", "okvis_ba_last_covariance_ms",
     "okvis_ba_landmark_covariance", "okvis_ba_last_landmark_covariance_ms",
@@ -101,6 +101,7 @@
     L.okvis_ba_reduced_dim.argtypes = [vp, C.c_int, _ip]
     L.okvis_ba_pair_count.argtypes = [vp, C.c_int, _ip]
     L.okvis_ba_helper_timeouts.argtypes = [vp, C.POINTER(C.c_int64)]
+    L.okvis_ba_pause_count.argtypes = [vp, C.POINTER(C.c_int64)]
     L.okvis_ba_launch_route.argtypes = [vp, _ip]
     L.okvis_ba_pairs.argtypes = [vp, C.c_int, _ip, _ip]
     L.okvis_ba_last_iterate_ms.argtypes = [vp, C.POINTER(C.c_float)]
diff --git a/okvis_amd/csrc/ba_capi.hip b/okvis_amd/csrc/ba_capi.hip
--- a/okvis_amd/csrc/ba_capi.hip
+++ b/okvis_amd/csrc/ba_capi.hip
@@ -97,6 +97,11 @@
   if (e == hipSuccess) e = hipEventCreate(&s->ev0);
   if (e == hipSuccess) e = hipEventCreate(&s->ev1);
   if (e == hipSuccess) e = hipEventCreateWithFlags(&s->ev_fork, hipEventDisableTiming);
+  if (e == hipSuccess) e = hipHostMalloc((void**)&s->h_pause, 64, hipHostMallocMapped | hipHostMallocCoherent);
+  if (e == hipSuccess) {
+    s->h_pause[0] = 0;
+    e = hipHostGetDevicePointer((void**)&s->d_pause, s->h_pause, 0);
+  }
   if (e == hipSuccess) e = hipMalloc(&s->d_opt, records_bytes(1));
   if (e == hipSuccess) {
     s->d_wins = reinterpret_cast<WinPtrs*>(reinterpret_cast<unsigned char*>(s->d_opt) + OPT_PAD);
@@ -131,6 +136,8 @@
   if (s->d_opt) (void)hipFree(s->d_opt);
   if (s->h_ctrl_stage) (void)hipHostFree(s->h_ctrl_stage);
   if (s->d_ctrl_stage) (void)hipFree(s->d_ctrl_stage);
+  if (s->h_pause) (void)hipHostFree(s->h_pause);
+  if (s->d_redo_mark) (void)hipFree(s->d_redo_mark);
   if (s->marg_scratch) (void)hipFree(s->marg_scratch);
   for (auto ev : s->ev_cov)
     if (ev) (void)hipEventDestroy(ev);
@@ -470,6 +477,7 @@
   const void* src = nullptr;
   int64_t count = 0;
   int width = 4;
+  std::vector<int32_t> plan_ints;
   switch (which) {
     case OKVIS_BA_LIST_GROUPS: src = at((const void*)P.groups), count = 16 * (int64_t)P.n_group; break;
     case OKVIS_BA_LIST_LM_OBS_BEGIN: src = at((const void*)P.lm_obs_begin), count = P.n_lm + 1; break;
@@ -514,6 +522,16 @@
       src = A.host.data() + off, count = (int64_t)stride * LIN_REC_INTS;
       break;
     }
+    case OKVIS_BA_LIST_PLAN: {
+      size_t off = 0;
+      BatchMax M = batch_max(&H, &H.ptrs, 1);
+      M.rec_stride = build_chunk_records(A, &H, 1, &off);
+      M.grec_stride = build_group_records(A, &H, 1, &off);
+      const LaunchPlan p = make_plan(L, M, o, n_windows);
+      plan_ints = {p.three, p.rides, p.small_iter.k == SMALL_PREPARE, p.budget, p.fused, p.solve.k, graph_key(10, false), graph_key(10, true)};
+      src = plan_ints.data(), count = (int64_t)plan_ints.size();
+      break;
+    }
     default: return OKVIS_BA_ERR_ARG;
   }
   *n = count;
@@ -767,8 +785,40 @@
     HIP_TRY(hipGetLastError());
   }
   HIP_TRY(launch_lin(s, whole(s), 1));
+  if (s->plan.three) {
+    const size_t n = s->wins.size();
+    if (s->redo_mark_windows < n) {
+      if (s->d_redo_mark) HIP_TRY(hipFree(s->d_redo_mark));
+      s->d_redo_mark = nullptr, s->redo_mark_windows = 0;
+      HIP_TRY(hipMalloc((void**)&s->d_redo_mark, sizeof(int) * n));
+      s->redo_mark_windows = n;
+    }
+    hipLaunchKernelGGL(redo_mark_kernel, dim3((unsigned)((n + 63) / 64)), dim3(64), 0, s->stream, s->d_wins, s->d_redo_mark, (int)n);
+    HIP_TRY(hipGetLastError());
+  }
+  s->pause_begin = s->pause_seen = __atomic_load_n(s->h_pause, __ATOMIC_ACQUIRE);
+  s->three_unseen = false;
   s->begun = true;
   s->evaluated = true;
+  return OKVIS_BA_OK;
+}
+
+static int settle_pauses(okvis_ba_solver* s, bool* four) {
+  *four = true;
+  if (!s->plan.three) return OKVIS_BA_OK;
+  if (s->three_unseen) {
+    HIP_TRY(hipStreamSynchronize(s->stream));
+    s->three_unseen = false;
+  }
+  const int word = __atomic_load_n(s->h_pause, __ATOMIC_ACQUIRE);
+  if (word != s->pause_seen) {
+    s->pause_seen = word;
+    std::vector<Ctrl> cs;
+    if (int rc = fetch_ctrl(s, cs)) return rc;
+    int n_paused = 0;
+    return resume_paused(s, cs, &n_paused);
+  }
+  *four = s->start_four;
   return OKVIS_BA_OK;
 }
 
@@ -779,57 +829,60 @@
   if (!s->begun) return OKVIS_BA_ERR_STATE;
   if (n == 0) return OKVIS_BA_OK;
   HIP_TRY(hipSetDevice(s->device));
+  bool four = true;
+  if (int rc = settle_pauses(s, &four)) return rc;
+  if (s->plan.three && !four) s->three_unseen = true;
   s->slots += n;
+  const int nsub = (int)s->sub_streams.size();
+  auto graph_of = [&](int k, bool r, hipGraphExec_t* exec) -> int {
+    const int key = graph_key(n, r);
+    if (k >= 0) {
+      auto it = s->sub_graphs.find({key, k});
+      if (it != s->sub_graphs.end()) return *exec = it->second, OKVIS_BA_OK;
+    } else {
+      auto it = s->graphs.find(key);
+      if (it != s->graphs.end()) return *exec = it->second, OKVIS_BA_OK;
+    }
+    hipGraph_t graph = nullptr;
+    const hipStream_t st = k >= 0 ? s->sub_streams[k] : s->stream;
+    HIP_TRY(hipStreamBeginCapture(st, hipStreamCaptureModeRelaxed));
+    hipError_t e = k >= 0 ? launch_chain(s, sub(st, s->plan.subs[k]), n, n, r) : launch_iterations_forked(s, n, -1, r);
+    hipError_t e2 = hipStreamEndCapture(st, &graph);
+    if (e != hipSuccess) HIP_TRY(e);
+    HIP_TRY(e2);
+    HIP_TRY(hipGraphInstantiate(exec, graph, nullptr, nullptr, 0));
+    HIP_TRY(hipGraphDestroy(graph));
+    if (k >= 0) s->sub_graphs[{key, k}] = *exec;
+    else s->graphs[key] = *exec;
+    return OKVIS_BA_OK;
+  };
+  std::vector<hipGraphExec_t> execs;
+  if (s->plan.graph) {
+    for (int k = nsub > 1 ? 0 : -1; k < (nsub > 1 ? nsub : 0); ++k) {
+      hipGraphExec_t exec = nullptr, other = nullptr;
+      if (int rc = graph_of(k, four, &exec)) return rc;
+      if (s->plan.three)
+        if (int rc = graph_of(k, !four, &other)) return rc;
+      execs.push_back(exec);
+    }
+  }
   HIP_TRY(hipEventRecord(s->ev0, s->stream));
-  const int nsub = (int)s->sub_streams.size();
   if (s->plan.graph && nsub > 1) {
     HIP_TRY(hipEventRecord(s->ev_fork, s->stream));
     for (int k = 0; k < nsub; ++k) {
-      hipGraphExec_t exec = nullptr;
-      auto it = s->sub_graphs.find({n, k});
-      if (it == s->sub_graphs.end()) {
-        hipGraph_t graph = nullptr;
-        const Sub b = sub(s->sub_streams[k], s->plan.subs[k]);
-        HIP_TRY(hipStreamBeginCapture(b.st, hipStreamCaptureModeRelaxed));
-        hipError_t e = launch_chain(s, b, n, n);
-        hipError_t e2 = hipStreamEndCapture(b.st, &graph);
-        if (e != hipSuccess) HIP_TRY(e);
-        HIP_TRY(e2);
-        HIP_TRY(hipGraphInstantiate(&exec, graph, nullptr, nullptr, 0));
-        HIP_TRY(hipGraphDestroy(graph));
-        s->sub_graphs[{n, k}] = exec;
-      } else {
-        exec = it->second;
-      }
       HIP_TRY(hipStreamWaitEvent(s->sub_streams[k], s->ev_fork, 0));
       if (k > 0 && s->stagger_ticks > 0) {
         hipLaunchKernelGGL(delay_kernel, dim3(1), dim3(64), 0, s->sub_streams[k], (long long)k * s->stagger_ticks);
         HIP_TRY(hipGetLastError());
       }
-      HIP_TRY(hipGraphLaunch(exec, s->sub_streams[k]));
+      HIP_TRY(hipGraphLaunch(execs[k], s->sub_streams[k]));
       HIP_TRY(hipEventRecord(s->sub_events[k], s->sub_streams[k]));
       HIP_TRY(hipStreamWaitEvent(s->stream, s->sub_events[k], 0));
     }
   } else if (s->plan.graph) {
-    hipGraphExec_t exec = nullptr;
-    auto it = s->graphs.find(n);
-    if (it == s->graphs.end()) {
-      hipGraph_t graph = nullptr;
-      HIP_TRY(hipStreamBeginCapture(s->stream, hipStreamCaptureModeRelaxed));
-      hipError_t e = launch_iterations_forked(s, n);
-      hipError_t e2 = hipStreamEndCapture(s->stream, &graph);
-      if (e != hipSuccess) HIP_TRY(e);
-      HIP_TRY(e2);
-      HIP_TRY(hipGraphInstantiate(&exec, graph, nullptr, nullptr, 0));
-      HIP_TRY(hipGraphDestroy(graph));
-      s->graphs[n] = exec;
-      HIP_TRY(hipEventRecord(s->ev0, s->stream));
-    } else {
-      exec = it->second;
-    }
-    HIP_TRY(hipGraphLaunch(exec, s->stream));
+    HIP_TRY(hipGraphLaunch(execs[0], s->stream));
   } else {
-    HIP_TRY(launch_iterations_forked(s, n));
+    HIP_TRY(launch_iterations_forked(s, n, -1, four));
   }
   HIP_TRY(hipEventRecord(s->ev1, s->stream));
   return OKVIS_BA_OK;
@@ -868,10 +921,24 @@
         HIP_TRY(hipMemcpyAsync(s->stage_res.data(), H0.ptrs.results, res_bytes, hipMemcpyDeviceToHost, s->stream));
       }
     }
-    return fetch_ctrl(s, cs);
+    return fetch_ctrl(s, cs, s->plan.three != 0);
   };
   int rc = finalize();
   if (rc != OKVIS_BA_OK) return rc;
+  if (s->plan.three) {
+    s->three_unseen = false;
+    int n_paused = 0;
+    if ((rc = resume_paused(s, cs, &n_paused)) != OKVIS_BA_OK) return rc;
+    if (n_paused > 0) {
+      HIP_TRY(launch_schur(s, whole(s), 1));
+      HIP_TRY(launch_solve(s, whole(s), 1));
+      if ((rc = finalize()) != OKVIS_BA_OK) return rc;
+    }
+    long redone = 0;
+    for (const Ctrl& c : cs) redone += c.pad2;
+    s->pause_seen = __atomic_load_n(s->h_pause, __ATOMIC_ACQUIRE);
+    s->start_four = s->pause_seen != s->pause_begin || redone > 0;
+  }
   if (s->opt.strategy == OKVIS_BA_STRATEGY_DOGLEG && !s->opt.gauss_newton) {
     for (int round = 0; round < 64 && !s->skip_topup; ++round) {
       int need = 0;
@@ -883,7 +950,7 @@
       }
       if (need <= 0) break;
       s->slots += need;
-      HIP_TRY(launch_iterations_forked(s, need, 0));
+      HIP_TRY(launch_iterations_forked(s, need, 0, true));
       HIP_TRY(launch_schur(s, whole(s), 1));
       HIP_TRY(launch_solve(s, whole(s), 1));
       rc = finalize();
@@ -1002,6 +1069,15 @@
   route[OKVIS_BA_ROUTE_SMALL_RIDES] = p.rides;
   route[OKVIS_BA_ROUTE_LIN_RECORDS] = p.grec_stride > 0;
   route[OKVIS_BA_ROUTE_SOLVE_MODE] = p.solve.k == SOLVE_NONE ? 0 : p.solve.k >= SOLVE_CHAIN ? OKVIS_BA_SOLVE_CHAIN : OKVIS_BA_SOLVE_DENSE;
+  route[OKVIS_BA_ROUTE_THREE_LAUNCH] = p.three;
+  return OKVIS_BA_OK;
+}
+int okvis_ba_pause_count(okvis_ba_solver* s, int64_t* count) {
+  if (!s || !count) return OKVIS_BA_ERR_ARG;
+  if (!s->uploaded) return OKVIS_BA_ERR_STATE;
+  HIP_TRY(hipSetDevice(s->device));
+  HIP_TRY(hipStreamSynchronize(s->stream));
+  *count = __atomic_load_n(s->h_pause, __ATOMIC_ACQUIRE) - s->pause_begin;
   return OKVIS_BA_OK;
 }
 int okvis_ba_pair_count(okvis_ba_solver* s, int w, int32_t* n_pair) {
diff --git a/okvis_amd/csrc/ba_solve.hpp b/okvis_amd/csrc/ba_solve.hpp
--- a/okvis_amd/csrc/ba_solve.hpp
+++ b/okvis_amd/csrc/ba_solve.hpp
@@ -103,6 +103,9 @@
 constexpr int SOLVE_HELPED_MAX_WINDOWS = 8;
 constexpr int MARG_BLOCKS_MAX = MAX_MARG_DIM / 6;
 constexpr int PRE_BLOCKS = 32;
+constexpr int PAUSE_MAX_TERMS = 16;
+constexpr int DONE_PAUSED = 64;
+constexpr double PAUSE_BIAS_THRESHOLD = 1e-4 * (1.0 - 1e-6);
 
 template <class LYT>
 __device__ void assemble_base(const WinPtrs& W, int acc, const LYT LY, double* S, double* g, double* d2,
@@ -427,8 +430,10 @@
 
 template <bool LARGE, bool DBUF, bool CHAIN = false>
 __global__ __launch_bounds__(SOLVE_THREADS) void solve_kernel(const WinPtrs* __restrict__ wins,
-                                                              const OptD* __restrict__ optp, int final_only, CtrlSlot* ctrls) {
+                                                              const OptD* __restrict__ optp, int final_only, CtrlSlot* ctrls,
+                                                              int* pause_word) {
   static_assert(!(LARGE && DBUF), "windows solved in HBM are never fused");
+  constexpr bool PAUSE = !LARGE && DBUF;
   static_assert(!(LARGE && CHAIN), "the chain solver is an LDS solver");
   extern __shared__ __attribute__((aligned(16))) double smem[];
   const long long t_start = clock64();
@@ -575,6 +580,27 @@
                         imu_v##j = src[on ? idx : 0]; }
     BA_IMU_REQ(0) BA_IMU_REQ(1) BA_IMU_REQ(2) BA_IMU_REQ(3) BA_IMU_REQ(4) BA_IMU_REQ(5)
 #undef BA_IMU_REQ
+  }
+  __shared__ double s_pz_ref[3 * PAUSE_MAX_TERMS], s_pz_dt[PAUSE_MAX_TERMS];
+  __shared__ int s_pz_ok[PAUSE_MAX_TERMS], s_pz_sb[PAUSE_MAX_TERMS], s_pause;
+  static_assert(PAUSE_MAX_TERMS == 16 && offsetof(ImuCacheD, valid) % 8 == 0, "16 terms x 4 roles = one wave; valid | redo_count is one word");
+  long long pz_a = 0, pz_b = 0;
+  int pz_c = 0;
+  const bool pz_on = PAUSE && pause_word != nullptr && W.n_imu > 0;
+  if constexpr (PAUSE) {
+    if (pz_on) {
+      typedef const __attribute__((address_space(1))) long long* gll;
+      const int u = tl - PRE_BLOCKS * 10, role = (u >> 4) & 3, f = u & 15;
+      const int fc = (u >= 0 && f < W.n_imu) ? f : 0;
+      auto cg = W.imu_cache + fc;
+      auto cp = W.imu_cache_prev + fc;
+      const gll pa = role == 0 ? (gll)(&cg->valid) : role == 1 ? (gll)(&cg->sb_ref[3])
+                     : role == 2 ? (gll)(&cg->sb_ref[5]) : as_global(W.imu_t0) + fc;
+      const gll pb = role == 0 ? (gll)(&cp->valid) : role == 1 ? (gll)(&cg->sb_ref[4])
+                     : role == 2 ? (gll)(&cg->sb_ref[5]) : as_global(W.imu_t1) + fc;
+      pz_a = *pa, pz_b = *pb;
+      pz_c = W.imu_sb0[fc];
+    }
   }
   const int goff = (int)(s_g - smem);
   const bool w0pri = !LARGE && n_pri > 0 && (W.n_pprior > 0 || W.n_sbprior > 0);
@@ -755,6 +781,7 @@
       s_old_cost = c.cost;
       s_lm_gmax = 0;
       s_fail = 0;
+      if constexpr (PAUSE) s_pause = 0;
       if (opt.dogleg) {
         if (pending) {
           c.last_rho = dl.rho;
@@ -887,6 +914,18 @@
         } else if (pre_on && t64 < PRE_BLOCKS * 10) {
           const int to = t64 - PRE_BLOCKS * 8;
           s_preoff[to] = to < PRE_BLOCKS ? (to < W.n_pose ? pre_po : -1) : (to - PRE_BLOCKS < W.n_sb ? pre_so : -1);
+        } else if (PAUSE && pz_on && t64 < PRE_BLOCKS * 10 + 4 * PAUSE_MAX_TERMS) {
+          const int u = t64 - PRE_BLOCKS * 10, role = u >> 4, f = u & 15;
+          if (role == 0) {
+            s_pz_ok[f] = f < W.n_imu ? ((int)pz_a == 1 && (int)pz_b == 0) : -1;
+            s_pz_sb[f] = pz_c;
+          } else if (role == 1) {
+            s_pz_ref[3 * f] = __longlong_as_double(pz_a), s_pz_ref[3 * f + 1] = __longlong_as_double(pz_b);
+          } else if (role == 2) {
+            s_pz_ref[3 * f + 2] = __longlong_as_double(pz_a);
+          } else {
+            s_pz_dt[f] = ns_to_sec(pz_b - pz_a);
+          }
         }
       };
       const int sum_expected = sum_launches + ((int)gridDim.y - 1);
@@ -1179,6 +1218,48 @@
     }
   }
   STAMP(6);
+  auto pause_check = [&]() {
+    if constexpr (PAUSE) {
+      const int f = tid - 192;
+      if (pz_on && f >= 0 && f < PAUSE_MAX_TERMS) {
+        if (Wl.n_imu > PAUSE_MAX_TERMS) s_pause = 1;
+        const int ok = s_pz_ok[f];
+        if (ok >= 0) {
+          const int b = s_pz_sb[f];
+          double v[3];
+          int off;
+          if (b < PRE_BLOCKS) {
+            off = s_preoff[PRE_BLOCKS + b];
+#pragma unroll
+            for (int k = 0; k < 3; ++k) v[k] = s_pre[PRE_BLOCKS * 7 + 9 * b + 3 + k];
+          } else {
+            off = Wl.sb_off[b];
+            auto xp = as_global(Wl.sb[acc] + 9 * (size_t)b);
+#pragma unroll
+            for (int k = 0; k < 3; ++k) v[k] = xp[3 + k];
+          }
+          double q = 0;
+#pragma unroll
+          for (int k = 0; k < 3; ++k) {
+            const double d = off >= 0 ? s_x[off + 3 + k] : 0.0;
+            const double db = (v[k] + d) - s_pz_ref[3 * f + k];
+            q += db * db;
+          }
+          if (!(ok == 1 && sqrt(q) * s_pz_dt[f] <= PAUSE_BIAS_THRESHOLD)) s_pause = 1;
+        }
+      }
+    }
+  };
+  auto pause_mark = [&]() {
+    if constexpr (PAUSE) {
+      if (pz_on && s_pause) c.done = DONE_PAUSED;
+    }
+  };
+  auto pause_tell = [&]() {
+    if constexpr (PAUSE) {
+      if (pz_on && s_pause) __hip_atomic_fetch_add(pause_word, 1, __ATOMIC_RELAXED, __HIP_MEMORY_SCOPE_SYSTEM);
+    }
+  };
   if constexpr (!LARGE) {
     if (opt.dogleg && c.explicit_next) {
       __shared__ double s_dl[2];
@@ -1235,6 +1316,7 @@
       __syncthreads();
       double s2 = 0, x2 = 0;
       trial_states(Wl, acc, s_x, tid, true, &s2, &x2, pre_on ? s_pre : nullptr, pre_on ? s_preoff : nullptr);
+      pause_check();
       s2 = wave_sum_full(s2);
       x2 = wave_sum_full(x2);
       if ((tid & 63) == 0) {
@@ -1256,7 +1338,9 @@
         c.explicit_next = 0;
         c.lambda = mu;
         c.pending = 1;
+        pause_mark();
         *gctrl = c;
+        pause_tell();
       }
       return;
     }
@@ -1317,6 +1401,7 @@
     STAMP(31);
     double x2 = 0, s2a = 0;
     trial_states(Wl, acc, s_x, tid, opt.dogleg != 0, &s2a, &x2, pre_on ? s_pre : nullptr, pre_on ? s_preoff : nullptr);
+    pause_check();
     STAMP(32);
     if (opt.dogleg) s2 = s2a;
     __shared__ double s_sc[4][SOLVE_THREADS / 64];
@@ -1351,7 +1436,9 @@
       c.have_tot = 0;
       c.iter++;
       c.pending = 1;
+      pause_mark();
       *gctrl = c;
+      pause_tell();
     }
   }
   STAMP(9);
diff --git a/okvis_amd/csrc/capi_launch.inc b/okvis_amd/csrc/capi_launch.inc
--- a/okvis_amd/csrc/capi_launch.inc
+++ b/okvis_amd/csrc/capi_launch.inc
@@ -75,6 +75,7 @@
                           &solve_kernel<false, true, true>, &solve_kernel<true, false>};
 enum { SCHUR_NONE, SCHUR_VALU, SCHUR_MFMA3, SCHUR_MFMA9, SCHUR_RIDE3, SCHUR_MFMA3_SERIAL, SCHUR_RIDE3_SERIAL };
 enum { SMALL_NONE, SMALL_ALL, SMALL_PREPARE };
+Extent make_extent(int w0, int nw) { return Extent{w0, nw, nw <= SOLVE_HELPED_MAX_WINDOWS ? SOLVE_HELPERS : 0}; }
 LaunchPlan make_plan(const BatchLayout& L, const BatchMax& M, const okvis_ba_options& o, int n_windows) {
   LaunchPlan p;
   const bool f32 = o.fp32_linearize != 0;
@@ -127,9 +128,11 @@
   }
   if (M.imu > 0 && o.strategy == OKVIS_BA_STRATEGY_DOGLEG && !o.gauss_newton) p.take_back = Launch{1, M.imu, 0};
   p.budget = o.strategy == OKVIS_BA_STRATEGY_DOGLEG;
+  p.three = p.small_iter.k == SMALL_PREPARE && p.budget && M.imu <= PAUSE_MAX_TERMS && p.solve.k != SOLVE_NONE && p.tiled.k == SOLVE_NONE &&
+            !(o.tuning.flags & OKVIS_BA_TUNE_FOUR_LAUNCH);
   int nsub = o.n_streams > 0 ? o.n_streams : (n_windows >= 128 ? 2 : (n_windows >= 56 ? 3 : (n_windows >= 8 ? 2 : 1)));
   nsub = std::max(1, std::min(nsub, n_windows));
-  auto extent = [](int w0, int nw) { return Extent{w0, nw, nw <= SOLVE_HELPED_MAX_WINDOWS ? SOLVE_HELPERS : 0}; };
+  auto extent = [](int w0, int nw) { return make_extent(w0, nw); };
   for (int k = 0; k < nsub; ++k) {
     const int w0 = (int)((int64_t)n_windows * k / nsub), w1 = (int)((int64_t)n_windows * (k + 1) / nsub);
     p.subs.push_back(extent(w0, w1 - w0));
@@ -158,10 +161,31 @@
     *W.ctrl = c;
   }
 }
-__global__ void gather_ctrl_kernel(const WinPtrs* wins, Ctrl* out, int n) {
+__global__ void gather_ctrl_kernel(const WinPtrs* wins, Ctrl* out, int n, const int* redo_mark) {
   const int w = blockIdx.x * (blockDim.x / 64) + threadIdx.x / 64, lane = threadIdx.x & 63;
-  if (w < n && lane < (int)(sizeof(Ctrl) / 8))
-    reinterpret_cast<double*>(out + w)[lane] = reinterpret_cast<const double*>(wins[w].ctrl)[lane];
+  if (w >= n) return;
+  constexpr int last = (int)(sizeof(Ctrl) / 8) - 1;
+  static_assert(offsetof(Ctrl, pad2) == sizeof(Ctrl) - 4, "the spare word closes the record");
+  if (lane > last) return;
+  union { double d; int i[2]; } v;
+  v.d = reinterpret_cast<const double*>(wins[w].ctrl)[lane];
+  if (redo_mark && lane == last) {
+    int r = 0;
+    for (int f = 0; f < wins[w].n_imu; ++f) r += wins[w].imu_cache[f].redo_count;
+    v.i[1] = r - redo_mark[w];
+  }
+  reinterpret_cast<double*>(out + w)[lane] = v.d;
+}
+__global__ void redo_mark_kernel(const WinPtrs* wins, int* redo_mark, int n) {
+  const int w = blockIdx.x * blockDim.x + threadIdx.x;
+  if (w >= n) return;
+  int r = 0;
+  for (int f = 0; f < wins[w].n_imu; ++f) r += wins[w].imu_cache[f].redo_count;
+  redo_mark[w] = r;
+}
+__global__ void resume_kernel(const WinPtrs* wins, int n) {
+  const int w = blockIdx.x * blockDim.x + threadIdx.x;
+  if (w < n && wins[w].ctrl->done == DONE_PAUSED) wins[w].ctrl->done = 0;
 }
 
 __global__ void delay_kernel(long long ticks) {
@@ -190,13 +214,14 @@
   }
   return hipGetLastError();
 }
-void launch_solve_kernel(okvis_ba_solver* s, const Launch& l, dim3 grid, hipStream_t st, const WinPtrs* wins, int final_only, CtrlSlot* ctrls) {
+void launch_solve_kernel(okvis_ba_solver* s, const Launch& l, dim3 grid, hipStream_t st, const WinPtrs* wins, int final_only, CtrlSlot* ctrls,
+                         int* pause = nullptr) {
   const SolveFn fn = SOLVE[l.k];
-  hipLaunchKernelGGL(fn, grid, dim3(SOLVE_THREADS), l.lds, st, wins, s->d_opt, final_only, ctrls);
-}
-hipError_t launch_solve(okvis_ba_solver* s, Sub b, int final_only) {
+  hipLaunchKernelGGL(fn, grid, dim3(SOLVE_THREADS), l.lds, st, wins, s->d_opt, final_only, ctrls, pause);
+}
+hipError_t launch_solve(okvis_ba_solver* s, Sub b, int final_only, int* pause = nullptr) {
   const LaunchPlan& p = s->plan;
-  if (p.solve.k) launch_solve_kernel(s, p.solve, dim3((unsigned)b.nw, 1 + b.helpers), b.st, s->d_wins + b.w0, final_only, s->d_ctrl + b.w0);
+  if (p.solve.k) launch_solve_kernel(s, p.solve, dim3((unsigned)b.nw, 1 + b.helpers), b.st, s->d_wins + b.w0, final_only, s->d_ctrl + b.w0, pause);
   if (p.tiled.k) {
     launch_solve_kernel(s, p.tiled, dim3((unsigned)b.nw), b.st, s->d_wins + b.w0, final_only, s->d_ctrl + b.w0);
     if (!final_only) {
@@ -210,10 +235,11 @@
   }
   return hipGetLastError();
 }
-hipError_t launch_lin(okvis_ba_solver* s, Sub b, int init) {
+hipError_t launch_lin(okvis_ba_solver* s, Sub b, int init, bool factors = true) {
   const LaunchPlan& p = s->plan;
   const WinPtrs* wins = s->d_wins + b.w0;
-  const Launch& f = init ? p.small_init : p.small_iter;
+  const Launch none;
+  const Launch& f = !factors ? none : init ? p.small_init : p.small_iter;
   if (f.k == SMALL_ALL) hipLaunchKernelGGL(small_kernel, dim3((unsigned)f.gx, (unsigned)b.nw), dim3(LIN_THREADS), f.lds, b.st, wins, init);
   if (f.k == SMALL_PREPARE) hipLaunchKernelGGL(small_prepare_kernel, dim3((unsigned)f.gx, (unsigned)b.nw), dim3(LIN_THREADS), f.lds, b.st, wins);
   const dim3 grid((unsigned)p.lin.gx, (unsigned)b.nw);
@@ -235,30 +261,32 @@
   hipLaunchKernelGGL(imu_take_back_kernel, dim3((unsigned)s->plan.take_back.gx, (unsigned)nw), dim3(64), 0, s->stream, s->d_wins + w0);
   return hipGetLastError();
 }
-hipError_t launch_iteration(okvis_ba_solver* s, Sub b) {
+hipError_t launch_iteration(okvis_ba_solver* s, Sub b, bool four) {
+  const bool three = s->plan.three && !four;
   hipError_t e;
   if ((e = launch_schur(s, b)) != hipSuccess) return e;
-  if ((e = launch_solve(s, b, 0)) != hipSuccess) return e;
-  return launch_lin(s, b, 0);
-}
+  if ((e = launch_solve(s, b, 0, three ? s->d_pause : nullptr)) != hipSuccess) return e;
+  return launch_lin(s, b, 0, !three);
+}
+inline int graph_key(int n, bool four) { return 2 * n + (four ? 1 : 0); }
 hipError_t launch_budget(okvis_ba_solver* s, Sub b, int n) {
   if (!s->plan.budget || n <= 0) return hipSuccess;
   hipLaunchKernelGGL(add_budget_kernel, dim3((unsigned)b.nw), dim3(64), 0, b.st, s->d_wins + b.w0, n);
   return hipGetLastError();
 }
-hipError_t launch_chain(okvis_ba_solver* s, Sub b, int n, int budget) {
+hipError_t launch_chain(okvis_ba_solver* s, Sub b, int n, int budget, bool four) {
   hipError_t e = launch_budget(s, b, budget);
-  for (int i = 0; i < n && e == hipSuccess; ++i) e = launch_iteration(s, b);
+  for (int i = 0; i < n && e == hipSuccess; ++i) e = launch_iteration(s, b, four);
   return e;
 }
-hipError_t launch_iterations_forked(okvis_ba_solver* s, int n, int budget = -1) {
+hipError_t launch_iterations_forked(okvis_ba_solver* s, int n, int budget, bool four) {
   const int nsub = (int)s->sub_streams.size();
   if (budget < 0) budget = n;
-  if (nsub <= 1) return launch_chain(s, whole(s), n, budget);
+  if (nsub <= 1) return launch_chain(s, whole(s), n, budget, four);
   hipError_t e = hipEventRecord(s->ev_fork, s->stream);
   for (int k = 0; k < nsub && e == hipSuccess; ++k) {
     e = hipStreamWaitEvent(s->sub_streams[k], s->ev_fork, 0);
-    if (e == hipSuccess) e = launch_chain(s, sub(s->sub_streams[k], s->plan.subs[k]), n, budget);
+    if (e == hipSuccess) e = launch_chain(s, sub(s->sub_streams[k], s->plan.subs[k]), n, budget, four);
     if (e == hipSuccess) e = hipEventRecord(s->sub_events[k], s->sub_streams[k]);
     if (e == hipSuccess) e = hipStreamWaitEvent(s->stream, s->sub_events[k], 0);
   }
@@ -287,11 +315,12 @@
   return e;
 }
 
-int fetch_ctrl(okvis_ba_solver* s, std::vector<Ctrl>& out) {
+int fetch_ctrl(okvis_ba_solver* s, std::vector<Ctrl>& out, bool redo = false) {
   const size_t n = s->wins.size();
   out.resize(n);
   HIP_TRY(reserve_ctrl_stage(s, n));
-  hipLaunchKernelGGL(gather_ctrl_kernel, dim3((unsigned)((n + 3) / 4)), dim3(256), 0, s->stream, s->d_wins, reinterpret_cast<Ctrl*>(s->d_ctrl_stage), (int)n);
+  hipLaunchKernelGGL(gather_ctrl_kernel, dim3((unsigned)((n + 3) / 4)), dim3(256), 0, s->stream, s->d_wins, reinterpret_cast<Ctrl*>(s->d_ctrl_stage), (int)n,
+                     redo && s->redo_mark_windows >= n ? s->d_redo_mark : nullptr);
   HIP_TRY(hipGetLastError());
   HIP_TRY(hipMemcpyAsync(s->h_ctrl_stage, s->d_ctrl_stage, sizeof(Ctrl) * n, hipMemcpyDeviceToHost, s->stream));
   HIP_TRY(hipStreamSynchronize(s->stream));
@@ -299,4 +328,30 @@
   return OKVIS_BA_OK;
 }
 
-}
+int resume_paused(okvis_ba_solver* s, const std::vector<Ctrl>& cs, int* n_paused) {
+  const int n = (int)cs.size();
+  auto owes = [&](int w) { return cs[w].done == DONE_PAUSED ? std::max(0, cs[w].max_iter - cs[w].iter) : -1; };
+  int most = 0;
+  *n_paused = 0;
+  for (int w0 = 0; w0 < n;) {
+    const int need = owes(w0);
+    int w1 = w0 + 1;
+    if (need < 0) {
+      w0 = w1;
+      continue;
+    }
+    while (w1 < n && owes(w1) == need) ++w1;
+    const Sub b = sub(s->stream, make_extent(w0, w1 - w0));
+    hipLaunchKernelGGL(resume_kernel, dim3((unsigned)((b.nw + 63) / 64)), dim3(64), 0, b.st, s->d_wins + b.w0, b.nw);
+    HIP_TRY(hipGetLastError());
+    HIP_TRY(launch_lin(s, b, 0));
+    HIP_TRY(launch_chain(s, b, need, 0, true));
+    most = std::max(most, need);
+    *n_paused += b.nw;
+    w0 = w1;
+  }
+  s->slots += most;
+  return OKVIS_BA_OK;
+}
+
+}
diff --git a/okvis_amd/csrc/capi_solver.inc b/okvis_amd/csrc/capi_solver.inc
--- a/okvis_amd/csrc/capi_solver.inc
+++ b/okvis_amd/csrc/capi_solver.inc
@@ -103,6 +103,7 @@
   Launch small_init, small_iter, lin; int lin_n_small = 0, sd = 0;
   int grec_stride = 0;
   Launch take_back; int budget = 0;
+  int three = 0;
   Extent whole; int one_helpers = 0;
 };
 struct LaunchPlan : PlanFixed {
@@ -170,6 +171,14 @@
   long long slots = 0;
   std::map<int, hipGraphExec_t> graphs;
   std::map<std::pair<int, int>, hipGraphExec_t> sub_graphs;
+  int* h_pause = nullptr;
+  int* d_pause = nullptr;
+  int pause_seen = 0;
+  int pause_begin = 0;
+  bool three_unseen = false;
+  bool start_four = false;
+  int* d_redo_mark = nullptr;
+  size_t redo_mark_windows = 0;
   float last_iterate_ms = 0.f;
   int last_hip_error = 0;
   unsigned char* marg_scratch = nullptr;
diff --git a/okvis_amd/solver.py b/okvis_amd/solver.py
--- a/okvis_amd/solver.py
+++ b/okvis_amd/solver.py
@@ -32,7 +32,7 @@
 
 INDEX_LISTS = ("groups", "lm_obs_begin", "lm_pair_begin", "pair_lm", "pair_block", "pair_off", "pair_role", "lm_piece_begin",
                "pair_piece", "pair_list_begin", "pair_list", "tasks", "task_list", "chunks", "chunk_diag_begin", "chunk_diag_out",
-               "chunk_desc", "piece_path", "ldl_comp", "chain", "chunk_recs", "group_recs")
+               "chunk_desc", "piece_path", "ldl_comp", "chain", "chunk_recs", "group_recs", "plan")
 
 
 def index_lists(window: Window, options: OptionsC | None = None, n_windows: int = 1) -> dict:
@@ -433,9 +433,14 @@
         _lib.check(self._L.okvis_ba_helper_timeouts(self._h, C.byref(n)))
         return n.value
 
+    def pause_count(self) -> int:
+        n = C.c_int64()
+        _lib.check(self._L.okvis_ba_pause_count(self._h, C.byref(n)))
+        return n.value
+
     ROUTE = ("windows", "fused", "decision_free_schur", "piece_path", "split_small", "sub_batches", "sub_batch_max_windows",
              "schur_kernel", "solve_dbuf", "solve_tiled", "solve_helpers", "graph", "max_chunks", "slots", "solve_mode", "small_rides",
-             "lin_records")
+             "lin_records", "three_launch")
 
     def launch_route(self) -> dict:
         r = (C.c_int32 * len(self.ROUTE))()
diff --git a/okvis_amd/window.py b/okvis_amd/window.py
--- a/okvis_amd/window.py
+++ b/okvis_amd/window.py
@@ -44,7 +44,7 @@
 
 TUNE_SCHUR_DECIDES, TUNE_SCHUR_VALU, TUNE_SCHUR_MFMA_LARGE, TUNE_NO_LDL_COMP, TUNE_LDL_COMP_ALL = 0x1, 0x2, 0x4, 0x8, 0x10
 TUNE_H0_ON_HOST, TUNE_NO_EARLY_PREINTEGRATION, TUNE_NO_MARG_TILES, TUNE_NO_SMALL_RIDE = 0x20, 0x40, 0x80, 0x100
-TUNE_SCHUR_SERIAL_BATCHES, TUNE_LIN_NO_RECORDS = 0x200, 0x400
+TUNE_SCHUR_SERIAL_BATCHES, TUNE_LIN_NO_RECORDS, TUNE_FOUR_LAUNCH = 0x200, 0x400, 0x800
 SOLVE_AUTO, SOLVE_DENSE, SOLVE_CHAIN = 0, 1, 2
 
 
```

Result: faster. 592,800 (median of 6 runs) (+4.8%).
